# ALRhub/d3il

Hardware: AMD Instinct MI355X
Metric: env-steps/s (higher is better)
Workload: dtype f64

## Files before the change

### d3il_amd/capi.py

```python
from __future__ import annotations

import ctypes as C
import os

from .model.blob import ModelBlob

_LIB = None


class Buffers(C.Structure):
    _fields_ = [("n_envs", C.c_int32), ("stride", C.c_int32), ("obs_dim", C.c_int32), ("action_dim", C.c_int32),
                ("obs", C.c_void_p), ("done", C.c_void_p), ("success", C.c_void_p), ("mode", C.c_void_p),
                ("state", C.c_void_p), ("flags", C.c_void_p), ("step_count", C.c_void_p), ("policy_des", C.c_void_p),
                ("info_f64", C.c_void_p), ("n_info_f64", C.c_int32), ("state_rows", C.c_int32), ("last_reset", C.c_void_p)]


STATE_F64 = 42
STATE_QPOS, STATE_QVEL, STATE_BIAS, STATE_TCP, STATE_IK_Q, STATE_IK_QD = 0, 9, 18, 25, 28, 35
FLAG_MODE_MASK, FLAG_TERMINATED, FLAG_SUCCESS, FLAG_ROD_CONTACT = 0x1FF, 1 << 12, 1 << 13, 1 << 14
FLAG_IK_VALID, FLAG_SOLVER_FAIL, FLAG_MULTI_CONTACT = 1 << 15, 1 << 16, 1 << 17
PUSH_STATE_BOX, PUSH_STATE_WARM, PUSH_STATE_TASK, PUSH_STATE_F64 = 42, 68, 89, 91
PFLAG_FIRST_MASK, PFLAG_MODE_MASK, PFLAG_WARM_VALID, PFLAG_CON_OVERFLOW, PFLAG_OFF_TABLE = 0x7, 0x38, 1 << 6, 1 << 18, 1 << 19
PFLAG_LINK_NEAR = 1 << 20
LINK_GUARD_SLACK = 1.25e-4
TASK_AVOIDING, TASK_PUSHING, TASK_SORTING, TASK_STACKING, TASK_ALIGNING, TASK_INSERTING = 0, 1, 2, 3, 4, 5
ALIGN_STATE_BOX, ALIGN_STATE_WARM, ALIGN_STATE_TARGET, ALIGN_STATE_F64 = 42, 55, 70, 77
STACK_STATE_BOX, STACK_STATE_WARM, STACK_STATE_F64 = 28, 67, 94
SFLAG_MODE_MASK, SFLAG_WARM_VALID, SFLAG_HAND_NEAR = 0xFF, 1 << 8, 1 << 20
TALLY_ROW, TALLY_ALL = 514, 256
ERCCL = -7
SORT_STATE_BOX, SORT_STATE_WARM, SORT_STATE_TASK, SORT_STATE_F64 = 42, 94, 127, 129
INS_STATE_BOX, INS_STATE_WARM, INS_STATE_TASK, INS_STATE_F64 = 42, 81, 108, 110
BUILD_POISON, BUILD_SK_POISON, BUILD_STATS = 1, 2, 4
BET_TAG = 0x42655448
DDPM_GPT_TAG = 0x44470000
IBC_TAG = 0x49420000
ACT_TAG = 0x41430000
CVAE_TAG = 0x43560000
DDPM_ACT_TAG = 0x44410000
HXG_CLIPPED, HXG_NONFINITE, HXG_LAUNCHES, HXG_N = 0, 1, 2, 4

EXPORTS = ["d3il_create", "d3il_destroy", "d3il_start", "d3il_reset", "d3il_step", "d3il_get_buffers", "d3il_get_state",
           "d3il_set_state", "d3il_policy_begin", "d3il_policy_action", "d3il_attention_causal_f32", "d3il_layernorm_f32", "d3il_mlp_gelu_residual_f32", "d3il_mlp_ln_gelu_residual_f32", "d3il_linear120_f32", "d3il_mlp_ln_gelu_residual_f16x3", "d3il_linear120_f16x3", "d3il_attn_half_f16x3", "d3il_f16x3_set_guard", "d3il_bet_head_f32", "d3il_ddpm_gpt_step_f32", "d3il_ibc_langevin_f32", "d3il_act_chunk_f32", "d3il_ddpm_act_chunk_f32", "d3il_cvae_decode_f32", "d3il_ddpm_mlp_f32", "d3il_resmlp_f32", "d3il_auto_reset", "d3il_set_tally", "d3il_count_metrics",
           "d3il_rccl_available", "d3il_comm_unique_id", "d3il_comm_init", "d3il_comm_count", "d3il_comm_destroy", "d3il_reduce_metrics", "d3il_set_timing",
           "d3il_last_step_ms", "d3il_timing_stats", "d3il_step_auto_reset", "d3il_random_rollout_step", "d3il_random_rollout_prepare", "d3il_group_create", "d3il_group_flush", "d3il_group_destroy", "d3il_group_set_option", "d3il_group_stats", "d3il_set_option", "d3il_set_link_guard", "d3il_debug_stats", "d3il_debug_wave_stats", "d3il_debug_wave_counts", "d3il_debug_scratch", "d3il_debug_build_flags", "d3il_last_error", "d3il_blob_sizeof", "d3il_version"]


class D3ilError(RuntimeError):
    pass


def lib_path() -> str:
    if os.environ.get("D3IL_LIB_PATH"):
        return os.environ["D3IL_LIB_PATH"]
    name = "libd3il_rollout_stats.so" if os.environ.get("D3IL_STATS_LIB") == "1" else "libd3il_rollout.so"
    return os.path.join(os.path.dirname(os.path.abspath(__file__)), name)


def load():
    global _LIB
    if _LIB is None:
        path = lib_path()
        if not os.path.exists(path):
            raise D3ilError("%s is missing: build it with `python -m d3il_amd.build` (hipcc, gfx950). "
                            "There is no CPU fallback for the rollout path." % path)
        L = C.CDLL(path)
        L.d3il_last_error.restype = C.c_char_p
        L.d3il_blob_sizeof.restype = C.c_size_t
        L.d3il_create.argtypes = [C.c_int, C.c_int, C.c_int, C.c_void_p, C.c_size_t, C.POINTER(C.c_void_p)]
        L.d3il_destroy.argtypes = [C.c_void_p]
        L.d3il_start.argtypes = [C.c_void_p, C.c_void_p]
        L.d3il_reset.argtypes = [C.c_void_p, C.c_void_p, C.c_void_p, C.c_void_p]
        L.d3il_step.argtypes = [C.c_void_p, C.c_void_p, C.c_void_p]
        L.d3il_get_buffers.argtypes = [C.c_void_p, C.POINTER(Buffers)]
        L.d3il_get_state.argtypes = [C.c_void_p, C.c_void_p, C.c_int32, C.c_void_p, C.c_void_p]
        L.d3il_set_state.argtypes = [C.c_void_p, C.c_void_p, C.c_int32, C.c_void_p, C.c_void_p]
        L.d3il_policy_begin.argtypes = [C.c_void_p, C.c_void_p, C.c_void_p]
        L.d3il_policy_action.argtypes = [C.c_void_p, C.c_uint64, C.c_uint64, C.c_uint32, C.c_void_p, C.c_void_p]
        L.d3il_count_metrics.argtypes = [C.c_void_p, C.c_void_p, C.c_void_p]
        L.d3il_attention_causal_f32.argtypes = [C.c_void_p, C.c_void_p, C.c_int, C.c_int, C.c_int, C.c_int, C.c_void_p]
        L.d3il_layernorm_f32.argtypes = [C.c_void_p, C.c_void_p, C.c_void_p, C.c_void_p, C.c_long, C.c_int, C.c_float, C.c_void_p]
        L.d3il_mlp_ln_gelu_residual_f32.argtypes = [C.c_void_p, C.c_void_p, C.c_void_p, C.c_float, C.c_void_p, C.c_void_p, C.c_void_p, C.c_void_p, C.c_void_p, C.c_long, C.c_int, C.c_int, C.c_void_p]
        L.d3il_linear120_f32.argtypes = [C.c_void_p, C.c_void_p, C.c_void_p, C.c_float, C.c_void_p, C.c_void_p, C.c_void_p, C.c_void_p, C.c_long, C.c_int, C.c_void_p]
        L.d3il_mlp_ln_gelu_residual_f16x3.argtypes = L.d3il_mlp_ln_gelu_residual_f32.argtypes
        L.d3il_linear120_f16x3.argtypes = L.d3il_linear120_f32.argtypes
        L.d3il_attn_half_f16x3.argtypes = [C.c_void_p, C.c_void_p, C.c_void_p, C.c_float, C.c_void_p, C.c_void_p, C.c_void_p, C.c_void_p, C.c_long, C.c_int, C.c_int, C.c_int, C.c_void_p]
        L.d3il_f16x3_set_guard.argtypes = [C.c_void_p]
        L.d3il_bet_head_f32.argtypes = [C.c_void_p, C.c_void_p, C.c_void_p, C.c_float] + [C.c_void_p] * 6 + [C.c_uint64, C.c_uint64] + [C.c_void_p] * 6 + [C.c_long, C.c_int, C.c_int, C.c_int, C.c_void_p]
        L.d3il_ddpm_gpt_step_f32.argtypes = [C.c_void_p, C.c_void_p, C.c_void_p, C.c_float] + [C.c_void_p] * 11 + [C.c_uint64, C.c_uint64] + [C.c_void_p] * 7 + [C.c_long] + [C.c_int] * 5 + [C.c_void_p]
        L.d3il_ibc_langevin_f32.argtypes = [C.c_void_p] * 10 + [C.c_float] + [C.c_void_p] * 5 + [C.c_uint64, C.c_uint64] + [C.c_void_p] * 11 + [C.c_long] + [C.c_int] * 6 + [C.c_void_p]
        L.d3il_act_chunk_f32.argtypes = [C.c_void_p] * 12 + [C.c_uint64, C.c_uint64] + [C.c_void_p] * 6 + [C.c_long] + [C.c_int] * 8 + [C.c_void_p]
        L.d3il_ddpm_act_chunk_f32.argtypes = [C.c_void_p] * 13 + [C.c_uint64, C.c_uint64] + [C.c_void_p] * 9 + [C.c_long] + [C.c_int] * 12 + [C.c_void_p]
        L.d3il_cvae_decode_f32.argtypes = [C.c_void_p] * 11 + [C.c_uint64, C.c_uint64] + [C.c_void_p] * 4 + [C.c_long] + [C.c_int] * 5 + [C.c_void_p]
        L.d3il_ddpm_mlp_f32.argtypes = [C.c_void_p] * 12 + [C.c_long, C.c_int, C.c_int, C.c_int, C.c_int, C.c_void_p]
        L.d3il_resmlp_f32.argtypes = [C.c_void_p] * 8 + [C.c_long, C.c_int, C.c_int, C.c_int, C.c_int, C.c_void_p]
        L.d3il_mlp_gelu_residual_f32.argtypes = [C.c_void_p, C.c_void_p, C.c_void_p, C.c_void_p, C.c_void_p, C.c_void_p, C.c_long, C.c_int, C.c_int, C.c_void_p]
        L.d3il_auto_reset.argtypes = [C.c_void_p, C.c_void_p, C.c_void_p]
        L.d3il_step_auto_reset.argtypes = [C.c_void_p, C.c_void_p, C.c_void_p, C.c_void_p]
        L.d3il_random_rollout_step.argtypes = [C.c_void_p, C.c_uint64, C.c_uint64, C.c_uint32, C.c_void_p, C.c_void_p, C.c_void_p]
        L.d3il_random_rollout_prepare.argtypes = [C.c_void_p, C.c_uint64, C.c_uint64, C.c_uint32, C.c_void_p, C.c_void_p, C.c_void_p]
        L.d3il_timing_stats.argtypes = [C.c_void_p, C.c_void_p]
        L.d3il_set_tally.argtypes = [C.c_void_p, C.c_void_p, C.c_int, C.c_void_p]
        L.d3il_comm_unique_id.argtypes = [C.c_void_p]
        L.d3il_comm_init.argtypes = [C.c_void_p, C.c_int, C.c_int, C.c_int, C.POINTER(C.c_void_p)]
        L.d3il_comm_destroy.argtypes = [C.c_void_p]
        L.d3il_comm_count.argtypes = [C.c_void_p, C.POINTER(C.c_int)]
        L.d3il_rccl_available.restype = C.c_int
        L.d3il_reduce_metrics.argtypes = [C.c_void_p, C.c_void_p, C.c_void_p, C.c_size_t, C.c_void_p]
        L.d3il_set_timing.argtypes = [C.c_void_p, C.c_int]
        L.d3il_last_step_ms.argtypes = [C.c_void_p, C.POINTER(C.c_float)]
        L.d3il_set_option.argtypes = [C.c_void_p, C.c_char_p, C.c_int]
        L.d3il_debug_scratch.argtypes = [C.c_void_p, C.c_int, C.c_void_p, C.c_int]
        L.d3il_debug_build_flags.argtypes = [C.c_void_p]
        L.d3il_set_link_guard.argtypes = [C.c_void_p, C.c_void_p, C.c_int, C.c_double, C.c_void_p]
        if hasattr(L, "d3il_group_create"):
            L.d3il_group_create.argtypes = [C.c_void_p, C.c_int, C.POINTER(C.c_void_p)]
            L.d3il_group_flush.argtypes = [C.c_void_p]
            L.d3il_group_destroy.argtypes = [C.c_void_p]
        if hasattr(L, "d3il_group_set_option"):
            L.d3il_group_set_option.argtypes = [C.c_void_p, C.c_char_p, C.c_int]
            L.d3il_group_stats.argtypes = [C.c_void_p, C.POINTER(C.c_int64), C.POINTER(C.c_int64)]
        if L.d3il_blob_sizeof() != C.sizeof(ModelBlob):
            raise D3ilError("model blob layout mismatch between include/d3il_model_blob.h and d3il_amd/model/blob.py")
        _LIB = L
    return _LIB


def has_step_group() -> bool:
    return hasattr(load(), "d3il_group_create")


def has_group_options() -> bool:
    return hasattr(load(), "d3il_group_set_option")


def is_unknown_group_option(err: Exception) -> bool:
    return isinstance(err, D3ilError) and "d3il_group_set_option: unknown option" in str(err)


def check(rc: int):
    if rc != 0:
        raise D3ilError("libd3il_rollout error %d: %s" % (rc, load().d3il_last_error().decode()))


_CAPSULES = os.path.join(os.path.dirname(os.path.abspath(__file__)), "model", "blobs", "panda_link_capsules.json")


def link_capsules(body_names, path: str | None = None):
    import json
    import numpy as np
    with open(path or _CAPSULES) as f:
        js = json.load(f)
    rows = [[body_names.index(c["body"]), c["statics"]] + list(c["p0"]) + list(c["p1"]) + [c["r"]] for c in js["capsules"]]
    return np.ascontiguousarray(rows, dtype=np.float64), float(js["margin"])


def set_link_guard(h, capsules, margin: float, counter_ptr=None):
    import numpy as np
    caps = np.zeros((0, 9)) if capsules is None else np.ascontiguousarray(capsules, dtype=np.float64).reshape(-1, 9)
    check(load().d3il_set_link_guard(h, caps.ctypes.data_as(C.c_void_p) if len(caps) else None, len(caps), float(margin), counter_ptr))
```

### d3il_amd/csrc/rollout.hip

```cpp
#include <hip/hip_runtime.h>
#include <cstdio>
#include <cstdlib>
#include <cstring>
#include <dlfcn.h>
#include <memory>
#include <mutex>
#include <string>
#include "../../include/d3il_rollout.h"
#include "panda_step.h"
#include "rigid_common.h"
#include "gen/avoiding_consts.inc"
#include "gen/stacking_consts.inc"

namespace d3il {
constexpr int WAVE = 64;
}
#include "gen_kernels.h"
#include "link_guard.h"
#include "stack_kernels.h"
#include "policy_f16x3.h"
#include "policy_bet.h"
#include "policy_ddpm_gpt.h"
#include "policy_ibc.h"
#include "policy_act.h"
// ... 31 lines not shown
#pragma unroll
  for (int i = 0; i < NARM; i++) s[(D3IL_STATE_BIAS + i) * (size_t)stride] = st.bias[i];
#pragma unroll
  for (int i = 0; i < 3; i++) s[(D3IL_STATE_TCP + i) * (size_t)stride] = st.tcp[i];
#pragma unroll
  for (int i = 0; i < NARM; i++) s[(D3IL_STATE_IK_Q + i) * (size_t)stride] = st.ikq[i];
#pragma unroll
  for (int i = 0; i < NARM; i++) s[(D3IL_STATE_IK_QD + i) * (size_t)stride] = st.ikqd[i];
  flags[e] = st.flags; steps[e] = st.step;
}
__device__ __forceinline__ void store_outputs(const EnvState& st, int e, const float* o, unsigned char dn, float* __restrict__ obs,
                                              unsigned char* __restrict__ done, unsigned char* __restrict__ success, unsigned short* __restrict__ mode) {
  obs[2 * e] = o[0]; obs[2 * e + 1] = o[1];
  done[e] = dn; success[e] = (st.flags & F_SUCCESS) ? 1 : 0; mode[e] = (unsigned short)(st.flags & F_MODE_MASK);
}

struct AvoidResetImage {
  const double* state;
  const unsigned* flags;
  const int* steps;
  const float* obs;
};
struct AvoidEpilogue {
  AvoidResetImage img;
  double* state; unsigned* flags; int* steps; float* obs; unsigned char* done; unsigned char* success; unsigned short* mode;
  double* des; long long* episode_counts; unsigned char* mask; const int* ctx_id; long long* table;
  double* actions; double* des_before;
  unsigned long long seed, env_offset;
  int n_ctx, n, stride, pad_;
};
typedef const __attribute__((address_space(4))) AvoidEpilogue CEpilogue4;
__device__ __forceinline__ void philox4x32_10(unsigned k0, unsigned k1, unsigned c0, unsigned c1, unsigned c2, unsigned c3, unsigned* out);
template <class IM>
__device__ __forceinline__ void store_reset_image(const IM& im, double* __restrict__ state, unsigned* __restrict__ flags, int* __restrict__ steps, float* __restrict__ obs,
                                                  unsigned char* __restrict__ done, unsigned char* __restrict__ success, unsigned short* __restrict__ mode, int stride, int e) {
  const double* src = im.state;
  double* s = state + e;
#pragma unroll
  for (int i = 0; i < D3IL_STATE_F64; i++) s[i * (size_t)stride] = src[i * WAVE];
  const unsigned fl = im.flags[0];
  flags[e] = fl; steps[e] = im.steps[0];
  obs[2 * e] = im.obs[0]; obs[2 * e + 1] = im.obs[1];
  done[e] = 0; success[e] = (fl & F_SUCCESS) ? 1 : 0; mode[e] = (unsigned short)(fl & F_MODE_MASK);
}
template <class EP>
__device__ __forceinline__ void avoiding_tail_lane(const EP& a, unsigned t_next, int e) {
  if (e >= a.n) return;
  unsigned char* done = a.done; unsigned char* success = a.success; unsigned short* mode = a.mode;
  const int stride = a.stride;
  const bool fin = done[e] != 0, ok = success[e] != 0;
  const int code = (int)(short)mode[e];
  a.mask[e] = fin ? 1 : 0;
  double* des = a.des;
  if (fin) {
    long long* episode_counts = a.episode_counts;
    atomicAdd((unsigned long long*)&episode_counts[0], 1ull);
    if (ok) atomicAdd((unsigned long long*)&episode_counts[1], 1ull);
    long long* table = a.table;
    if (table) {
      const int* ctx_id = a.ctx_id;
      int c = ctx_id ? ctx_id[e] : 0;
      if (c >= 0 && c < a.n_ctx) {
        long long* row = table + (size_t)c * D3IL_TALLY_ROW;
        atomicAdd((unsigned long long*)&row[0], 1ull);
        if (ok) {
          atomicAdd((unsigned long long*)&row[1], 1ull);
          if (code >= 0 && code < D3IL_TALLY_ROW - 2) atomicAdd((unsigned long long*)&row[2 + code], 1ull);
        }
      }
    }
    store_reset_image(a.img, a.state, a.flags, a.steps, a.obs, done, success, mode, stride, e);
    const double* tcp = a.img.state + D3IL_STATE_TCP * WAVE;
#pragma unroll
    for (int k = 0; k < 3; k++) des[k * (size_t)stride + e] = tcp[k * WAVE];
  }
  unsigned long long ge = a.env_offset + (unsigned long long)e;
  const unsigned long long seed = a.seed;
  unsigned r[4];
  philox4x32_10((unsigned)seed, (unsigned)(seed >> 32), (unsigned)ge, (unsigned)(ge >> 32), t_next, 0u, r);
  double u0 = r[0] * (1.0 / 4294967296.0), u1 = r[1] * (1.0 / 4294967296.0);
  double* des_before = a.des_before;
  const double dx = des[e], dy = des[(size_t)stride + e];
  des_before[e] = dx; des_before[(size_t)stride + e] = dy;
  double x = dx + (0.02 * u0 - 0.01), y = dy + (0.02 * u1 - 0.01), z = des[2 * (size_t)stride + e];
  des[e] = x; des[(size_t)stride + e] = y;
  double* act = a.actions + (size_t)e * 7;
  act[0] = x; act[1] = y; act[2] = z; act[3] = 0; act[4] = 1; act[5] = 0; act[6] = 0;
}

template <bool FAST, bool BAKED>
__global__ __launch_bounds__(WAVE) void k_avoiding_step(const PandaConsts* __restrict__ cp, double* __restrict__ state,
                                                        unsigned* __restrict__ flags, int* __restrict__ steps,
                                                        const double* __restrict__ actions, float* __restrict__ obs,
                                                        unsigned char* __restrict__ done, unsigned char* __restrict__ success,
                                                        unsigned short* __restrict__ mode, int n, int stride, int n_substeps, int max_steps, int lanes) {
  int e = blockIdx.x * lanes + threadIdx.x;
  if ((int)threadIdx.x >= lanes || e >= n) return;
  EnvState st;
  load_state(state, flags, steps, stride, e, st);
  double act[7];
#pragma unroll
  for (int k = 0; k < 7; k++) act[k] = actions[(size_t)e * 7 + k];
  const bool bad_action = sanitize_action(act, actions + (size_t)e * 7);
  float o[2]; unsigned char dn;
#if defined(D3IL_DEVICE_STATS)
  unsigned long long t0 = wall_clock64();
#endif
  if constexpr (BAKED) env_step<FAST>(kAvoidingConsts, st, act, o, &dn, n_substeps, max_steps);
  else env_step<FAST>(*to_const_as(cp), st, act, o, &dn, n_substeps, max_steps);
#if defined(D3IL_DEVICE_STATS)
  if (threadIdx.x == 0 && blockIdx.x < 4096) g_dev_wave[blockIdx.x][9] = wall_clock64() - t0;
#endif
  if (bad_action) st.flags |= F_SOLVER_FAIL | F_TERMINATED;
  store_state(state, flags, steps, stride, e, st);
  store_outputs(st, e, o, dn, obs, done, success, mode);
}

struct RareXch {
  static constexpr bool remote = true, retire = true;
  double* buf;
  int* ctl;
  int lane, seq;
  __device__ __forceinline__ void put(int k, double v) { buf[k * WAVE + lane] = v; }
  __device__ __forceinline__ double get(int k) const { return buf[k * WAVE + lane]; }
  __device__ __forceinline__ bool post(bool need) {
    const unsigned long long m = __ballot(need);
    if (lane == 0) { ctl[2] = (int)(unsigned)m; ctl[3] = (int)(unsigned)(m >> 32); }
    __builtin_amdgcn_fence(__ATOMIC_RELEASE, "workgroup");
    if (lane == 0) __hip_atomic_store(&ctl[0], seq, __ATOMIC_RELEASE, __HIP_MEMORY_SCOPE_WORKGROUP);
    if (m == 0) return false;
    while (__builtin_amdgcn_readfirstlane(__hip_atomic_load(&ctl[1], __ATOMIC_ACQUIRE, __HIP_MEMORY_SCOPE_WORKGROUP)) != seq) __builtin_amdgcn_s_sleep(1);
    __builtin_amdgcn_fence(__ATOMIC_ACQUIRE, "workgroup");
    return true;
  }
  __device__ __forceinline__ unsigned long long wait_request() {
    while (__builtin_amdgcn_readfirstlane(__hip_atomic_load(&ctl[0], __ATOMIC_ACQUIRE, __HIP_MEMORY_SCOPE_WORKGROUP)) != seq) __builtin_amdgcn_s_sleep(2);
    __builtin_amdgcn_fence(__ATOMIC_ACQUIRE, "workgroup");
    return (unsigned long long)(unsigned)ctl[2] | ((unsigned long long)(unsigned)ctl[3] << 32);
  }
  __device__ __forceinline__ void acknowledge() {
    __builtin_amdgcn_fence(__ATOMIC_RELEASE, "workgroup");
    if (lane == 0) __hip_atomic_store(&ctl[1], seq, __ATOMIC_RELEASE, __HIP_MEMORY_SCOPE_WORKGROUP);
  }
};
constexpr size_t AVOID_LDS_SERVE = (size_t)RX_ROWS * WAVE * sizeof(double) + 4 * sizeof(int);

constexpr int AVOID_GROUP_MAX = 8;
struct AvoidGroupMember {
  double* state; unsigned* flags; int* steps; const double* actions; float* obs; unsigned char* done; unsigned char* success; unsigned short* mode;
  const AvoidEpilogue* ep;
  int n, stride;
  unsigned first_wg, pad_;
};
struct AvoidGroupTable { AvoidGroupMember m[AVOID_GROUP_MAX]; };
typedef const __attribute__((address_space(4))) AvoidGroupTable CGroupTable4;
template <bool FAST, bool SERVE, bool GROUP = false>
__global__ __launch_bounds__((SERVE ? 3 : 2) * WAVE) void k_avoiding_step_split(typename std::conditional<GROUP, const AvoidGroupTable*, const PandaConsts*>::type __restrict__ cp, double* __restrict__ state,
                                                                  unsigned* __restrict__ flags, int* __restrict__ steps,
                                                                  const double* __restrict__ actions, float* __restrict__ obs,
                                                                  unsigned char* __restrict__ done, unsigned char* __restrict__ success,
                                                                  unsigned short* __restrict__ mode, int n, int stride, int n_substeps, int max_steps,
                                                                  const AvoidEpilogue* __restrict__ ep, unsigned t_next) {
  __shared__ double xch[2][2 * NARM][WAVE];
  __shared__ double trg[2][2 * NARM + 1][WAVE];
  extern __shared__ double rx_smem[];
  __shared__ unsigned long long ep_arg[3];
  const int lane = threadIdx.x & (WAVE - 1);
  const int role = threadIdx.x / WAVE;
  RareXch rx; rx.buf = rx_smem; rx.ctl = (int*)(rx_smem + RX_ROWS * WAVE); rx.lane = lane; rx.seq = 0;
  unsigned wg_index = blockIdx.x;
  if constexpr (GROUP) {
    CGroupTable4* gt = (CGroupTable4*)(unsigned long long)cp;
    int k = 0;
#pragma unroll
    for (int j = 1; j < AVOID_GROUP_MAX; j++) if (blockIdx.x >= gt->m[j].first_wg) k = j;
    state = gt->m[k].state; flags = gt->m[k].flags; steps = gt->m[k].steps; actions = gt->m[k].actions; obs = gt->m[k].obs;
    done = gt->m[k].done; success = gt->m[k].success; mode = gt->m[k].mode; ep = gt->m[k].ep; n = gt->m[k].n; stride = gt->m[k].stride;
    wg_index = blockIdx.x - gt->m[k].first_wg;
  }
  int e = wg_index * WAVE + lane;
  const bool live = e < n;
  if (!live) e = n - 1;
  const PandaConsts& c = kAvoidingConsts;
  (void)cp;
#if defined(D3IL_POISON)
  {
    auto poison = [](void* p, int words, int idx, int nthreads) { for (int q = idx; q < words; q += nthreads) ((unsigned long long*)p)[q] = D3IL_POISON_BITS; };
    const int nt = (SERVE ? 3 : 2) * WAVE;
    poison(&xch[0][0][0], 2 * 2 * NARM * WAVE, threadIdx.x, nt);
    poison(&trg[0][0][0], 2 * (2 * NARM + 1) * WAVE, threadIdx.x, nt);
    if (SERVE) poison(rx_smem, (int)(AVOID_LDS_SERVE / 8), threadIdx.x, nt);
    __syncthreads();
  }
#endif
#if defined(D3IL_DEVICE_STATS)
  unsigned long long t0 = wall_clock64(), tw = 0;
#endif
  if (role == 0) {
    const double* sp = state + e;
    double ikq[NARM], ikqd[NARM], q0[NARM], act[7], des[7];
#pragma unroll
    for (int i = 0; i < NARM; i++) {
      ikq[i] = sp[(D3IL_STATE_IK_Q + i) * (size_t)stride]; ikqd[i] = sp[(D3IL_STATE_IK_QD + i) * (size_t)stride];
      q0[i] = sp[(D3IL_STATE_QPOS + i) * (size_t)stride];
    }
#pragma unroll
    for (int k = 0; k < 7; k++) act[k] = actions[(size_t)e * 7 + k];
    unsigned fl = flags[e];
    sanitize_action(act, actions + (size_t)e * 7);
    make_setpoint(act, des);
    double vwarm[7];
    vwarm[6] = 0.0; trg[0][2 * NARM][lane] = 0.0;
#pragma clang loop unroll(disable)
    for (int s = 0; s < n_substeps; s++) {
      {
        double trig[2 * NARM + 1];
#pragma unroll
        for (int k = 0; k <= 2 * NARM; k++) trig[k] = trg[0][k][lane];
        ik_update<FAST>(c, des, des + 3, q0, fl, ikq, ikqd, vwarm, trig);
#pragma unroll
        for (int k = 0; k <= 2 * NARM; k++) trg[0][k][lane] = trig[k];
      }
      const int b = s & 1;
#pragma unroll
      for (int k = 0; k < NARM; k++) { xch[b][k][lane] = ikq[k]; xch[b][NARM + k][lane] = ikqd[k]; }
#if defined(D3IL_DEVICE_STATS)
      unsigned long long tb = wall_clock64();
#endif
      __syncthreads();
#if defined(D3IL_DEVICE_STATS)
      tw += wall_clock64() - tb;
#endif
    }
#if defined(D3IL_DEVICE_STATS)
    if (lane == 0 && blockIdx.x < 4096) { g_dev_wave[blockIdx.x][8] = wall_clock64() - t0 - tw; }
#endif
    if (live) {
      double* so = state + e;
#pragma unroll
      for (int i = 0; i < NARM; i++) { so[(D3IL_STATE_IK_Q + i) * (size_t)stride] = ikq[i]; so[(D3IL_STATE_IK_QD + i) * (size_t)stride] = ikqd[i]; }
    }
    __syncthreads();
  } else if (SERVE && role == 2) {
    double warm[6];
    warm[5] = 0.0;
    if (lane == 0) { rx.ctl[0] = 0; rx.ctl[1] = 0; }
#pragma clang loop unroll(disable)
    for (int s = 0; s < n_substeps; s++) {
      __syncthreads();
      rx.seq = s + 1;
      const unsigned long long m = rx.wait_request();
      if (m != 0) {
#if defined(D3IL_DEVICE_STATS)
        unsigned long long tb = wall_clock64();
#endif
        if ((m >> lane) & 1ull) rare_serve(c, &rx, warm);
        rx.acknowledge();
#if defined(D3IL_DEVICE_STATS)
        tw += wall_clock64() - tb;
#endif
      }
    }
#if defined(D3IL_DEVICE_STATS)
    if (lane == 0 && blockIdx.x < 4096) g_dev_wave[blockIdx.x][7] = tw;
#endif
    __syncthreads();
  } else {
    ep_arg[0] = (unsigned long long)ep; ep_arg[1] = t_next; ep_arg[2] = wg_index;
    EnvState st;
    load_state(state, flags, steps, stride, e, st);
    float o[2]; unsigned char dn;
    step_begin(c, st, o, &dn, max_steps);
    st.flags = ((((unsigned long long)ep | t_next) != 0ull) && dn && !(st.flags & F_SUCCESS)) ? (st.flags | F_RETIRED) : (st.flags & ~F_RETIRED);
    double warm[6];
    warm[5] = 0.0;
#pragma unroll
    for (int k = 0; k < NARM; k++) { double sk, ck; sincos(st.q[k], &sk, &ck); trg[1][k][lane] = sk; trg[1][NARM + k][lane] = ck; }
#pragma clang loop unroll(disable)
    for (int s = 0; s < n_substeps; s++) {
#if defined(D3IL_DEVICE_STATS)
      unsigned long long tb = wall_clock64();
#endif
      __syncthreads();
#if defined(D3IL_DEVICE_STATS)
      tw += wall_clock64() - tb;
#endif
      const int b = s & 1;
      double qd[NARM], qdd[NARM];
#pragma unroll
      for (int k = 0; k < NARM; k++) { qd[k] = xch[b][k][lane]; qdd[k] = xch[b][NARM + k][lane]; }
#if defined(D3IL_POISON)
      for (int k = 0; k < 2 * NARM; k++) ((unsigned long long*)&xch[b][k][lane])[0] = D3IL_POISON_BITS;
#endif
      double trig[2 * NARM];
#pragma unroll
      for (int k = 0; k < 2 * NARM; k++) trig[k] = trg[1][k][lane];
      if constexpr (SERVE) { rx.seq = s + 1; control_and_physics(c, st, qd, qdd, 0.04, false, warm, trig, &rx); }
      else control_and_physics(c, st, qd, qdd, 0.04, false, warm, trig, (RareInlineRetire*)nullptr);
#pragma unroll
      for (int k = 0; k < 2 * NARM; k++) trg[1][k][lane] = trig[k];
    }
#if defined(D3IL_DEVICE_STATS)
    if (lane == 0 && blockIdx.x < 4096) { g_dev_wave[blockIdx.x][9] = wall_clock64() - t0 - tw; }
#endif
    st.flags = (st.flags & ~F_RETIRED) | F_IK_VALID;
    if (action_is_bad(actions + (size_t)e * 7)) st.flags |= F_SOLVER_FAIL | F_TERMINATED;
    step_end(c, st);
    if (live) {
      double* so = state + e;
#pragma unroll
      for (int i = 0; i < NDOF; i++) { so[(D3IL_STATE_QPOS + i) * (size_t)stride] = st.q[i]; so[(D3IL_STATE_QVEL + i) * (size_t)stride] = st.v[i]; }
#pragma unroll
      for (int i = 0; i < NARM; i++) so[(D3IL_STATE_BIAS + i) * (size_t)stride] = st.bias[i];
#pragma unroll
      for (int i = 0; i < 3; i++) so[(D3IL_STATE_TCP + i) * (size_t)stride] = st.tcp[i];
      flags[e] = st.flags; steps[e] = st.step;
      store_outputs(st, e, o, dn, obs, done, success, mode);
    }
    __syncthreads();
    const unsigned ep_lo = __builtin_amdgcn_readfirstlane((unsigned)ep_arg[0]), ep_hi = __builtin_amdgcn_readfirstlane((unsigned)(ep_arg[0] >> 32));
    const unsigned long long ep_bits = (unsigned long long)ep_lo | ((unsigned long long)ep_hi << 32);
    const unsigned lane_now = __builtin_amdgcn_mbcnt_hi(~0u, __builtin_amdgcn_mbcnt_lo(~0u, 0u));
    if (ep_bits != 0ull) {
      const unsigned wg = __builtin_amdgcn_readfirstlane((unsigned)ep_arg[2]);
      avoiding_tail_lane(*(CEpilogue4*)ep_bits, __builtin_amdgcn_readfirstlane((unsigned)ep_arg[1]), (int)(wg * WAVE + lane_now));
    }
  }
}

__global__ __launch_bounds__(WAVE) void k_avoiding_reset(const PandaConsts* __restrict__ cp, const double* __restrict__ init_qpos,
                                                         const unsigned char* __restrict__ mask, double* __restrict__ state,
                                                         unsigned* __restrict__ flags, int* __restrict__ steps, float* __restrict__ obs,
                                                         unsigned char* __restrict__ done, unsigned char* __restrict__ success,
                                                         unsigned short* __restrict__ mode, int n, int stride) {
  int e = blockIdx.x * WAVE + threadIdx.x;
  if (e >= n) return;
  if (mask && !mask[e]) return;
  EnvState st;
  double iq[NARM];
#pragma unroll
  for (int k = 0; k < NARM; k++) iq[k] = init_qpos[k];
  float o[2];
  env_reset(kAvoidingConsts, st, iq, o);
  store_state(state, flags, steps, stride, e, st);
  store_outputs(st, e, o, 0, obs, done, success, mode);
}

__global__ __launch_bounds__(WAVE) void k_avoiding_auto_reset(AvoidResetImage img, double* __restrict__ state, unsigned* __restrict__ flags, int* __restrict__ steps,
                                                              float* __restrict__ obs, unsigned char* __restrict__ done,
                                                              unsigned char* __restrict__ success, unsigned short* __restrict__ mode,
                                                              double* __restrict__ des, long long* __restrict__ episode_counts, int n, int stride) {
  int e = blockIdx.x * WAVE + threadIdx.x;
  if (e >= n || !done[e]) return;
  atomicAdd((unsigned long long*)&episode_counts[0], 1ull);
  if (success[e]) atomicAdd((unsigned long long*)&episode_counts[1], 1ull);
  store_reset_image(img, state, flags, steps, obs, done, success, mode, stride, e);
#pragma unroll
  for (int k = 0; k < 3; k++) des[k * (size_t)stride + e] = img.state[(D3IL_STATE_TCP + k) * WAVE];
}

typedef float mlp_f4 __attribute__((ext_vector_type(4)));
constexpr int MLP_C = 120, MLP_H = 480, MLP_CHUNKS = MLP_H / 16, MLP_CHUNK_F = 16 * 256;
__device__ __forceinline__ void mlp_load_row(const float* __restrict__ src, long rr, int g, const float* __restrict__ ln_w, const float* __restrict__ ln_b, float eps, float* hk) {
#pragma unroll
  for (int s2 = 0; s2 < MLP_C / 4; s2++) hk[s2] = src[rr * MLP_C + 4 * s2 + g];
  if (ln_w) {
    float sum = 0.f;
#pragma unroll
    for (int s2 = 0; s2 < MLP_C / 4; s2++) sum += hk[s2];
    sum += __shfl_xor(sum, 16); sum += __shfl_xor(sum, 32);
    const float mean = sum * (1.0f / MLP_C);
    float var = 0.f;
#pragma unroll
    for (int s2 = 0; s2 < MLP_C / 4; s2++) { const float d = hk[s2] - mean; var += d * d; }
    var += __shfl_xor(var, 16); var += __shfl_xor(var, 32);
    const float rstd = 1.0f / sqrtf(var * (1.0f / MLP_C) + eps);
#pragma unroll
    for (int s2 = 0; s2 < MLP_C / 4; s2++) hk[s2] = (hk[s2] - mean) * rstd * ln_w[4 * s2 + g] + ln_b[4 * s2 + g];
  }
}
__global__ __launch_bounds__(256) void k_mlp_gelu_residual_f32(const float* __restrict__ h, const float* __restrict__ x, const float* __restrict__ wp,
                                                                const float* __restrict__ b1, const float* __restrict__ b2, float* __restrict__ out, long M,
                                                                const float* __restrict__ ln_w, const float* __restrict__ ln_b, float eps) {
  __shared__ mlp_f4 sw[2][MLP_CHUNK_F / 4];
  const int tid = threadIdx.x, lane = tid & 63, wave = tid >> 6, j = lane & 15, g = lane >> 4;
  const long row0 = (long)blockIdx.x * 64 + wave * 16, row = row0 + j;
  const bool live = row < M;
  const long rr = live ? row : (M - 1);
  float hk[MLP_C / 4];
  mlp_load_row(h, rr, g, ln_w, ln_b, eps, hk);
  mlp_f4 acc2[8];
#pragma unroll
  for (int t = 0; t < 8; t++) acc2[t] = mlp_f4{0.f, 0.f, 0.f, 0.f};
  const mlp_f4* wp4 = (const mlp_f4*)wp;
  mlp_f4 pre[4];
#pragma unroll
  for (int q = 0; q < 4; q++) sw[0][tid + 256 * q] = wp4[tid + 256 * q];
  __syncthreads();
  for (int c = 0; c < MLP_CHUNKS; c++) {
    const int cur = c & 1;
    if (c + 1 < MLP_CHUNKS) {
#pragma unroll
      for (int q = 0; q < 4; q++) pre[q] = wp4[(long)(c + 1) * (MLP_CHUNK_F / 4) + tid + 256 * q];
    }
    mlp_f4 acc1 = mlp_f4{0.f, 0.f, 0.f, 0.f}, acc1b = mlp_f4{0.f, 0.f, 0.f, 0.f};
#pragma unroll
    for (int q = 0; q < 8; q++) {
      const mlp_f4 a4 = sw[cur][q * 64 + lane];
#pragma unroll
      for (int e = 0; e < 4; e++) if (4 * q + e < MLP_C / 4) {
        if (e & 1) acc1b = __builtin_amdgcn_mfma_f32_16x16x4f32(a4[e], hk[4 * q + e], acc1b, 0, 0, 0);
        else acc1 = __builtin_amdgcn_mfma_f32_16x16x4f32(a4[e], hk[4 * q + e], acc1, 0, 0, 0);
      }
    }
    acc1 += acc1b;
    float gv[4];
#pragma unroll
    for (int r = 0; r < 4; r++) {
      const float v = acc1[r] + b1[16 * c + 4 * g + r];
      gv[r] = 0.5f * v * (1.0f + erff(v * 0.70710678118654752440f));
    }
#pragma unroll
    for (int t = 0; t < 8; t++) {
      const mlp_f4 a4 = sw[cur][(8 + t) * 64 + lane];
#pragma unroll
      for (int e = 0; e < 4; e++) acc2[t] = __builtin_amdgcn_mfma_f32_16x16x4f32(a4[e], gv[e], acc2[t], 0, 0, 0);
    }
    if (c + 1 < MLP_CHUNKS) {
#pragma unroll
      for (int q = 0; q < 4; q++) sw[cur ^ 1][tid + 256 * q] = pre[q];
    }
    __syncthreads();
  }
  if (!live) return;
#pragma unroll
  for (int t = 0; t < 8; t++) {
    const int col = 16 * t + 4 * g;
    if (col >= MLP_C) continue;
    const mlp_f4 xr = *(const mlp_f4*)(x + row * MLP_C + col), bb = *(const mlp_f4*)(b2 + col);
    *(mlp_f4*)(out + row * MLP_C + col) = xr + bb + acc2[t];
  }
}
__global__ __launch_bounds__(256) void k_linear120_f32(const float* __restrict__ xin, const float* __restrict__ wp, const float* __restrict__ bias, const float* __restrict__ resid,
                                                        float* __restrict__ out, long M, int N, const float* __restrict__ ln_w, const float* __restrict__ ln_b, float eps) {
  __shared__ mlp_f4 sw[2][8 * 64];
  const int tid = threadIdx.x, lane = tid & 63, wave = tid >> 6, j = lane & 15, g = lane >> 4;
  const long row = (long)blockIdx.x * 64 + wave * 16 + j;
  const bool live = row < M;
  const long rr = live ? row : (M - 1);
  float hk[MLP_C / 4];
  mlp_load_row(xin, rr, g, ln_w, ln_b, eps, hk);
  const int ntiles = (N + 15) / 16;
  const mlp_f4* wp4 = (const mlp_f4*)wp;
  mlp_f4 pre[2];
#pragma unroll
  for (int q = 0; q < 2; q++) sw[0][tid + 256 * q] = wp4[tid + 256 * q];
  __syncthreads();
  for (int t = 0; t < ntiles; t++) {
    const int cur = t & 1;
    if (t + 1 < ntiles) {
#pragma unroll
      for (int q = 0; q < 2; q++) pre[q] = wp4[(long)(t + 1) * 512 + tid + 256 * q];
    }
    mlp_f4 acc = mlp_f4{0.f, 0.f, 0.f, 0.f}, acc_b = mlp_f4{0.f, 0.f, 0.f, 0.f};
#pragma unroll
    for (int q = 0; q < 8; q++) {
      const mlp_f4 a4 = sw[cur][q * 64 + lane];
#pragma unroll
      for (int e = 0; e < 4; e++) if (4 * q + e < MLP_C / 4) {
        if (e & 1) acc_b = __builtin_amdgcn_mfma_f32_16x16x4f32(a4[e], hk[4 * q + e], acc_b, 0, 0, 0);
        else acc = __builtin_amdgcn_mfma_f32_16x16x4f32(a4[e], hk[4 * q + e], acc, 0, 0, 0);
      }
    }
    const int col = 16 * t + 4 * g;
    if (live && col < N) {
      mlp_f4 v = acc + acc_b + *(const mlp_f4*)(bias + col);
      if (resid) v += *(const mlp_f4*)(resid + row * (long)N + col);
      *(mlp_f4*)(out + row * (long)N + col) = v;
    }
// ... 250 lines not shown
    }
  };
  for (int half = 0; half < 2; half++) {
    const int i = half == 0 ? p : T - 1 - p;
    if (half == 1 && i == p) break;
    float q[DR], acc[DR], kk[DR], vv[DR];
    load(base + (long)i * 3 * C, q);
#pragma unroll
    for (int d = 0; d < DR; d++) q[d] *= scale;
    load(base + C, kk); load(base + 2 * C, acc);
    float m = 0.0f, l = 1.0f;
#pragma unroll
    for (int d = 0; d < DR; d++) m += q[d] * kk[d];
    for (int j = 1; j <= i; j++) {
      const float* kj = base + (long)j * 3 * C + C;
      load(kj, kk); load(kj + C, vv);
      float sc = 0.0f;
#pragma unroll
      for (int d = 0; d < DR; d++) sc += q[d] * kk[d];
      const float mn = fmaxf(m, sc), corr = __expf(m - mn), pj = __expf(sc - mn);
      l = l * corr + pj;
#pragma unroll
      for (int d = 0; d < DR; d++) acc[d] = acc[d] * corr + pj * vv[d];
      m = mn;
    }
    float* o = out + (b * T + i) * (long)C + h * D;
    const float inv = 1.0f / l;
    if constexpr (D4 > 0) {
#pragma unroll
      for (int c = 0; c < D4; c++) reinterpret_cast<float4*>(o)[c] = make_float4(acc[4 * c] * inv, acc[4 * c + 1] * inv, acc[4 * c + 2] * inv, acc[4 * c + 3] * inv);
    } else {
#pragma unroll
      for (int d = 0; d < 32; d++) if (d < D) o[d] = acc[d] * inv;
    }
  }
  if (p == 0) {
    float s0 = 0.0f;
    for (int d = 0; d < D; d++) s0 += (base[d] * scale) * base[C + d];
    if (dd_nonfinite(s0)) {
      float* o = out + (b * T) * (long)C + h * D;
      const float qnan = __uint_as_float(0x7FC00000u);
      for (int d = 0; d < D; d++) o[d] = qnan;
    }
  }
}

__device__ __forceinline__ void philox4x32_10(unsigned k0, unsigned k1, unsigned c0, unsigned c1, unsigned c2, unsigned c3, unsigned* out) {
  const unsigned M0 = 0xD2511F53u, M1 = 0xCD9E8D57u, W0 = 0x9E3779B9u, W1 = 0xBB67AE85u;
#pragma unroll
  for (int r = 0; r < 10; r++) {
    unsigned hi0 = __umulhi(M0, c0), lo0 = M0 * c0, hi1 = __umulhi(M1, c2), lo1 = M1 * c2;
    unsigned n0 = hi1 ^ c1 ^ k0, n1 = lo1, n2 = hi0 ^ c3 ^ k1, n3 = lo0;
    c0 = n0; c1 = n1; c2 = n2; c3 = n3; k0 += W0; k1 += W1;
  }
  out[0] = c0; out[1] = c1; out[2] = c2; out[3] = c3;
}
__global__ void k_policy_begin(const unsigned char* __restrict__ mask, const double* __restrict__ state, double* __restrict__ des, int n, int stride) {
  int e = blockIdx.x * blockDim.x + threadIdx.x;
  if (e >= n || (mask && !mask[e])) return;
#pragma unroll
  for (int k = 0; k < 3; k++) des[k * (size_t)stride + e] = state[(D3IL_STATE_TCP + k) * (size_t)stride + e];
}
__global__ void k_policy_action(double* __restrict__ des, double* __restrict__ actions, unsigned long long seed, unsigned long long env_offset,
                                unsigned t, int n, int stride) {
  int e = blockIdx.x * blockDim.x + threadIdx.x;
  if (e >= n) return;
  unsigned long long ge = env_offset + (unsigned long long)e;
  unsigned r[4];
  philox4x32_10((unsigned)seed, (unsigned)(seed >> 32), (unsigned)ge, (unsigned)(ge >> 32), t, 0u, r);
  double u0 = r[0] * (1.0 / 4294967296.0), u1 = r[1] * (1.0 / 4294967296.0);
  double x = des[e] + (0.02 * u0 - 0.01), y = des[(size_t)stride + e] + (0.02 * u1 - 0.01), z = des[2 * (size_t)stride + e];
  des[e] = x; des[(size_t)stride + e] = y;
  double* a = actions + (size_t)e * 7;
  a[0] = x; a[1] = y; a[2] = z; a[3] = 0; a[4] = 1; a[5] = 0; a[6] = 0;
}
__global__ void k_policy_action_dev(double* __restrict__ des, double* __restrict__ actions, unsigned long long seed, unsigned long long env_offset,
                                    const unsigned* __restrict__ t_dev, int n, int stride) {
  int e = blockIdx.x * blockDim.x + threadIdx.x;
  if (e >= n) return;
  const unsigned t = *t_dev;
  unsigned long long ge = env_offset + (unsigned long long)e;
  unsigned r[4];
  philox4x32_10((unsigned)seed, (unsigned)(seed >> 32), (unsigned)ge, (unsigned)(ge >> 32), t, 0u, r);
  double u0 = r[0] * (1.0 / 4294967296.0), u1 = r[1] * (1.0 / 4294967296.0);
  double x = des[e] + (0.02 * u0 - 0.01), y = des[(size_t)stride + e] + (0.02 * u1 - 0.01), z = des[2 * (size_t)stride + e];
  des[e] = x; des[(size_t)stride + e] = y;
  double* a = actions + (size_t)e * 7;
  a[0] = x; a[1] = y; a[2] = z; a[3] = 0; a[4] = 1; a[5] = 0; a[6] = 0;
}
__global__ void k_inc_counter(unsigned* __restrict__ t_dev) { if (threadIdx.x == 0 && blockIdx.x == 0) *t_dev += 1u; }
__global__ __launch_bounds__(WAVE) void k_avoiding_tail(AvoidEpilogue a, unsigned t_next) { avoiding_tail_lane(a, t_next, (int)(blockIdx.x * WAVE + threadIdx.x)); }
__global__ void k_restore_des(double* __restrict__ des, const double* __restrict__ des_before, int n, int stride) {
  int e = blockIdx.x * blockDim.x + threadIdx.x;
  if (e >= n) return;
  des[e] = des_before[e]; des[(size_t)stride + e] = des_before[(size_t)stride + e];
}

__global__ void k_count_metrics(const unsigned char* __restrict__ done, const unsigned* __restrict__ flags, long long* __restrict__ counts, int n) {
  int e = blockIdx.x * blockDim.x + threadIdx.x;
  if (e >= n) return;
  if (done[e]) atomicAdd((unsigned long long*)&counts[0], 1ull);
  if (flags[e] & F_SUCCESS) {
    atomicAdd((unsigned long long*)&counts[1], 1ull);
    atomicAdd((unsigned long long*)&counts[2 + (flags[e] & F_MODE_MASK)], 1ull);
  }
}

__global__ void k_episode_tally(const unsigned char* __restrict__ done, const unsigned char* __restrict__ success, const unsigned short* __restrict__ mode,
                                const int* __restrict__ ctx_id, long long* __restrict__ table, long long* __restrict__ episode_counts, int n, int n_ctx, int mode_bias, int all_by_code) {
  int e = blockIdx.x * blockDim.x + threadIdx.x;
  if (e >= n || !done[e]) return;
  if (episode_counts) {
    atomicAdd((unsigned long long*)&episode_counts[0], 1ull);
    if (success[e]) atomicAdd((unsigned long long*)&episode_counts[1], 1ull);
  }
  if (!table) return;
  int c = ctx_id ? ctx_id[e] : 0;
  if (c < 0 || c >= n_ctx) return;
  long long* row = table + (size_t)c * D3IL_TALLY_ROW;
  atomicAdd((unsigned long long*)&row[0], 1ull);
  int code = (int)(short)mode[e] + mode_bias;
  if (success[e]) {
    atomicAdd((unsigned long long*)&row[1], 1ull);
    if (code >= 0 && code < D3IL_TALLY_ROW - 2) atomicAdd((unsigned long long*)&row[2 + code], 1ull);
  }
  if (all_by_code && code >= 0 && code < 256) atomicAdd((unsigned long long*)&row[2 + D3IL_TALLY_ALL + code], 1ull);
}
__global__ void k_store_contexts(const unsigned char* __restrict__ mask, const double* __restrict__ src, double* __restrict__ dst, int n, int dim) {
  int i = blockIdx.x * blockDim.x + threadIdx.x;
  if (i >= n * dim) return;
  if (mask && !mask[i / dim]) return;
  dst[i] = src[i];
}

}

using namespace d3il;

static_assert(D3IL_STACK_STATE_BOX == SK_STATE_BOX && D3IL_STACK_STATE_WARM == SK_STATE_WARM && D3IL_STACK_STATE_F64 == SK_STATE_F64, "d3il_rollout.h: Stacking state layout");
static_assert(D3IL_SFLAG_WARM_VALID == SKF_WARM_VALID && D3IL_SFLAG_HAND_NEAR == SKF_HAND_NEAR && D3IL_PFLAG_CON_OVERFLOW == SKF_CON_OVERFLOW && D3IL_PFLAG_OFF_TABLE == SKF_OFF_TABLE,
              "d3il_rollout.h: Stacking flag bits");
static_assert(D3IL_PFLAG_LINK_NEAR == LG_FLAG && D3IL_PFLAG_LINK_NEAR == D3IL_SFLAG_HAND_NEAR, "d3il_rollout.h: the link-near bit of the generic engine is the hand-near bit of the cooperative one");
static_assert(D3IL_SFLAG_MODE_MASK == (SKF_NMODE_MASK | (0x3Fu << SKF_IND_SHIFT)), "d3il_rollout.h: Stacking order code");
static_assert(D3IL_ALIGN_STATE_BOX == AL_STATE_BOX && D3IL_ALIGN_STATE_WARM == AL_STATE_WARM && D3IL_ALIGN_STATE_TARGET == AL_STATE_TARGET && D3IL_ALIGN_STATE_F64 == AL_STATE_F64, "d3il_rollout.h: Aligning state layout");
static_assert(D3IL_INS_STATE_BOX == 42 && D3IL_INS_STATE_WARM == 42 + 13 * 3 && D3IL_INS_STATE_TASK == 42 + 13 * 3 + 6 * 3 + NDOF && D3IL_INS_STATE_F64 == gen_state_rows(3), "d3il_rollout.h: Inserting state layout");
static_assert(D3IL_PUSH_STATE_BOX == 42 && D3IL_PUSH_STATE_WARM == 42 + 13 * 2 && D3IL_PUSH_STATE_TASK == 42 + 13 * 2 + 6 * 2 + NDOF && D3IL_PUSH_STATE_F64 == gen_state_rows(2) && D3IL_TALLY_ALL + 256 <= D3IL_TALLY_ROW - 2,
              "d3il_rollout.h: Pushing state rows / tally row");

static inline bool gen_task(int task_id) {
  return task_id == D3IL_TASK_SORTING || task_id == D3IL_TASK_INSERTING || task_id == D3IL_TASK_PUSHING;
}

constexpr int RG_SLOTS = 2, RG_SAMPLE = 8;
struct d3il_handle_s {
  int task_id, n, stride, device;
  PandaConsts hc;
  PandaConsts* dc;
  GenConsts gc;
  StackConsts kc;
  AlignTask atk;
  double* d_scratch;
  int state_rows;
  double* d_init_qpos;
  bool started;
  d3il_buffers buf;
  bool fast, timing;
  int split;
  bool serve_avail;
  int serve_max_wg;
  int lanes;
  int lds_pad;
  hipEvent_t ev0, ev1;
  bool ev_valid, ev_created;
  hipEvent_t ring0[128], ring1[128];
  bool ring_created;
  long ring_head, ring_drained, t_n;
  double t_sum, t_min, t_max;
  int tol_mode;
  int stack_reset_coop;
  unsigned long long kc_id;
  double* d_ctx;
  int ctx_dim;
  uint8_t* d_mask;
  const int32_t* tally_ctx; int tally_nctx; int64_t* tally_table;
  bool rg_enabled, rg_ready, rg_capturing, rg_ev_made, rg_timing;
  int rg_slot;
  hipGraph_t rg_graph[RG_SLOTS]; hipGraphExec_t rg_exec[RG_SLOTS];
  unsigned* rg_t_dev; uint32_t rg_next_t; long rg_launched, rg_drained;
  uint64_t rg_seed, rg_off; double* rg_actions; int64_t* rg_counts; hipStream_t rg_stream;
  void* d_reset_img; AvoidResetImage reset_img; AvoidEpilogue* d_epilogue; AvoidEpilogue epilogue_host; bool epilogue_valid; hipStream_t epilogue_stream;
  bool prep_valid; uint32_t prep_t; uint64_t prep_seed, prep_off; double* prep_actions; bool fuse_tail; double* d_des_before; hipStream_t prep_stream;
  bool info_is_view;
  d3il_model_blob model;
  LinkGuardConsts lg; LinkGuardConsts* d_lg; int64_t* lg_flagged;
  struct d3il_group_s* group; int grp_set; bool grp_pending; uint64_t grp_seed, grp_off; uint32_t grp_t; double* grp_actions; int64_t* grp_counts; hipStream_t grp_stream;
  hipEvent_t ring_alt0[128], ring_alt1[128];
};
struct d3il_dispatch_set {
  int count; d3il_handle_s* m[AVOID_GROUP_MAX];
  int n_pending;
  uint32_t t; int n_substeps, max_steps; bool timing;
  AvoidGroupTable* d_table; AvoidGroupTable table_host; bool table_valid;
  hipEvent_t ev_join[AVOID_GROUP_MAX], ev_done; bool ev_made;
  hipEvent_t ring0[128], ring1[128]; bool ring_created; long ring_head;
  bool armed;
};
struct d3il_group_s {
  int device, count; d3il_handle_s* m[AVOID_GROUP_MAX];
  int n_sets; d3il_dispatch_set set[AVOID_GROUP_MAX];
  int n_pending; bool busy;
  bool quiet; int64_t n_merged, n_joined;
};
static inline void group_arm(d3il_group_s* g) { for (int k = 0; k < AVOID_GROUP_MAX; k++) g->set[k].armed = true; }
#if defined(D3IL_EVENT_SYSTEM_FENCE)
constexpr unsigned EV_ORDER_FLAGS = hipEventDisableTiming, EV_TIMING_FLAGS = hipEventDefault;
#else
constexpr unsigned EV_ORDER_FLAGS = hipEventDisableTiming | hipEventDisableSystemFence, EV_TIMING_FLAGS = hipEventDefault | hipEventDisableSystemFence;
#endif

struct ActiveModel { int refs; bool valid; GenConsts gc; StackConsts kc; };
static ActiveModel g_active_gen[16], g_active_stack[16];
static int g_active_tol[16];
static std::mutex g_model_mutex;

static unsigned long long g_stack_loaded_id[16];
static StackConsts g_stack_loaded[16];
static unsigned long long g_kc_counter = 0;

static thread_local std::string g_err;
static int fail(int code, const std::string& msg) { g_err = msg; return code; }
#define HIPCHK(x) do { hipError_t e_ = (x); if (e_ != hipSuccess) return fail(D3IL_EHIP, std::string(#x) + ": " + hipGetErrorString(e_)); } while (0)

extern "C" {

static int group_flush(d3il_group_s* g);
static inline int group_settle(d3il_handle_s* h) {
  if (!h || !h->group || h->group->busy) return D3IL_OK;
  group_arm(h->group);
  return h->group->n_pending ? group_flush(h->group) : D3IL_OK;
}
#define GROUP_SETTLE(h) do { if (int rc_g_ = group_settle(h)) return rc_g_; } while (0)

const char* d3il_last_error(void) { return g_err.c_str(); }
size_t d3il_blob_sizeof(void) { return sizeof(d3il_model_blob); }
int d3il_version(void) { return 2; }

static void rg_drop(d3il_handle_s* h);
static void group_leave(d3il_handle_s* h);
static void rg_drop_for_free(d3il_handle_s* h) {
  if (h->rg_ready) for (int k = 0; k < RG_SLOTS; k++) { (void)hipGraphExecDestroy(h->rg_exec[k]); (void)hipGraphDestroy(h->rg_graph[k]); }
  if (h->rg_t_dev) (void)hipFree(h->rg_t_dev);
}
static void free_handle(d3il_handle_s* h) {
  if (!h) return;
  int dev = h->device;
  if (dev >= 0 && dev < 16) {
    std::lock_guard<std::mutex> lock(g_model_mutex);
    if (gen_task(h->task_id) && g_active_gen[dev].refs > 0) g_active_gen[dev].refs--;
    if (h->task_id == D3IL_TASK_STACKING && g_active_stack[dev].refs > 0) g_active_stack[dev].refs--;
  }
  void* ptrs[] = {h->dc, h->d_init_qpos, h->buf.obs, h->buf.done, h->buf.success, h->buf.mode, h->buf.state, h->buf.flags, h->buf.step_count, h->buf.policy_des,
                  h->info_is_view ? nullptr : (void*)h->buf.info_f64, h->d_scratch, h->d_ctx, h->d_mask, h->d_des_before, h->d_lg, h->d_reset_img, h->d_epilogue};
  for (void* p : ptrs) if (p) (void)hipFree(p);
  if (h->ring_created) for (int i = 0; i < 128; i++) { (void)hipEventDestroy(h->ring0[i]); (void)hipEventDestroy(h->ring1[i]); }
  rg_drop_for_free(h);
  delete h;
}
#define HIPCHK_H(x) do { hipError_t e_ = (x); if (e_ != hipSuccess) { free_handle(h); return fail(D3IL_EHIP, std::string(#x) + ": " + hipGetErrorString(e_)); } } while (0)

int d3il_create(int task_id, int n_envs, int device_id, const void* model_blob, size_t blob_len, d3il_handle* out) {
  if (!out || !model_blob) return fail(D3IL_EINVAL, "d3il_create: null argument");
  *out = nullptr;
  if (blob_len != sizeof(d3il_model_blob)) return fail(D3IL_EBLOB, "d3il_create: blob size mismatch");
  if (n_envs <= 0) return fail(D3IL_EINVAL, "d3il_create: n_envs must be positive");
  const d3il_model_blob& m = *(const d3il_model_blob*)model_blob;
  if (task_id != m.task_id) return fail(D3IL_EINVAL, "d3il_create: task_id does not match the model blob");
  if (task_id != D3IL_TASK_AVOIDING && task_id != D3IL_TASK_PUSHING && task_id != D3IL_TASK_SORTING && task_id != D3IL_TASK_STACKING && task_id != D3IL_TASK_ALIGNING && task_id != D3IL_TASK_INSERTING)
    return fail(D3IL_EUNSUPPORTED, "d3il_create: unknown task id (Avoiding, Pushing, Sorting, Stacking, Aligning and Inserting are implemented)");
  int ndev = 0;
  if (hipGetDeviceCount(&ndev) != hipSuccess || ndev <= 0) return fail(D3IL_ENODEVICE, "d3il_create: no HIP device available (there is no CPU fallback)");
  if (device_id < 0 || device_id >= ndev || device_id >= 16) return fail(D3IL_ENODEVICE, "d3il_create: device_id out of range");
  HIPCHK(hipSetDevice(device_id));
  d3il_handle_s* h = new d3il_handle_s();
  std::memset(&h->buf, 0, sizeof h->buf);
  h->task_id = -1; h->device = device_id;
  h->model = m; h->d_lg = nullptr; h->lg_flagged = nullptr; h->lg.n = 0;
  h->dc = nullptr; h->d_init_qpos = nullptr; h->d_scratch = nullptr; h->d_ctx = nullptr; h->d_mask = nullptr; h->ev_created = false; h->ring_created = false;
  h->tally_ctx = nullptr; h->tally_nctx = 0; h->tally_table = nullptr; h->tol_mode = 0; h->ctx_dim = 0; h->stack_reset_coop = 1; h->kc_id = 0;
  const char* err = "";
  int rc = build_panda_consts(m, h->hc, &err);
  if (rc) { free_handle(h); return fail(D3IL_EBLOB, std::string("d3il_create: ") + err); }
  finish_invweights(h->hc);
  if (gen_task(task_id) && build_gen_consts(m, h->hc, h->gc, &err)) { free_handle(h); return fail(D3IL_EBLOB, std::string("d3il_create: ") + err); }
  if (task_id == D3IL_TASK_STACKING && build_stack_consts(m, h->hc, h->kc, &err)) { free_handle(h); return fail(D3IL_EBLOB, std::string("d3il_create: ") + err); }
  if (task_id == D3IL_TASK_ALIGNING && build_coop_align_consts(m, h->hc, h->kc, h->atk, &err)) { free_handle(h); return fail(D3IL_EBLOB, std::string("d3il_create: ") + err); }
  {
    PandaConsts a = h->hc, b = task_id == D3IL_TASK_STACKING ? kStackingConsts : kAvoidingConsts;
    if (task_id != D3IL_TASK_AVOIDING) {
      a.n_obst = b.n_obst;
      std::memcpy(a.ob_c, b.ob_c, sizeof a.ob_c); std::memcpy(a.ob_u, b.ob_u, sizeof a.ob_u); std::memcpy(a.ob_r, b.ob_r, sizeof a.ob_r); std::memcpy(a.ob_h, b.ob_h, sizeof a.ob_h);
      std::memcpy(a.ct_K, b.ct_K, sizeof a.ct_K); std::memcpy(a.ct_B, b.ct_B, sizeof a.ct_B); std::memcpy(a.ct_solimp, b.ct_solimp, sizeof a.ct_solimp);
      std::memcpy(a.ct_margin, b.ct_margin, sizeof a.ct_margin); std::memcpy(a.ct_fric, b.ct_fric, sizeof a.ct_fric); std::memcpy(a.task_f, b.task_f, sizeof a.task_f);
    }
    bool same = a.n_obst == b.n_obst && a.ik_iters == b.ik_iters;
    a.n_obst = b.n_obst = 0; a.ik_iters = b.ik_iters = 0; a.n_substeps = b.n_substeps = 0; a.max_steps = b.max_steps = 0; a.pad_i = b.pad_i = 0; a.pad_j = b.pad_j = 0;
    const double* pa = (const double*)&a; const double* pb = (const double*)&b;
    for (size_t i = 0; same && i < sizeof(PandaConsts) / sizeof(double); i++) {
      double d = pa[i] - pb[i], m = pa[i] < 0 ? -pa[i] : pa[i];
      if (!(d <= 1e-12 * (m > 1 ? m : 1) && -d <= 1e-12 * (m > 1 ? m : 1))) same = false;
    }
    if (!same) { free_handle(h); return fail(D3IL_EUNSUPPORTED, "d3il_create: the model blob differs from the model this library was specialised for at build time; "
                                                                 "regenerate csrc/gen/*_consts.inc and rebuild (python -m d3il_amd.build)"); }
  }
  const bool sorting = gen_task(task_id);
  const bool gen_pushing = sorting && task_id == D3IL_TASK_PUSHING;
  const bool stacking = task_id == D3IL_TASK_STACKING;
  if (stacking) {
    ActiveModel& am = g_active_stack[device_id];
    bool other;
    { std::lock_guard<std::mutex> lock(g_model_mutex); other = am.refs > 0 && std::memcmp(&am.kc, &h->kc, sizeof(StackConsts)) != 0; }
    if (other) {
      free_handle(h);
      return fail(D3IL_EUNSUPPORTED, "d3il_create: another live Stacking handle on this device uses a different model (the kernels read one model per device from constant memory); destroy it first");
    }
  }
  h->n = n_envs; h->stride = (n_envs + WAVE - 1) / WAVE * WAVE;
  h->started = false; h->split = -1; h->serve_avail = true; h->serve_max_wg = 256; h->lanes = WAVE; h->lds_pad = -1; h->fast = true; h->timing = false; h->ev_valid = false;
  const bool aligning = task_id == D3IL_TASK_ALIGNING;
  h->state_rows = (sorting ? gen_state_rows(h->gc.nb) : (stacking ? SK_STATE_F64 : (aligning ? AL_STATE_F64 : D3IL_STATE_F64)));
  h->ctx_dim = (sorting ? 7 * h->gc.nb : (stacking ? 21 : (aligning ? AL_CTX : 0)));
  size_t S = (size_t)h->stride;
  d3il_buffers& b = h->buf;
  b.n_envs = n_envs; b.stride = h->stride; b.obs_dim = sorting ? 2 + 3 * h->gc.nb : (stacking ? SK_OBS : (aligning ? AL_OBS : 2)); b.action_dim = stacking ? SK_ACT : 7; b.state_rows = h->state_rows; b.n_info_f64 = (aligning || gen_pushing) ? 2 : (stacking ? 1 : 0);
  HIPCHK_H(hipMalloc(&h->dc, sizeof(PandaConsts)));
  if (task_id == D3IL_TASK_AVOIDING) {
    if (hipFuncSetAttribute((const void*)k_avoiding_step_split<true, true>, hipFuncAttributeMaxDynamicSharedMemorySize, (int)AVOID_LDS_SERVE) != hipSuccess) {
      (void)hipGetLastError();
      h->serve_avail = false; h->serve_max_wg = 0;
    }
    const size_t img_bytes = (size_t)WAVE * (D3IL_STATE_F64 * sizeof(double) + sizeof(unsigned) + sizeof(int) + 2 * sizeof(float) + 2 + sizeof(unsigned short));
    HIPCHK_H(hipMalloc(&h->d_reset_img, img_bytes)); HIPCHK_H(hipMemset(h->d_reset_img, 0, img_bytes));
    HIPCHK_H(hipMalloc(&h->d_epilogue, sizeof(AvoidEpilogue)));
  }
  HIPCHK_H(hipMemcpy(h->dc, &h->hc, sizeof(PandaConsts), hipMemcpyHostToDevice));
  HIPCHK_H(hipMalloc(&h->d_init_qpos, 7 * sizeof(double)));
  HIPCHK_H(hipMalloc(&b.obs, S * b.obs_dim * sizeof(float)));
  HIPCHK_H(hipMalloc(&b.done, S)); HIPCHK_H(hipMalloc(&b.success, S));
  HIPCHK_H(hipMalloc(&b.mode, S * sizeof(uint16_t)));
  HIPCHK_H(hipMalloc(&b.state, S * h->state_rows * sizeof(double)));
  HIPCHK_H(hipMalloc(&b.flags, S * sizeof(uint32_t)));
  HIPCHK_H(hipMalloc(&b.step_count, S * sizeof(int32_t)));
  HIPCHK_H(hipMalloc(&b.policy_des, S * 3 * sizeof(double)));
  HIPCHK_H(hipMalloc(&h->d_mask, S)); HIPCHK_H(hipMemset(h->d_mask, 0, S));
  b.last_reset = h->d_mask;
  HIPCHK_H(hipMemset(b.obs, 0, S * b.obs_dim * sizeof(float))); HIPCHK_H(hipMemset(b.done, 0, S)); HIPCHK_H(hipMemset(b.success, 0, S));
  HIPCHK_H(hipMemset(b.mode, 0, S * sizeof(uint16_t))); HIPCHK_H(hipMemset(b.state, 0, S * h->state_rows * sizeof(double)));
  HIPCHK_H(hipMemset(b.flags, 0, S * sizeof(uint32_t))); HIPCHK_H(hipMemset(b.step_count, 0, S * sizeof(int32_t)));
  HIPCHK_H(hipMemset(b.policy_des, 0, S * 3 * sizeof(double)));
  if (h->ctx_dim) { HIPCHK_H(hipMalloc(&h->d_ctx, S * h->ctx_dim * sizeof(double))); HIPCHK_H(hipMemset(h->d_ctx, 0, S * h->ctx_dim * sizeof(double))); }
  if (sorting) {
    {
      std::lock_guard<std::mutex> lock(g_model_mutex);
      g_active_gen[device_id].refs++; h->task_id = task_id;
    }
#if defined(D3IL_POISON)
    HIPCHK_H(hipMalloc(&h->d_scratch, S * GG_BLOCK * sizeof(double))); HIPCHK_H(hipMemset(h->d_scratch, 0xFF, S * GG_BLOCK * sizeof(double)));
#else
    HIPCHK_H(hipMalloc(&h->d_scratch, S * GG_BLOCK * sizeof(double))); HIPCHK_H(hipMemset(h->d_scratch, 0, S * GG_BLOCK * sizeof(double)));
#endif
    if (gen_pushing) { b.info_f64 = b.state + (size_t)(gen_state_rows(h->gc.nb) - 2) * S; h->info_is_view = true; }
    HIPCHK_H(hipFuncSetAttribute((const void*)k_sorting_step<true, false>, hipFuncAttributeMaxDynamicSharedMemorySize, GEN_LDS_STEP));
    HIPCHK_H(hipFuncSetAttribute((const void*)k_sorting_step<false, false>, hipFuncAttributeMaxDynamicSharedMemorySize, GEN_LDS_STEP));
    HIPCHK_H(hipFuncSetAttribute((const void*)k_sorting_step<true, true>, hipFuncAttributeMaxDynamicSharedMemorySize, GEN_LDS_STEP));
    HIPCHK_H(hipFuncSetAttribute((const void*)k_sorting_step<false, true>, hipFuncAttributeMaxDynamicSharedMemorySize, GEN_LDS_STEP));
    HIPCHK_H(hipFuncSetAttribute((const void*)k_sorting_reset, hipFuncAttributeMaxDynamicSharedMemorySize, GEN_LDS_H));
  }
  if (stacking) {
    ActiveModel& am = g_active_stack[device_id];
    {
      std::unique_lock<std::mutex> lock(g_model_mutex);
      if (am.refs == 0) am.kc = h->kc;
      am.refs++; h->task_id = task_id;
      h->kc_id = ++g_kc_counter;
    }
    HIPCHK_H(hipMalloc(&b.info_f64, S * sizeof(double))); HIPCHK_H(hipMemset(b.info_f64, 0, S * sizeof(double)));
    HIPCHK_H(hipMalloc(&h->d_scratch, S * SG_SIZE * sizeof(double))); HIPCHK_H(hipMemset(h->d_scratch, 0, S * SG_SIZE * sizeof(double)));
    HIPCHK_H(hipFuncSetAttribute((const void*)k_stacking_step, hipFuncAttributeMaxDynamicSharedMemorySize, STACK_LDS));
    HIPCHK_H(hipFuncSetAttribute((const void*)k_stacking_reset, hipFuncAttributeMaxDynamicSharedMemorySize, STACK_LDS_RESET));
  }
  if (aligning) {
    {
      std::lock_guard<std::mutex> lock(g_model_mutex);
      h->kc_id = ++g_kc_counter;
    }
    HIPCHK_H(hipMalloc(&b.info_f64, S * 2 * sizeof(double))); HIPCHK_H(hipMemset(b.info_f64, 0, S * 2 * sizeof(double)));
    HIPCHK_H(hipMalloc(&h->d_scratch, S * SG_SIZE * sizeof(double))); HIPCHK_H(hipMemset(h->d_scratch, 0, S * SG_SIZE * sizeof(double)));
    HIPCHK_H(hipFuncSetAttribute((const void*)k_aligning_step, hipFuncAttributeMaxDynamicSharedMemorySize, STACK_LDS));
  }
  h->task_id = task_id;
  h->ring_created = false; h->ring_head = h->ring_drained = h->t_n = 0; h->t_sum = 0; h->t_min = 1e300; h->t_max = 0;
  h->ev_created = true;
  *out = h;
  return D3IL_OK;
}

int d3il_destroy(d3il_handle h) {
  if (!h) return fail(D3IL_EINVAL, "d3il_destroy: null handle");
  (void)hipSetDevice(h->device);
  group_leave(h);
  (void)hipDeviceSynchronize();
  free_handle(h);
  return D3IL_OK;
}

int d3il_start(d3il_handle h, const double* init_qpos7) {
  GROUP_SETTLE(h);
  if (!h || !init_qpos7) return fail(D3IL_EINVAL, "d3il_start: null argument");
  for (int k = 0; k < 7; k++) if (!(init_qpos7[k] == init_qpos7[k])) return fail(D3IL_EINVAL, "d3il_start: init_qpos contains NaN");
  HIPCHK(hipSetDevice(h->device));
  HIPCHK(hipMemcpy(h->d_init_qpos, init_qpos7, 7 * sizeof(double), hipMemcpyHostToDevice));
  if (h->task_id == D3IL_TASK_AVOIDING) {
    double* st = (double*)h->d_reset_img;
    unsigned* fl = (unsigned*)(st + (size_t)D3IL_STATE_F64 * WAVE);
    int* sc = (int*)(fl + WAVE);
    float* ob = (float*)(sc + WAVE);
    unsigned char* dn = (unsigned char*)(ob + 2 * WAVE);
    unsigned short* md = (unsigned short*)(dn + 2 * WAVE);
    HIPCHK(hipDeviceSynchronize());
    hipLaunchKernelGGL(k_avoiding_reset, dim3(1), dim3(WAVE), 0, (hipStream_t)nullptr, h->dc, h->d_init_qpos, (const unsigned char*)nullptr, st, fl, sc, ob, dn, dn + WAVE, md, 1, WAVE);
    HIPCHK(hipGetLastError());
    HIPCHK(hipDeviceSynchronize());
    h->reset_img.state = st; h->reset_img.flags = fl; h->reset_img.steps = sc; h->reset_img.obs = ob;
  }
  h->started = true;
  return D3IL_OK;
}

static AlignTask g_align_loaded[16];
static bool g_align_loaded_valid[16];
static int sync_stack_consts_locked(d3il_handle_s* h) {
  if (h->task_id == D3IL_TASK_ALIGNING && (!g_align_loaded_valid[h->device] || std::memcmp(&g_align_loaded[h->device], &h->atk, sizeof(AlignTask)) != 0)) {
    HIPCHK(hipDeviceSynchronize());
    HIPCHK(hipMemcpyToSymbol(HIP_SYMBOL(g_align_task), &h->atk, sizeof(AlignTask)));
    HIPCHK(hipDeviceSynchronize());
    g_align_loaded[h->device] = h->atk; g_align_loaded_valid[h->device] = true;
  }
  if (g_stack_loaded_id[h->device] == h->kc_id) return D3IL_OK;
  if (g_stack_loaded_id[h->device] != 0 && std::memcmp(&g_stack_loaded[h->device], &h->kc, sizeof(StackConsts)) == 0) { g_stack_loaded_id[h->device] = h->kc_id; return D3IL_OK; }
  HIPCHK(hipDeviceSynchronize());
  HIPCHK(hipMemcpyToSymbol(HIP_SYMBOL(g_stack_consts), &h->kc, sizeof(StackConsts)));
  HIPCHK(hipDeviceSynchronize());
  g_stack_loaded[h->device] = h->kc; g_stack_loaded_id[h->device] = h->kc_id;
  return D3IL_OK;
}
struct StackLaunch {
  std::unique_lock<std::mutex> lock;
  int rc;
  explicit StackLaunch(d3il_handle_s* h) : lock(g_model_mutex), rc(sync_stack_consts_locked(h)) {}
};

static GenConsts g_gen_loaded[16];
static bool g_gen_loaded_valid[16];
static int sync_gen_consts_locked(d3il_handle_s* h) {
  if (g_gen_loaded_valid[h->device] && std::memcmp(&g_gen_loaded[h->device], &h->gc, sizeof(GenConsts)) == 0) return D3IL_OK;
  HIPCHK(hipDeviceSynchronize());
  HIPCHK(hipMemcpyToSymbol(HIP_SYMBOL(g_gen_consts), &h->gc, sizeof(GenConsts)));
  HIPCHK(hipDeviceSynchronize());
  g_gen_loaded[h->device] = h->gc; g_gen_loaded_valid[h->device] = true;
  return D3IL_OK;
}
struct GenLaunch {
  std::unique_lock<std::mutex> lock;
  int rc;
  explicit GenLaunch(d3il_handle_s* h) : lock(g_model_mutex), rc(sync_gen_consts_locked(h)) {}
};

static int sync_solver_tol(d3il_handle_s* h, hipStream_t s) {
  static const SolverTol k_tol[2] = {SOLVER_TOL_PRODUCTION, SOLVER_TOL_STRICT};
  if (h->task_id == D3IL_TASK_AVOIDING) return D3IL_OK;
  std::lock_guard<std::mutex> lock(g_model_mutex);
  if (g_active_tol[h->device] == h->tol_mode) return D3IL_OK;
  (void)s;
  HIPCHK(hipDeviceSynchronize());
  HIPCHK(hipMemcpyToSymbol(HIP_SYMBOL(g_solver_tol), &k_tol[h->tol_mode ? 1 : 0], sizeof(SolverTol)));
  HIPCHK(hipDeviceSynchronize());
  g_active_tol[h->device] = h->tol_mode;
  return D3IL_OK;
}

static int drop_prepared_action(d3il_handle_s* h) {
  if (!h->prep_valid) return D3IL_OK;
  h->prep_valid = false;
  HIPCHK(hipSetDevice(h->device));
  hipLaunchKernelGGL(k_restore_des, dim3((h->n + 255) / 256), dim3(256), 0, h->prep_stream, h->buf.policy_des, h->d_des_before, h->n, h->stride);
  HIPCHK(hipGetLastError());
  return D3IL_OK;
}
int d3il_reset(d3il_handle h, const uint8_t* env_mask, const double* contexts, void* stream) {
  GROUP_SETTLE(h);
  if (!h) return fail(D3IL_EINVAL, "d3il_reset: null handle");
  if (int rc_ = drop_prepared_action(h)) return rc_;
  if (!h->started) return fail(D3IL_ESTATE, "d3il_reset: d3il_start() has not been called (env.start() before env.reset())");
  HIPCHK(hipSetDevice(h->device));
  d3il_buffers& b = h->buf;
  if (h->ctx_dim && !contexts) return fail(D3IL_EINVAL, "d3il_reset: this task needs contexts (device f64 [n_envs][ctx_dim]: Pushing 14, Sorting 7 n_boxes, Stacking 21, Aligning 14)");
  if (!h->ctx_dim && contexts) return fail(D3IL_EUNSUPPORTED, "d3il_reset: the Avoiding task takes no contexts");
  if (int rc = sync_solver_tol(h, (hipStream_t)stream)) return rc;
  if (h->ctx_dim && contexts && contexts != h->d_ctx) {
    int tot = h->n * h->ctx_dim;
    hipLaunchKernelGGL(k_store_contexts, dim3((tot + 255) / 256), dim3(256), 0, (hipStream_t)stream, env_mask, contexts, h->d_ctx, h->n, h->ctx_dim);
    HIPCHK(hipGetLastError());
  }
  if (gen_task(h->task_id)) {
    if (!contexts) return fail(D3IL_EINVAL, "d3il_reset: the task needs contexts (device f64 [n_envs][7 * n_boxes])");
    GenLaunch guard(h);
    if (guard.rc) return guard.rc;
    hipLaunchKernelGGL(k_sorting_reset, dim3((h->n + GEN_LANES - 1) / GEN_LANES), dim3(WAVE), GEN_LDS_H, (hipStream_t)stream, h->d_init_qpos, env_mask, contexts, b.state,
                       b.flags, b.step_count, b.obs, b.done, b.success, b.mode, h->d_scratch, h->n, h->stride);
    HIPCHK(hipGetLastError());
    return D3IL_OK;
  }
  if (h->task_id == D3IL_TASK_STACKING) {
    if (!contexts) return fail(D3IL_EINVAL, "d3il_reset: the Stacking task needs contexts (device f64 [n_envs][21])");
    StackLaunch guard(h);
    if (guard.rc) return guard.rc;
    if (h->stack_reset_coop)
      hipLaunchKernelGGL(k_stacking_step, dim3((h->n + SK_LANES - 1) / SK_LANES), dim3(WAVE), STACK_LDS, (hipStream_t)stream, b.state, b.flags, b.step_count, (const double*)nullptr, b.obs,
                         b.done, b.success, b.mode, b.info_f64, h->d_scratch, h->n, h->stride, 1, h->hc.max_steps, 1, env_mask, h->d_init_qpos, contexts);
    else
      hipLaunchKernelGGL(k_stacking_reset, dim3((h->n + SK_LANES - 1) / SK_LANES), dim3(WAVE), STACK_LDS_RESET, (hipStream_t)stream, h->d_init_qpos, env_mask, contexts, b.state,
                         b.flags, b.step_count, b.obs, b.done, b.success, b.mode, b.info_f64, h->d_scratch, h->n, h->stride);
    HIPCHK(hipGetLastError());
    return D3IL_OK;
  }
  if (h->task_id == D3IL_TASK_ALIGNING) {
    if (!contexts) return fail(D3IL_EINVAL, "d3il_reset: the Aligning task needs contexts (device f64 [n_envs][14]: box pos3 quat4 | target pos3 quat4)");
    StackLaunch guard(h);
    if (guard.rc) return guard.rc;
    hipLaunchKernelGGL(k_aligning_step, dim3((h->n + SK_LANES - 1) / SK_LANES), dim3(WAVE), STACK_LDS, (hipStream_t)stream, b.state, b.flags, b.step_count, (const double*)nullptr, b.obs,
                       b.done, b.success, b.mode, b.info_f64, h->d_scratch, h->n, h->stride, 1, h->hc.max_steps, 1, env_mask, h->d_init_qpos, contexts);
    HIPCHK(hipGetLastError());
    return D3IL_OK;
  }
  if (contexts) return fail(D3IL_EUNSUPPORTED, "d3il_reset: the Avoiding task takes no contexts");
  hipLaunchKernelGGL(k_avoiding_reset, dim3(h->stride / WAVE), dim3(WAVE), 0, (hipStream_t)stream, h->dc, h->d_init_qpos, env_mask, b.state, b.flags,
                     b.step_count, b.obs, b.done, b.success, b.mode, h->n, h->stride);
  HIPCHK(hipGetLastError());
  return D3IL_OK;
}

static int timing_drain_one(d3il_handle h) {
  const int slot = (int)(h->ring_drained % 128);
  float ms = 0;
  hipEvent_t e0 = h->ring_alt0[slot] ? h->ring_alt0[slot] : h->ring0[slot], e1 = h->ring_alt1[slot] ? h->ring_alt1[slot] : h->ring1[slot];
  HIPCHK(hipEventSynchronize(e1));
  HIPCHK(hipEventElapsedTime(&ms, e0, e1));
  h->t_sum += ms; h->t_n++; if (ms < h->t_min) h->t_min = ms; if (ms > h->t_max) h->t_max = ms;
  h->ring_drained++;
  return D3IL_OK;
}
static int timing_begin(d3il_handle h, hipStream_t s) {
  if (h->ring_head - h->ring_drained >= 128) { if (int rc = timing_drain_one(h)) return rc; }
  const int slot = (int)(h->ring_head % 128);
  h->ev0 = h->ring0[slot]; h->ev1 = h->ring1[slot]; h->ring_alt0[slot] = nullptr; h->ring_alt1[slot] = nullptr;
  HIPCHK(hipEventRecord(h->ev0, s));
  return D3IL_OK;
}
static bool split_step_kernel(const d3il_handle_s* h) { return h->task_id == D3IL_TASK_AVOIDING && h->fast && h->lanes == WAVE && h->split != 0; }
static int step_launch(d3il_handle h, const double* actions, void* stream, const AvoidEpilogue* ep, unsigned t_next);
int d3il_step(d3il_handle h, const double* actions, void* stream) { GROUP_SETTLE(h); return step_launch(h, actions, stream, nullptr, 0u); }
static int step_launch(d3il_handle h, const double* actions, void* stream, const AvoidEpilogue* ep, unsigned t_next) {
  if (!h || !actions) return fail(D3IL_EINVAL, "d3il_step: null argument");
  if (int rc_ = drop_prepared_action(h)) return rc_;
  if (!h->started) return fail(D3IL_ESTATE, "d3il_step: d3il_start() has not been called");
  HIPCHK(hipSetDevice(h->device));
  d3il_buffers& b = h->buf;
  hipStream_t s = (hipStream_t)stream;
  if (int rc = sync_solver_tol(h, s)) return rc;
  if (gen_task(h->task_id)) {
    int nwgs = (h->n + GEN_LANES - 1) / GEN_LANES;
    GenLaunch guard(h);
    if (guard.rc) return guard.rc;
    if (h->timing) { if (int rc_ = timing_begin(h, s)) return rc_; }
#define D3IL_GEN_LAUNCH(F, R) hipLaunchKernelGGL((k_sorting_step<F, R>), dim3(nwgs), dim3((1 + GEN_NSUB) * WAVE), GEN_LDS_STEP, s, b.state, b.flags, b.step_count, actions, b.obs, b.done, \
                                                  b.success, b.mode, h->d_scratch, h->n, h->stride, h->hc.n_substeps, h->hc.max_steps)
    if (h->gc.rod_static) { if (h->fast) D3IL_GEN_LAUNCH(true, true); else D3IL_GEN_LAUNCH(false, true); }
    else { if (h->fast) D3IL_GEN_LAUNCH(true, false); else D3IL_GEN_LAUNCH(false, false); }
#undef D3IL_GEN_LAUNCH
    HIPCHK(hipGetLastError());
    if (h->timing) { HIPCHK(hipEventRecord(h->ev1, s)); h->ev_valid = true; h->ring_head++; }
    if (h->lg.n > 0) {
      hipLaunchKernelGGL(k_gen_link_guard, dim3((h->n + LG_ENVS - 1) / LG_ENVS), dim3(GEN_WAVE), 0, s, h->d_lg, b.state, b.flags, (unsigned long long*)h->lg_flagged, h->n, h->stride);
      HIPCHK(hipGetLastError());
    }
    return D3IL_OK;
  }
  if (h->task_id == D3IL_TASK_STACKING) {
    StackLaunch guard(h);
    if (guard.rc) return guard.rc;
    if (h->timing) { if (int rc_ = timing_begin(h, s)) return rc_; }
    hipLaunchKernelGGL(k_stacking_step, dim3((h->n + SK_LANES - 1) / SK_LANES), dim3(WAVE), STACK_LDS, s, b.state, b.flags, b.step_count, actions, b.obs, b.done, b.success, b.mode,
                       b.info_f64, h->d_scratch, h->n, h->stride, h->hc.n_substeps, h->hc.max_steps, 0, (const unsigned char*)nullptr, (const double*)nullptr, (const double*)nullptr);
    HIPCHK(hipGetLastError());
    if (h->timing) { HIPCHK(hipEventRecord(h->ev1, s)); h->ev_valid = true; h->ring_head++; }
    return D3IL_OK;
  }
  if (h->task_id == D3IL_TASK_ALIGNING) {
    StackLaunch guard(h);
    if (guard.rc) return guard.rc;
    if (h->timing) { if (int rc_ = timing_begin(h, s)) return rc_; }
    hipLaunchKernelGGL(k_aligning_step, dim3((h->n + SK_LANES - 1) / SK_LANES), dim3(WAVE), STACK_LDS, s, b.state, b.flags, b.step_count, actions, b.obs, b.done, b.success, b.mode,
                       b.info_f64, h->d_scratch, h->n, h->stride, h->hc.n_substeps, h->hc.max_steps, 0, (const unsigned char*)nullptr, (const double*)nullptr, (const double*)nullptr);
    HIPCHK(hipGetLastError());
    if (h->timing) { HIPCHK(hipEventRecord(h->ev1, s)); h->ev_valid = true; h->ring_head++; }
    return D3IL_OK;
  }
  int nwg = (h->n + h->lanes - 1) / h->lanes, lds = h->lds_pad;
  if (lds < 0) {
    int per_cu = (nwg + 255) / 256;
    lds = per_cu >= 8 ? 0 : (160 * 1024 / per_cu) - 1024;
    if (lds > 64 * 1024) lds = 64 * 1024;
  }
  if (h->timing && !h->rg_capturing) { if (int rc_ = timing_begin(h, s)) return rc_; }
  const bool split = split_step_kernel(h);
  if (ep && !split) return fail(D3IL_ESTATE, "d3il_step: the rollout epilogue needs the split step kernel");
  if (split && nwg <= h->serve_max_wg)
    hipLaunchKernelGGL((k_avoiding_step_split<true, true>), dim3(nwg), dim3(3 * WAVE), AVOID_LDS_SERVE, s, h->dc, b.state, b.flags, b.step_count, actions, b.obs, b.done,
                       b.success, b.mode, h->n, h->stride, h->hc.n_substeps, h->hc.max_steps, ep, t_next);
  else if (split)
    hipLaunchKernelGGL((k_avoiding_step_split<true, false>), dim3(nwg), dim3(2 * WAVE), 0, s, h->dc, b.state, b.flags, b.step_count, actions, b.obs, b.done,
                       b.success, b.mode, h->n, h->stride, h->hc.n_substeps, h->hc.max_steps, ep, t_next);
  else if (h->fast)
    hipLaunchKernelGGL((k_avoiding_step<true, true>), dim3(nwg), dim3(WAVE), lds, s, h->dc, b.state, b.flags, b.step_count, actions, b.obs, b.done,
                       b.success, b.mode, h->n, h->stride, h->hc.n_substeps, h->hc.max_steps, h->lanes);
  else
    hipLaunchKernelGGL((k_avoiding_step<false, true>), dim3(nwg), dim3(WAVE), lds, s, h->dc, b.state, b.flags, b.step_count, actions, b.obs, b.done,
                       b.success, b.mode, h->n, h->stride, h->hc.n_substeps, h->hc.max_steps, h->lanes);
  HIPCHK(hipGetLastError());
  if (h->timing && !h->rg_capturing) { HIPCHK(hipEventRecord(h->ev1, s)); h->ev_valid = true; h->ring_head++; }
  return D3IL_OK;
}

int d3il_get_buffers(d3il_handle h, d3il_buffers* out) {
  if (!h || !out) return fail(D3IL_EINVAL, "d3il_get_buffers: null argument");
  *out = h->buf;
  return D3IL_OK;
}

static int check_state_rows(d3il_handle h, const void* state, int32_t state_rows, const char* who) {
  if (state && state_rows != h->state_rows)
    return fail(D3IL_EINVAL, std::string(who) + ": the caller's buffer has " + std::to_string(state_rows) + " state rows, this handle has " + std::to_string(h->state_rows) +
                                 " (d3il_buffers.state_rows)");
  return D3IL_OK;
}
int d3il_get_state(d3il_handle h, double* state, int32_t state_rows, uint32_t* flags, int32_t* steps) {
  GROUP_SETTLE(h);
  if (!h) return fail(D3IL_EINVAL, "d3il_get_state: null handle");
  if (int rc_ = check_state_rows(h, state, state_rows, "d3il_get_state")) return rc_;
  HIPCHK(hipSetDevice(h->device));
  HIPCHK(hipDeviceSynchronize());
  if (state) HIPCHK(hipMemcpy2D(state, (size_t)h->n * 8, h->buf.state, (size_t)h->stride * 8, (size_t)h->n * 8, h->state_rows, hipMemcpyDeviceToHost));
  if (flags) HIPCHK(hipMemcpy(flags, h->buf.flags, (size_t)h->n * 4, hipMemcpyDeviceToHost));
  if (steps) HIPCHK(hipMemcpy(steps, h->buf.step_count, (size_t)h->n * 4, hipMemcpyDeviceToHost));
  return D3IL_OK;
}
int d3il_set_state(d3il_handle h, const double* state, int32_t state_rows, const uint32_t* flags, const int32_t* steps) {
  GROUP_SETTLE(h);
  if (!h) return fail(D3IL_EINVAL, "d3il_set_state: null handle");
  if (int rc_ = check_state_rows(h, state, state_rows, "d3il_set_state")) return rc_;
  if (int rc_ = drop_prepared_action(h)) return rc_;
  HIPCHK(hipSetDevice(h->device));
  HIPCHK(hipDeviceSynchronize());
  if (state) HIPCHK(hipMemcpy2D(h->buf.state, (size_t)h->stride * 8, state, (size_t)h->n * 8, (size_t)h->n * 8, h->state_rows, hipMemcpyHostToDevice));
  if (flags) HIPCHK(hipMemcpy(h->buf.flags, flags, (size_t)h->n * 4, hipMemcpyHostToDevice));
  if (steps) HIPCHK(hipMemcpy(h->buf.step_count, steps, (size_t)h->n * 4, hipMemcpyHostToDevice));
  return D3IL_OK;
}

int d3il_policy_begin(d3il_handle h, const uint8_t* env_mask, void* stream) {
  GROUP_SETTLE(h);
  if (!h) return fail(D3IL_EINVAL, "d3il_policy_begin: null handle");
  if (int rc_ = drop_prepared_action(h)) return rc_;
  HIPCHK(hipSetDevice(h->device));
  hipLaunchKernelGGL(k_policy_begin, dim3((h->n + 255) / 256), dim3(256), 0, (hipStream_t)stream, env_mask, h->buf.state, h->buf.policy_des, h->n, h->stride);
  HIPCHK(hipGetLastError());
  return D3IL_OK;
}
int d3il_policy_action(d3il_handle h, uint64_t seed, uint64_t env_offset, uint32_t t, double* actions, void* stream) {
  GROUP_SETTLE(h);
  if (!h || !actions) return fail(D3IL_EINVAL, "d3il_policy_action: null argument");
  if (int rc_ = drop_prepared_action(h)) return rc_;
  if (h->buf.action_dim != 7) return fail(D3IL_EUNSUPPORTED, "d3il_policy_action: the random Cartesian policy writes 7-wide rows (Avoiding / Pushing / Sorting); Stacking actions are 8 wide");
  HIPCHK(hipSetDevice(h->device));
  hipLaunchKernelGGL(k_policy_action, dim3((h->n + 255) / 256), dim3(256), 0, (hipStream_t)stream, h->buf.policy_des, actions, (unsigned long long)seed,
                     (unsigned long long)env_offset, t, h->n, h->stride);
  HIPCHK(hipGetLastError());
  return D3IL_OK;
}
int d3il_attention_causal_f32(const float* qkv, float* out, int B, int T, int H, int D, void* stream) {
  if (!qkv || !out) return fail(D3IL_EINVAL, "d3il_attention_causal_f32: null argument");
  if (B < 0 || T < 1 || T > 32 || H < 1 || D < 1 || D > 32) return fail(D3IL_EINVAL, "d3il_attention_causal_f32: needs 1 <= T <= 32, 1 <= D <= 32");
  const long total = (long)B * H * ((T + 1) / 2);
  if (total == 0) return D3IL_OK;
  const dim3 grid((unsigned)((total + 255) / 256)), block(256);
  const bool aligned = D % 4 == 0 && ((uintptr_t)qkv % 16) == 0 && ((uintptr_t)out % 16) == 0;
  if (aligned && D == 20) hipLaunchKernelGGL(k_attention_causal_f32<5>, grid, block, 0, (hipStream_t)stream, qkv, out, B, T, H, D);
  else if (aligned && D == 16) hipLaunchKernelGGL(k_attention_causal_f32<4>, grid, block, 0, (hipStream_t)stream, qkv, out, B, T, H, D);
  else if (aligned && D == 32) hipLaunchKernelGGL(k_attention_causal_f32<8>, grid, block, 0, (hipStream_t)stream, qkv, out, B, T, H, D);
  else hipLaunchKernelGGL(k_attention_causal_f32<0>, grid, block, 0, (hipStream_t)stream, qkv, out, B, T, H, D);
  HIPCHK(hipGetLastError());
  return D3IL_OK;
}
int d3il_layernorm_f32(const float* x, const float* weight, const float* bias, float* y, long rows, int C, float eps, void* stream) {
  if (!x || !weight || !bias || !y) return fail(D3IL_EINVAL, "d3il_layernorm_f32: null argument");
  if (rows < 0 || C < 4 || C > 128 || C % 4 != 0) return fail(D3IL_EINVAL, "d3il_layernorm_f32: needs 4 <= C <= 128, C a multiple of 4");
  if (((uintptr_t)x | (uintptr_t)y | (uintptr_t)weight | (uintptr_t)bias) % 16 != 0) return fail(D3IL_EINVAL, "d3il_layernorm_f32: pointers must be 16-byte aligned");
  if (rows == 0) return D3IL_OK;
  const long threads = rows * 32;
  hipLaunchKernelGGL(k_layernorm_f32, dim3((unsigned)((threads + 255) / 256)), dim3(256), 0, (hipStream_t)stream, x, weight, bias, y, rows, C, eps);
  HIPCHK(hipGetLastError());
  return D3IL_OK;
}
int d3il_linear120_f32(const float* xin, const float* ln_weight, const float* ln_bias, float ln_eps, const float* w_packed, const float* bias, const float* resid, float* out,
                       long rows, int N, void* stream) {
  if (!xin || !w_packed || !bias || !out) return fail(D3IL_EINVAL, "d3il_linear120_f32: null argument");
  if ((ln_weight == nullptr) != (ln_bias == nullptr)) return fail(D3IL_EINVAL, "d3il_linear120_f32: LayerNorm weight and bias come together");
  if (rows < 0 || N < 4 || N % 4 != 0) return fail(D3IL_EINVAL, "d3il_linear120_f32: needs rows >= 0 and N a positive multiple of 4");
  if (((uintptr_t)xin | (uintptr_t)w_packed | (uintptr_t)bias | (uintptr_t)resid | (uintptr_t)out) % 16 != 0) return fail(D3IL_EINVAL, "d3il_linear120_f32: pointers must be 16-byte aligned");
  if (rows == 0) return D3IL_OK;
  hipLaunchKernelGGL(k_linear120_f32, dim3((unsigned)((rows + 63) / 64)), dim3(256), 0, (hipStream_t)stream, xin, w_packed, bias, resid, out, rows, N, ln_weight, ln_bias, ln_eps);
  HIPCHK(hipGetLastError());
  return D3IL_OK;
}
int d3il_ddpm_mlp_f32(const float* state, const float* noise, const float* temb, const float* w_in, const float* b_in, const float* w_blocks, const float* b_blocks,
                      const float* w_out, const float* b_out, const float* sched, const float* bounds, float* out, long rows, int state_dim, int n_timesteps, int hidden,
                      int n_blocks, void* stream) {
  if (!state || !noise || !temb || !w_in || !b_in || !w_blocks || !b_blocks || !w_out || !b_out || !sched || !bounds || !out) return fail(D3IL_EINVAL, "d3il_ddpm_mlp_f32: null argument");
  if (hidden != DD_H) return fail(D3IL_EUNSUPPORTED, "d3il_ddpm_mlp_f32: built for hidden 256 (the DiffusionMLP of the DDPM configs)");
  if (state_dim < 1 || state_dim > 18) return fail(D3IL_EUNSUPPORTED, "d3il_ddpm_mlp_f32: action 2 + time embedding 8 + state must fit 28 inputs (state_dim <= 18)");
  if (n_timesteps < 1 || n_blocks < 0 || rows < 0) return fail(D3IL_EINVAL, "d3il_ddpm_mlp_f32: bad counts");
  if (((uintptr_t)w_in | (uintptr_t)b_in | (uintptr_t)w_blocks | (uintptr_t)b_blocks | (uintptr_t)w_out) % 16 != 0) return fail(D3IL_EINVAL, "d3il_ddpm_mlp_f32: weights and biases must be 16-byte aligned");
  if (rows == 0) return D3IL_OK;
  hipLaunchKernelGGL(k_ddpm_mlp_f32, dim3((unsigned)((rows + 15) / 16)), dim3(64 * DD_NW), 0, (hipStream_t)stream, state, noise, temb, w_in, b_in, w_blocks, b_blocks, w_out, b_out, sched, bounds, out,
                     rows, state_dim, n_timesteps, n_blocks);
  HIPCHK(hipGetLastError());
  return D3IL_OK;
}
int d3il_resmlp_f32(const float* x, const float* w_in, const float* b_in, const float* w_blocks, const float* b_blocks, const float* w_out, const float* b_out, float* out, long rows,
                    int in_dim, int hidden, int n_blocks, int out_dim, void* stream) {
  if (!x || !w_in || !b_in || !w_blocks || !b_blocks || !w_out || !b_out || !out) return fail(D3IL_EINVAL, "d3il_resmlp_f32: null argument");
  if (hidden != 128 && hidden != 256) return fail(D3IL_EUNSUPPORTED, "d3il_resmlp_f32: built for hidden 128 and 256 (the ResidualMLPNetwork of the BC and DDPM configs)");
  if (in_dim < 1 || in_dim > 28 || out_dim < 1 || out_dim > 16) return fail(D3IL_EUNSUPPORTED, "d3il_resmlp_f32: at most 28 inputs and 16 outputs");
  if (n_blocks < 0 || rows < 0) return fail(D3IL_EINVAL, "d3il_resmlp_f32: bad counts");
  if (((uintptr_t)w_in | (uintptr_t)b_in | (uintptr_t)w_blocks | (uintptr_t)b_blocks | (uintptr_t)w_out) % 16 != 0) return fail(D3IL_EINVAL, "d3il_resmlp_f32: weights and biases must be 16-byte aligned");
  if (rows == 0) return D3IL_OK;
  const dim3 grid((unsigned)((rows + 15) / 16)), block(512);
  if (hidden == 128) hipLaunchKernelGGL(k_resmlp_f32<128>, grid, block, 0, (hipStream_t)stream, x, w_in, b_in, w_blocks, b_blocks, w_out, b_out, out, rows, in_dim, out_dim, n_blocks);
  else hipLaunchKernelGGL(k_resmlp_f32<256>, grid, block, 0, (hipStream_t)stream, x, w_in, b_in, w_blocks, b_blocks, w_out, b_out, out, rows, in_dim, out_dim, n_blocks);
  HIPCHK(hipGetLastError());
  return D3IL_OK;
}
int d3il_mlp_gelu_residual_f32(const float* h, const float* x, const float* w_packed, const float* b1, const float* b2, float* out, long rows, int C, int H, void* stream) {
  return d3il_mlp_ln_gelu_residual_f32(h, nullptr, nullptr, 0.f, x, w_packed, b1, b2, out, rows, C, H, stream);
}
int d3il_mlp_ln_gelu_residual_f32(const float* h, const float* ln_weight, const float* ln_bias, float ln_eps, const float* x, const float* w_packed, const float* b1, const float* b2,
                                  float* out, long rows, int C, int H, void* stream) {
  if ((ln_weight == nullptr) != (ln_bias == nullptr)) return fail(D3IL_EINVAL, "d3il_mlp_ln_gelu_residual_f32: LayerNorm weight and bias come together");
  if (!h || !x || !w_packed || !b1 || !b2 || !out) return fail(D3IL_EINVAL, "d3il_mlp_gelu_residual_f32: null argument");
  if (C != MLP_C || H != MLP_H) return fail(D3IL_EUNSUPPORTED, "d3il_mlp_gelu_residual_f32: built for n_embd 120, hidden 480 (the DiffusionGPT of the BESO configs)");
  if (rows < 0) return fail(D3IL_EINVAL, "d3il_mlp_gelu_residual_f32: negative row count");
  if (((uintptr_t)h | (uintptr_t)x | (uintptr_t)w_packed | (uintptr_t)b2 | (uintptr_t)out) % 16 != 0) return fail(D3IL_EINVAL, "d3il_mlp_gelu_residual_f32: pointers must be 16-byte aligned");
  if (rows == 0) return D3IL_OK;
  hipLaunchKernelGGL(k_mlp_gelu_residual_f32, dim3((unsigned)((rows + 63) / 64)), dim3(256), 0, (hipStream_t)stream, h, x, w_packed, b1, b2, out, rows, ln_weight, ln_bias, ln_eps);
  HIPCHK(hipGetLastError());
  return D3IL_OK;
}
static long long* g_hx_guard_counts = nullptr;
int d3il_f16x3_set_guard(long long* counts_device) {
  g_hx_guard_counts = counts_device;
  return D3IL_OK;
}
int d3il_mlp_ln_gelu_residual_f16x3(const float* h, const float* ln_weight, const float* ln_bias, float ln_eps, const float* x, const void* w_packed, const float* b1, const float* b2,
                                    float* out, long rows, int C, int H, void* stream) {
  if ((ln_weight == nullptr) != (ln_bias == nullptr)) return fail(D3IL_EINVAL, "d3il_mlp_ln_gelu_residual_f16x3: LayerNorm weight and bias come together");
  if (!h || !x || !w_packed || !b1 || !b2 || !out) return fail(D3IL_EINVAL, "d3il_mlp_ln_gelu_residual_f16x3: null argument");
  if (C != HX_C || H != HX_H) return fail(D3IL_EUNSUPPORTED, "d3il_mlp_ln_gelu_residual_f16x3: built for n_embd 120, hidden 480 (the DiffusionGPT of the BESO configs)");
  if (rows < 0) return fail(D3IL_EINVAL, "d3il_mlp_ln_gelu_residual_f16x3: negative row count");
  if (((uintptr_t)h | (uintptr_t)x | (uintptr_t)w_packed | (uintptr_t)b2 | (uintptr_t)out) % 16 != 0) return fail(D3IL_EINVAL, "d3il_mlp_ln_gelu_residual_f16x3: pointers must be 16-byte aligned");
  if (rows == 0) return D3IL_OK;
  const dim3 grid((unsigned)((rows + 16 * HX_MLP_NW - 1) / (16 * HX_MLP_NW))), block(64 * HX_MLP_NW);
  if (long long* counts = g_hx_guard_counts)
    hipLaunchKernelGGL((k_mlp_gelu_residual_f16x3<HX_MLP_NW, true>), grid, block, 0, (hipStream_t)stream, h, x, (const hx_h8*)w_packed, b1, b2, out, rows, ln_weight, ln_bias, ln_eps, counts);
  else
    hipLaunchKernelGGL((k_mlp_gelu_residual_f16x3<HX_MLP_NW, false>), grid, block, 0, (hipStream_t)stream, h, x, (const hx_h8*)w_packed, b1, b2, out, rows, ln_weight, ln_bias, ln_eps, (long long*)nullptr);
  HIPCHK(hipGetLastError());
  return D3IL_OK;
}
int d3il_linear120_f16x3(const float* xin, const float* ln_weight, const float* ln_bias, float ln_eps, const void* w_packed, const float* bias, const float* resid, float* out,
                         long rows, int N, void* stream) {
  if (!xin || !w_packed || !bias || !out) return fail(D3IL_EINVAL, "d3il_linear120_f16x3: null argument");
  if ((ln_weight == nullptr) != (ln_bias == nullptr)) return fail(D3IL_EINVAL, "d3il_linear120_f16x3: LayerNorm weight and bias come together");
  if (rows < 0 || N < 4 || N % 4 != 0 || N > 384) return fail(D3IL_EINVAL, "d3il_linear120_f16x3: needs rows >= 0 and N a multiple of 4 in 4 .. 384");
  if (((uintptr_t)xin | (uintptr_t)w_packed | (uintptr_t)bias | (uintptr_t)resid | (uintptr_t)out) % 16 != 0) return fail(D3IL_EINVAL, "d3il_linear120_f16x3: pointers must be 16-byte aligned");
  if (rows == 0) return D3IL_OK;
  const dim3 grid((unsigned)((rows + 16 * HX_LIN_NW - 1) / (16 * HX_LIN_NW))), block(64 * HX_LIN_NW);
  if (long long* counts = g_hx_guard_counts)
    hipLaunchKernelGGL((k_linear120_f16x3<HX_LIN_NW, true>), grid, block, 0, (hipStream_t)stream, xin, (const hx_h8*)w_packed, bias, resid, out, rows, N, ln_weight, ln_bias, ln_eps, counts);
  else
    hipLaunchKernelGGL((k_linear120_f16x3<HX_LIN_NW, false>), grid, block, 0, (hipStream_t)stream, xin, (const hx_h8*)w_packed, bias, resid, out, rows, N, ln_weight, ln_bias, ln_eps, (long long*)nullptr);
  HIPCHK(hipGetLastError());
  return D3IL_OK;
}
int d3il_attn_half_f16x3(const float* x, const float* ln_weight, const float* ln_bias, float ln_eps, const void* w_packed, const float* b_qkv, const float* b_proj, float* out,
// ... 137 lines not shown
             n_env, obs_dim, latent, A, n_blocks};
  const dim3 grid((unsigned)((n_env + 15) / 16)), block(512);
  if (hidden == 128) hipLaunchKernelGGL(k_cvae_decode<128>, grid, block, 0, (hipStream_t)stream, a);
  else hipLaunchKernelGGL(k_cvae_decode<256>, grid, block, 0, (hipStream_t)stream, a);
  HIPCHK(hipGetLastError());
  return D3IL_OK;
}
int d3il_set_tally(d3il_handle h, const int32_t* ctx_id_device, int n_ctx, int64_t* table_device) {
  GROUP_SETTLE(h);
  if (!h) return fail(D3IL_EINVAL, "d3il_set_tally: null handle");
  if (table_device && n_ctx <= 0) return fail(D3IL_EINVAL, "d3il_set_tally: n_ctx must be positive");
  if (h->rg_ready) { HIPCHK(hipDeviceSynchronize()); rg_drop(h); }
  h->tally_ctx = ctx_id_device; h->tally_nctx = n_ctx; h->tally_table = table_device;
  return D3IL_OK;
}

int d3il_auto_reset(d3il_handle h, int64_t* episode_counts_device, void* stream) {
  GROUP_SETTLE(h);
  if (!h) return fail(D3IL_EINVAL, "d3il_auto_reset: null handle");
  if (int rc_ = drop_prepared_action(h)) return rc_;
  if (!h->started) return fail(D3IL_ESTATE, "d3il_auto_reset: d3il_start() has not been called");
  HIPCHK(hipSetDevice(h->device));
  d3il_buffers& b = h->buf;
  hipStream_t s = (hipStream_t)stream;
  const bool avoiding = h->task_id == D3IL_TASK_AVOIDING;
  if (avoiding && !episode_counts_device) return fail(D3IL_EINVAL, "d3il_auto_reset: the Avoiding task needs episode_counts (device i64[2])");
  HIPCHK(hipMemcpyAsync(h->d_mask, b.done, (size_t)h->n, hipMemcpyDeviceToDevice, s));
  if (h->tally_table || (!avoiding && episode_counts_device)) {
    hipLaunchKernelGGL(k_episode_tally, dim3((h->n + 255) / 256), dim3(256), 0, s, b.done, b.success, b.mode, h->tally_ctx, (long long*)h->tally_table,
                       avoiding ? (long long*)nullptr : (long long*)episode_counts_device, h->n, h->tally_nctx, (h->task_id == D3IL_TASK_PUSHING || h->task_id == D3IL_TASK_ALIGNING) ? 1 : 0,
                       (h->task_id == D3IL_TASK_STACKING || h->task_id == D3IL_TASK_INSERTING) ? 1 : 0);
    HIPCHK(hipGetLastError());
  }
  if (avoiding) {
    hipLaunchKernelGGL(k_avoiding_auto_reset, dim3(h->stride / WAVE), dim3(WAVE), 0, s, h->reset_img, b.state, b.flags, b.step_count,
                       b.obs, b.done, b.success, b.mode, b.policy_des, (long long*)episode_counts_device, h->n, h->stride);
    HIPCHK(hipGetLastError());
    return D3IL_OK;
  }
  if (int rc = d3il_reset(h, h->d_mask, h->d_ctx, stream)) return rc;
  return d3il_policy_begin(h, h->d_mask, stream);
}

int d3il_count_metrics(d3il_handle h, int64_t* out_counts_device, void* stream) {
  GROUP_SETTLE(h);
  if (!h || !out_counts_device) return fail(D3IL_EINVAL, "d3il_count_metrics: null argument");
  if (h->task_id != D3IL_TASK_AVOIDING) return fail(D3IL_EUNSUPPORTED, "d3il_count_metrics: Avoiding only");
  HIPCHK(hipSetDevice(h->device));
  HIPCHK(hipMemsetAsync(out_counts_device, 0, (2 + 512) * sizeof(int64_t), (hipStream_t)stream));
  hipLaunchKernelGGL(k_count_metrics, dim3((h->n + 255) / 256), dim3(256), 0, (hipStream_t)stream, h->buf.done, h->buf.flags, (long long*)out_counts_device, h->n);
  HIPCHK(hipGetLastError());
  return D3IL_OK;
}
namespace {
struct RcclApi {
  int (*GetUniqueId)(void*);
  int (*CommInitRank)(void**, int, d3il_rccl_unique_id, int);
  int (*CommDestroy)(void*);
  int (*AllReduce)(const void*, void*, size_t, int, int, void*, hipStream_t);
  int (*CommCount)(void*, int*);
  const char* (*GetErrorString)(int);
  bool ok;
};
RcclApi* rccl_api() {
  static RcclApi api = [] {
    RcclApi a{}; a.ok = false;
    void* hnd = RTLD_DEFAULT;
    if (!dlsym(hnd, "ncclAllReduce")) {
      hnd = dlopen("librccl.so", RTLD_NOW | RTLD_GLOBAL);
      if (!hnd) hnd = dlopen("librccl.so.1", RTLD_NOW | RTLD_GLOBAL);
      if (!hnd) hnd = dlopen("/opt/rocm/lib/librccl.so", RTLD_NOW | RTLD_GLOBAL);
      if (!hnd) return a;
    }
    a.GetUniqueId = (int (*)(void*))dlsym(hnd, "ncclGetUniqueId");
    a.CommInitRank = (int (*)(void**, int, d3il_rccl_unique_id, int))dlsym(hnd, "ncclCommInitRank");
    a.CommDestroy = (int (*)(void*))dlsym(hnd, "ncclCommDestroy");
    a.AllReduce = (int (*)(const void*, void*, size_t, int, int, void*, hipStream_t))dlsym(hnd, "ncclAllReduce");
    a.CommCount = (int (*)(void*, int*))dlsym(hnd, "ncclCommCount");
    a.GetErrorString = (const char* (*)(int))dlsym(hnd, "ncclGetErrorString");
    a.ok = a.GetUniqueId && a.CommInitRank && a.CommDestroy && a.AllReduce;
    return a;
  }();
  return &api;
}
int rccl_fail(const char* what, int rc) {
  RcclApi* a = rccl_api();
  return fail(D3IL_ERCCL, std::string(what) + ": " + (a->GetErrorString ? a->GetErrorString(rc) : "RCCL error") + " (" + std::to_string(rc) + ")");
}
}

int d3il_rccl_available(void) { return rccl_api()->ok ? 1 : 0; }
int d3il_comm_count(d3il_comm comm, int* ranks) {
  if (!comm || !ranks) return fail(D3IL_EINVAL, "d3il_comm_count: null argument");
  RcclApi* a = rccl_api();
  if (!a->ok || !a->CommCount) return fail(D3IL_ERCCL, "d3il_comm_count: RCCL could not be resolved");
  if (int rc = a->CommCount((void*)comm, ranks)) return rccl_fail("ncclCommCount", rc);
  return D3IL_OK;
}
int d3il_comm_unique_id(d3il_rccl_unique_id* out) {
  if (!out) return fail(D3IL_EINVAL, "d3il_comm_unique_id: null argument");
  RcclApi* a = rccl_api();
  if (!a->ok) return fail(D3IL_ERCCL, "d3il_comm_unique_id: RCCL (librccl.so) could not be resolved");
  if (int rc = a->GetUniqueId(out)) return rccl_fail("ncclGetUniqueId", rc);
  return D3IL_OK;
}
int d3il_comm_init(const d3il_rccl_unique_id* id, int rank, int world, int device_id, d3il_comm* out) {
  if (!id || !out) return fail(D3IL_EINVAL, "d3il_comm_init: null argument");
  if (world < 1 || rank < 0 || rank >= world) return fail(D3IL_EINVAL, "d3il_comm_init: need 0 <= rank < world");
  RcclApi* a = rccl_api();
  if (!a->ok) return fail(D3IL_ERCCL, "d3il_comm_init: RCCL (librccl.so) could not be resolved");
  HIPCHK(hipSetDevice(device_id));
  void* comm = nullptr;
  if (int rc = a->CommInitRank(&comm, world, *id, rank)) return rccl_fail("ncclCommInitRank", rc);
  *out = (d3il_comm)comm;
  return D3IL_OK;
}
int d3il_comm_destroy(d3il_comm comm) {
  if (!comm) return fail(D3IL_EINVAL, "d3il_comm_destroy: null communicator");
  RcclApi* a = rccl_api();
  if (!a->ok) return fail(D3IL_ERCCL, "d3il_comm_destroy: RCCL could not be resolved");
  if (int rc = a->CommDestroy((void*)comm)) return rccl_fail("ncclCommDestroy", rc);
  return D3IL_OK;
}
int d3il_reduce_metrics(d3il_handle h, d3il_comm comm, int64_t* table_device, size_t count, void* stream) {
  GROUP_SETTLE(h);
  if (!comm || (!h && !table_device)) return fail(D3IL_EINVAL, "d3il_reduce_metrics: null argument");
  if (!table_device) { table_device = h->tally_table; count = (size_t)h->tally_nctx * D3IL_TALLY_ROW; }
  if (!table_device || count == 0) return fail(D3IL_EINVAL, "d3il_reduce_metrics: no table (pass one, or register it with d3il_set_tally)");
  RcclApi* a = rccl_api();
  if (!a->ok) return fail(D3IL_ERCCL, "d3il_reduce_metrics: RCCL could not be resolved");
  if (h) HIPCHK(hipSetDevice(h->device));
  if (int rc = a->AllReduce(table_device, table_device, count, 4, 0, (void*)comm, (hipStream_t)stream)) return rccl_fail("ncclAllReduce", rc);
  return D3IL_OK;
}

int d3il_set_timing(d3il_handle h, int enabled) {
  GROUP_SETTLE(h);
  if (!h) return fail(D3IL_EINVAL, "d3il_set_timing: null handle");
  HIPCHK(hipSetDevice(h->device));
  if (enabled && !h->ring_created) {
    for (int i = 0; i < 128; i++) { HIPCHK(hipEventCreateWithFlags(&h->ring0[i], EV_TIMING_FLAGS)); HIPCHK(hipEventCreateWithFlags(&h->ring1[i], EV_TIMING_FLAGS)); }
    h->ring_created = true;
  }
  if (h->rg_ready) { HIPCHK(hipDeviceSynchronize()); rg_drop(h); }
  if (enabled) { HIPCHK(hipDeviceSynchronize()); h->ring_head = h->ring_drained = h->t_n = 0; h->t_sum = 0; h->t_min = 1e300; h->t_max = 0; }
  h->timing = enabled != 0; h->ev_valid = false;
  return D3IL_OK;
}
int d3il_timing_stats(d3il_handle h, double* out4) {
  GROUP_SETTLE(h);
  if (!h || !out4) return fail(D3IL_EINVAL, "d3il_timing_stats: null argument");
  HIPCHK(hipSetDevice(h->device));
  while (h->ring_drained < h->ring_head) { if (int rc = timing_drain_one(h)) return rc; }
  out4[0] = h->t_sum; out4[1] = h->t_n ? h->t_min : 0.0; out4[2] = h->t_max; out4[3] = (double)h->t_n;
  return D3IL_OK;
}
int d3il_step_auto_reset(d3il_handle h, const double* actions, int64_t* episode_counts_device, void* stream) {
  GROUP_SETTLE(h);
  if (h && h->task_id == D3IL_TASK_AVOIDING && split_step_kernel(h)) {
    if (!episode_counts_device) return fail(D3IL_EINVAL, "d3il_step_auto_reset: the Avoiding task needs episode_counts (device i64[2])");
    if (int rc = step_launch(h, actions, stream, nullptr, 1u)) return rc;
    return d3il_auto_reset(h, episode_counts_device, stream);
  }
  if (int rc = d3il_step(h, actions, stream)) return rc;
  return d3il_auto_reset(h, episode_counts_device, stream);
}
static void rg_drop(d3il_handle_s* h) {
  if (!h->rg_ready) return;
  for (int k = 0; k < RG_SLOTS; k++) { (void)hipGraphExecDestroy(h->rg_exec[k]); (void)hipGraphDestroy(h->rg_graph[k]); }
  h->rg_ready = false;
}
static int rg_capture(d3il_handle h, uint64_t seed, uint64_t env_offset, uint32_t t, double* actions, int64_t* counts, hipStream_t s) {
  if (int rc_ = drop_prepared_action(h)) return rc_;
  if (!h->rg_t_dev) HIPCHK(hipMalloc(&h->rg_t_dev, sizeof(unsigned)));
  HIPCHK(hipMemcpyAsync(h->rg_t_dev, &t, sizeof(unsigned), hipMemcpyHostToDevice, s));
  HIPCHK(hipStreamSynchronize(s));
  h->rg_timing = h->timing;
  for (int k = 0; k < RG_SLOTS; k++) {
    HIPCHK(hipStreamBeginCapture(s, hipStreamCaptureModeRelaxed));
    h->rg_capturing = true; h->rg_slot = k;
    hipLaunchKernelGGL(k_policy_action_dev, dim3((h->n + 255) / 256), dim3(256), 0, s, h->buf.policy_des, actions, (unsigned long long)seed, (unsigned long long)env_offset,
                       (const unsigned*)h->rg_t_dev, h->n, h->stride);
    int rc = d3il_step(h, actions, s);
    if (!rc) rc = d3il_auto_reset(h, counts, s);
    if (!rc) hipLaunchKernelGGL(k_inc_counter, dim3(1), dim3(64), 0, s, h->rg_t_dev);
    h->rg_capturing = false;
    hipGraph_t g = nullptr;
    hipError_t e = hipStreamEndCapture(s, &g);
    if (rc || e != hipSuccess || !g) {
      for (int j = 0; j < k; j++) { (void)hipGraphExecDestroy(h->rg_exec[j]); (void)hipGraphDestroy(h->rg_graph[j]); }
      if (g) (void)hipGraphDestroy(g);
      return rc ? rc : fail(D3IL_EHIP, std::string("graph_rollout: stream capture failed: ") + hipGetErrorString(e));
    }
    h->rg_graph[k] = g;
    e = hipGraphInstantiate(&h->rg_exec[k], g, nullptr, nullptr, 0);
    if (e != hipSuccess) {
      for (int j = 0; j < k; j++) { (void)hipGraphExecDestroy(h->rg_exec[j]); (void)hipGraphDestroy(h->rg_graph[j]); }
      (void)hipGraphDestroy(g);
      return fail(D3IL_EHIP, std::string("graph_rollout: hipGraphInstantiate: ") + hipGetErrorString(e));
    }
  }
  h->rg_seed = seed; h->rg_off = env_offset; h->rg_actions = actions; h->rg_counts = counts; h->rg_stream = s; h->rg_next_t = t;
  h->rg_launched = h->rg_drained = 0; h->rg_ready = true;
  return D3IL_OK;
}
int d3il_random_rollout_prepare(d3il_handle h, uint64_t seed, uint64_t env_offset, uint32_t t, double* actions, int64_t* episode_counts_device, void* stream) {
  GROUP_SETTLE(h);
  if (!h || !actions) return fail(D3IL_EINVAL, "d3il_random_rollout_prepare: null argument");
  if (!(h->rg_enabled && h->task_id == D3IL_TASK_AVOIDING && stream != nullptr && h->started)) return D3IL_OK;
  hipStream_t s = (hipStream_t)stream;
  HIPCHK(hipSetDevice(h->device));
  if (h->rg_ready && (h->rg_seed != seed || h->rg_off != env_offset || h->rg_actions != actions || h->rg_counts != episode_counts_device || h->rg_stream != s ||
                      h->rg_timing != h->timing)) {
    HIPCHK(hipStreamSynchronize(h->rg_stream));
    rg_drop(h);
  }
  if (!h->rg_ready) return rg_capture(h, seed, env_offset, t, actions, episode_counts_device, s);
  return D3IL_OK;
}
static bool continues_sequence(const d3il_handle_s* h, uint64_t seed, uint64_t env_offset, uint32_t t, const double* actions, void* stream) {
  return h->prep_valid && h->prep_t == t && h->prep_seed == seed && h->prep_off == env_offset && h->prep_actions == actions && h->prep_stream == (hipStream_t)stream;
}
static int fused_step_begin(d3il_handle h, uint64_t seed, uint64_t env_offset, uint32_t t, double* actions, int64_t* episode_counts_device, void* stream, AvoidEpilogue& a) {
  const bool cont = continues_sequence(h, seed, env_offset, t, actions, stream);
  if (!h->d_des_before) { HIPCHK(hipSetDevice(h->device)); HIPCHK(hipMalloc(&h->d_des_before, (size_t)h->stride * 2 * sizeof(double))); }
  if (cont) h->prep_valid = 0;
  else { if (int rc = d3il_policy_action(h, seed, env_offset, t, actions, stream)) return rc; }
  d3il_buffers& b = h->buf;
  a = AvoidEpilogue{};
  a.img = h->reset_img; a.state = b.state; a.flags = b.flags; a.steps = b.step_count; a.obs = b.obs; a.done = b.done; a.success = b.success; a.mode = b.mode;
  a.n = h->n; a.stride = h->stride; a.des = b.policy_des; a.episode_counts = (long long*)episode_counts_device; a.mask = h->d_mask; a.ctx_id = h->tally_ctx;
  a.table = (long long*)h->tally_table; a.actions = actions; a.des_before = h->d_des_before; a.seed = seed; a.env_offset = env_offset; a.n_ctx = h->tally_nctx;
  if (split_step_kernel(h)) {
    if (!h->epilogue_valid || std::memcmp(&h->epilogue_host, &a, sizeof a) != 0) {
      HIPCHK(hipSetDevice(h->device));
      if (h->epilogue_valid && (h->epilogue_stream != (hipStream_t)stream || h->group)) HIPCHK(hipDeviceSynchronize());
      HIPCHK(hipMemcpyAsync(h->d_epilogue, &a, sizeof a, hipMemcpyHostToDevice, (hipStream_t)stream));
      HIPCHK(hipStreamSynchronize((hipStream_t)stream));
      h->epilogue_host = a; h->epilogue_valid = true; h->epilogue_stream = (hipStream_t)stream;
    }
  }
  return D3IL_OK;
}
static void fused_step_end(d3il_handle h, uint64_t seed, uint64_t env_offset, uint32_t t, double* actions, void* stream) {
  h->prep_valid = true; h->prep_t = t + 1u; h->prep_seed = seed; h->prep_off = env_offset; h->prep_actions = actions; h->prep_stream = (hipStream_t)stream;
}
static int rollout_step_single(d3il_handle h, uint64_t seed, uint64_t env_offset, uint32_t t, double* actions, int64_t* episode_counts_device, void* stream) {
  if (h && h->rg_enabled && h->task_id == D3IL_TASK_AVOIDING && stream != nullptr && actions && h->started) {
    hipStream_t s = (hipStream_t)stream;
    if (int rc_ = drop_prepared_action(h)) return rc_;
    if (int rc = d3il_random_rollout_prepare(h, seed, env_offset, t, actions, episode_counts_device, stream)) return rc;
    if (t != h->rg_next_t) { HIPCHK(hipMemcpyAsync(h->rg_t_dev, &t, sizeof(unsigned), hipMemcpyHostToDevice, s)); HIPCHK(hipStreamSynchronize(s)); }
    if (h->timing && h->rg_launched % RG_SAMPLE == RG_SAMPLE - 1) {
      if (int rc = d3il_policy_action(h, seed, env_offset, t, actions, stream)) return rc;
      if (int rc = d3il_step(h, actions, stream)) return rc;
      if (int rc = d3il_auto_reset(h, episode_counts_device, stream)) return rc;
      hipLaunchKernelGGL(k_inc_counter, dim3(1), dim3(64), 0, s, h->rg_t_dev);
      HIPCHK(hipGetLastError());
    } else HIPCHK(hipGraphLaunch(h->rg_exec[h->rg_launched % RG_SLOTS], s));
    h->rg_launched++; h->rg_next_t = t + 1;
    return D3IL_OK;
  }
  if (h && h->fuse_tail && h->task_id == D3IL_TASK_AVOIDING && actions && episode_counts_device && h->started) {
    AvoidEpilogue a;
    if (int rc = fused_step_begin(h, seed, env_offset, t, actions, episode_counts_device, stream, a)) return rc;
    if (split_step_kernel(h)) {
      if (int rc = step_launch(h, actions, stream, h->d_epilogue, t + 1u)) return rc;
    } else {
      if (int rc = d3il_step(h, actions, stream)) return rc;
      hipLaunchKernelGGL(k_avoiding_tail, dim3(h->stride / WAVE), dim3(WAVE), 0, (hipStream_t)stream, a, t + 1u);
      HIPCHK(hipGetLastError());
    }
    fused_step_end(h, seed, env_offset, t, actions, stream);
    return D3IL_OK;
  }
  if (int rc = d3il_policy_action(h, seed, env_offset, t, actions, stream)) return rc;
  if (int rc = d3il_step(h, actions, stream)) return rc;
  return d3il_auto_reset(h, episode_counts_device, stream);
}

static int group_flush(d3il_group_s* g) {
  if (g->busy) return D3IL_OK;
  group_arm(g);
  g->busy = true;
  int rc = D3IL_OK;
  for (int i = 0; i < g->count; i++) {
    d3il_handle_s* h = g->m[i];
    if (!h->grp_pending) continue;
    h->grp_pending = false; g->n_pending--;
    if (!rc) rc = rollout_step_single(h, h->grp_seed, h->grp_off, h->grp_t, h->grp_actions, h->grp_counts, (void*)h->grp_stream);
  }
  for (int k = 0; k < g->n_sets; k++) g->set[k].n_pending = 0;
  g->n_pending = 0; g->busy = false;
  return rc;
}
static int group_launch_locked(d3il_group_s* grp, d3il_dispatch_set* g) {
  HIPCHK(hipSetDevice(grp->device));
  if (!g->ev_made) {
    for (int i = 0; i < AVOID_GROUP_MAX; i++) HIPCHK(hipEventCreateWithFlags(&g->ev_join[i], EV_ORDER_FLAGS));
    HIPCHK(hipEventCreateWithFlags(&g->ev_done, EV_ORDER_FLAGS));
    HIPCHK(hipMalloc(&g->d_table, sizeof(AvoidGroupTable)));
    g->ev_made = true;
  }
  AvoidGroupTable tab;
  std::memset(&tab, 0, sizeof tab);
  unsigned total = 0; int serve_budget = 0;
  for (int i = 0; i < AVOID_GROUP_MAX; i++) tab.m[i].first_wg = 0xFFFFFFFFu;
  for (int i = 0; i < g->count; i++) {
    d3il_handle_s* h = g->m[i];
    AvoidEpilogue a;
    if (int rc = fused_step_begin(h, h->grp_seed, h->grp_off, h->grp_t, h->grp_actions, h->grp_counts, (void*)h->grp_stream, a)) return rc;
    const d3il_buffers& b = h->buf;
    AvoidGroupMember& r = tab.m[i];
    r.state = b.state; r.flags = b.flags; r.steps = b.step_count; r.actions = h->grp_actions; r.obs = b.obs; r.done = b.done; r.success = b.success; r.mode = b.mode;
    r.ep = h->d_epilogue; r.n = h->n; r.stride = h->stride; r.first_wg = total;
    total += (unsigned)((h->n + WAVE - 1) / WAVE); serve_budget += h->serve_max_wg;
  }
  hipStream_t s0 = g->m[0]->grp_stream;
  if (!g->table_valid || std::memcmp(&g->table_host, &tab, sizeof tab) != 0) {
    if (g->table_valid) HIPCHK(hipDeviceSynchronize());
    HIPCHK(hipMemcpy(g->d_table, &tab, sizeof tab, hipMemcpyHostToDevice));
    g->table_host = tab; g->table_valid = true;
  }
  const bool join = !grp->quiet || g->armed;
  if (join) for (int i = 1; i < g->count; i++) {
    if (g->m[i]->grp_stream == s0) continue;
    HIPCHK(hipEventRecord(g->ev_join[i], g->m[i]->grp_stream));
    HIPCHK(hipStreamWaitEvent(s0, g->ev_join[i], 0));
  }
  hipEvent_t t0 = nullptr, t1 = nullptr;
  if (g->timing) {
    if (!g->ring_created) {
      for (int i = 0; i < 128; i++) { HIPCHK(hipEventCreateWithFlags(&g->ring0[i], EV_TIMING_FLAGS)); HIPCHK(hipEventCreateWithFlags(&g->ring1[i], EV_TIMING_FLAGS)); }
      g->ring_created = true;
    }
    for (int i = 0; i < g->count; i++) { d3il_handle_s* h = g->m[i]; if (h->ring_head - h->ring_drained >= 128) { if (int rc = timing_drain_one(h)) return rc; } }
    t0 = g->ring0[g->ring_head % 128]; t1 = g->ring1[g->ring_head % 128];
    HIPCHK(hipEventRecord(t0, s0));
  }
  const d3il_handle_s* h0 = g->m[0];
  const unsigned t_next = g->t + 1u;
  if ((long)total <= (long)serve_budget)
    hipLaunchKernelGGL((k_avoiding_step_split<true, true, true>), dim3(total), dim3(3 * WAVE), AVOID_LDS_SERVE, s0, (const AvoidGroupTable*)g->d_table, (double*)nullptr, (unsigned*)nullptr,
                       (int*)nullptr, (const double*)nullptr, (float*)nullptr, (unsigned char*)nullptr, (unsigned char*)nullptr, (unsigned short*)nullptr, 0, 0, h0->hc.n_substeps,
                       h0->hc.max_steps, (const AvoidEpilogue*)nullptr, t_next);
  else
    hipLaunchKernelGGL((k_avoiding_step_split<true, false, true>), dim3(total), dim3(2 * WAVE), 0, s0, (const AvoidGroupTable*)g->d_table, (double*)nullptr, (unsigned*)nullptr,
                       (int*)nullptr, (const double*)nullptr, (float*)nullptr, (unsigned char*)nullptr, (unsigned char*)nullptr, (unsigned short*)nullptr, 0, 0, h0->hc.n_substeps,
                       h0->hc.max_steps, (const AvoidEpilogue*)nullptr, t_next);
  HIPCHK(hipGetLastError());
  hipEvent_t done_ev = g->ev_done;
  if (g->timing) {
    HIPCHK(hipEventRecord(t1, s0));
    done_ev = t1;
    for (int i = 0; i < g->count; i++) {
      d3il_handle_s* h = g->m[i];
      const int slot = (int)(h->ring_head % 128);
      h->ring_alt0[slot] = t0; h->ring_alt1[slot] = t1; h->ev0 = t0; h->ev1 = t1; h->ev_valid = true; h->ring_head++;
    }
    g->ring_head++;
  } else HIPCHK(hipEventRecord(done_ev, s0));
  for (int i = 1; i < g->count; i++) if (g->m[i]->grp_stream != s0) HIPCHK(hipStreamWaitEvent(g->m[i]->grp_stream, done_ev, 0));
  for (int i = 0; i < g->count; i++) { d3il_handle_s* h = g->m[i]; fused_step_end(h, h->grp_seed, h->grp_off, h->grp_t, h->grp_actions, (void*)h->grp_stream); }
  grp->n_merged++; grp->n_joined += join ? 1 : 0;
  g->armed = false;
  return D3IL_OK;
}
static int group_launch(d3il_group_s* g, d3il_dispatch_set* s) {
  g->busy = true;
  const int rc = group_launch_locked(g, s);
  for (int i = 0; i < s->count; i++) s->m[i]->grp_pending = false;
  g->n_pending -= s->n_pending; s->n_pending = 0;
  if (rc) {
    group_arm(g);
    for (int i = 0; i < g->count; i++) g->m[i]->grp_pending = false;
    for (int k = 0; k < g->n_sets; k++) g->set[k].n_pending = 0;
    g->n_pending = 0;
  }
  g->busy = false;
  return rc;
}
static int group_rollout_step(d3il_handle h, uint64_t seed, uint64_t env_offset, uint32_t t, double* actions, int64_t* episode_counts_device, void* stream, int* handled) {
  d3il_group_s* g = h->group;
  *handled = 0;
  if (g->busy) return D3IL_OK;
  const bool eligible = h->fuse_tail && !h->rg_enabled && h->task_id == D3IL_TASK_AVOIDING && actions && episode_counts_device && h->started && split_step_kernel(h) &&
                        h->serve_avail && continues_sequence(h, seed, env_offset, t, actions, stream);
  if (!eligible) {
    group_arm(g);
    return g->n_pending ? group_flush(g) : D3IL_OK;
  }
  d3il_dispatch_set* s = &g->set[h->grp_set];
  if (s->n_pending && (h->grp_pending || s->t != t || s->n_substeps != h->hc.n_substeps || s->max_steps != h->hc.max_steps || s->timing != h->timing)) {
    if (int rc = group_flush(g)) return rc;
  }
  if (!s->n_pending) { s->t = t; s->n_substeps = h->hc.n_substeps; s->max_steps = h->hc.max_steps; s->timing = h->timing; }
  h->grp_pending = true; h->grp_seed = seed; h->grp_off = env_offset; h->grp_t = t; h->grp_actions = actions; h->grp_counts = episode_counts_device; h->grp_stream = (hipStream_t)stream;
  s->n_pending++; g->n_pending++;
  *handled = 1;
  return s->n_pending == s->count ? group_launch(g, s) : D3IL_OK;
}
int d3il_random_rollout_step(d3il_handle h, uint64_t seed, uint64_t env_offset, uint32_t t, double* actions, int64_t* episode_counts_device, void* stream) {
  if (h && h->group) {
    int handled = 0;
    if (int rc = group_rollout_step(h, seed, env_offset, t, actions, episode_counts_device, stream, &handled)) return rc;
    if (handled) return D3IL_OK;
  }
  return rollout_step_single(h, seed, env_offset, t, actions, episode_counts_device, stream);
}
static void timing_drain_all(d3il_handle_s* h) { while (h->ring_drained < h->ring_head) { if (timing_drain_one(h)) { h->ring_drained = h->ring_head; break; } } }
static void group_forget_events(d3il_handle_s* h) {
  timing_drain_all(h);
  if (h->ring_head > 0 && h->ring_alt0[(h->ring_head - 1) % 128]) { h->ev_valid = false; h->ev0 = h->ev1 = nullptr; }
  for (int i = 0; i < 128; i++) h->ring_alt0[i] = h->ring_alt1[i] = nullptr;
}
static void group_leave(d3il_handle_s* h) {
  d3il_group_s* g = h->group;
  if (!g) return;
  (void)group_flush(g);
  group_arm(g);
  group_forget_events(h);
  d3il_dispatch_set* s = &g->set[h->grp_set];
  if (h->grp_pending) { s->n_pending--; g->n_pending--; }
  int k = 0;
  for (int i = 0; i < s->count; i++) if (s->m[i] != h) s->m[k++] = s->m[i];
  s->count = k;
  k = 0;
  for (int i = 0; i < g->count; i++) if (g->m[i] != h) g->m[k++] = g->m[i];
  g->count = k; h->group = nullptr; h->grp_pending = false;
}
static void group_partition(d3il_group_s* g, int k) {
  const int base = g->count / k, extra = g->count % k;
  g->n_sets = k;
  int i = 0;
  for (int j = 0; j < AVOID_GROUP_MAX; j++) {
    d3il_dispatch_set* s = &g->set[j];
    s->count = j < k ? base + (j < extra ? 1 : 0) : 0;
    s->n_pending = 0;
    for (int q = 0; q < s->count; q++, i++) {
      d3il_handle_s* h = g->m[i];
      if (h->grp_set != j) group_forget_events(h);
      s->m[q] = h; h->grp_set = j;
    }
  }
}
int d3il_group_create(const d3il_handle* handles, int count, d3il_group* out) {
  if (!handles || !out) return fail(D3IL_EINVAL, "d3il_group_create: null argument");
  *out = nullptr;
  if (count < 1 || count > AVOID_GROUP_MAX) return fail(D3IL_EINVAL, "d3il_group_create: a group has 1 .. 8 members");
  for (int i = 0; i < count; i++) {
    d3il_handle_s* h = handles[i];
    if (!h) return fail(D3IL_EINVAL, "d3il_group_create: null handle");
    if (h->task_id != D3IL_TASK_AVOIDING) return fail(D3IL_EUNSUPPORTED, "d3il_group_create: Avoiding handles only");
    if (h->device != handles[0]->device) return fail(D3IL_EINVAL, "d3il_group_create: the members must live on one device");
    if (h->group) return fail(D3IL_ESTATE, "d3il_group_create: a handle is already in a group");
    for (int j = 0; j < i; j++) if (handles[j] == h) return fail(D3IL_EINVAL, "d3il_group_create: a handle is listed twice");
  }
  HIPCHK(hipSetDevice(handles[0]->device));
  if (hipFuncSetAttribute((const void*)k_avoiding_step_split<true, true, true>, hipFuncAttributeMaxDynamicSharedMemorySize, (int)AVOID_LDS_SERVE) != hipSuccess) (void)hipGetLastError();
  d3il_group_s* g = new d3il_group_s();
  g->device = handles[0]->device; g->count = count;
  group_arm(g);
  for (int i = 0; i < count; i++) { g->m[i] = handles[i]; handles[i]->group = g; handles[i]->grp_set = 0; handles[i]->grp_pending = false; }
  group_partition(g, 1);
  *out = g;
  return D3IL_OK;
}
int d3il_group_flush(d3il_group g) {
  if (!g) return fail(D3IL_EINVAL, "d3il_group_flush: null group");
  group_arm(g);
  return g->n_pending ? group_flush(g) : D3IL_OK;
}
int d3il_group_set_option(d3il_group g, const char* name, int value) {
  if (!g || !name) return fail(D3IL_EINVAL, "d3il_group_set_option: null argument");
  if (std::strcmp(name, "quiet_streams") == 0) {
    if (value != 0 && value != 1) return fail(D3IL_EINVAL, "quiet_streams must be 0 or 1");
    group_arm(g);
    if (g->n_pending) { if (int rc = group_flush(g)) return rc; }
    g->quiet = value != 0;
    return D3IL_OK;
  }
  if (std::strcmp(name, "dispatch_sets") == 0) {
    if (value < 1 || value > g->count) return fail(D3IL_EINVAL, "dispatch_sets must be 1 .. the number of members");
    group_arm(g);
    if (g->n_pending) { if (int rc = group_flush(g)) return rc; }
    (void)hipSetDevice(g->device);
    group_partition(g, value);
    return D3IL_OK;
  }
  return fail(D3IL_EINVAL, std::string("d3il_group_set_option: unknown option ") + name);
}
int d3il_group_stats(d3il_group g, int64_t* merged_rounds, int64_t* joined_rounds) {
  if (!g || !merged_rounds || !joined_rounds) return fail(D3IL_EINVAL, "d3il_group_stats: null argument");
  *merged_rounds = g->n_merged; *joined_rounds = g->n_joined;
  return D3IL_OK;
}
int d3il_group_destroy(d3il_group g) {
  if (!g) return fail(D3IL_EINVAL, "d3il_group_destroy: null group");
  (void)hipSetDevice(g->device);
  const int rc = group_flush(g);
  while (g->count > 0) group_leave(g->m[g->count - 1]);
  (void)hipDeviceSynchronize();
  for (int k = 0; k < AVOID_GROUP_MAX; k++) {
    d3il_dispatch_set* s = &g->set[k];
    if (s->ev_made) { for (int i = 0; i < AVOID_GROUP_MAX; i++) (void)hipEventDestroy(s->ev_join[i]); (void)hipEventDestroy(s->ev_done); (void)hipFree(s->d_table); }
    if (s->ring_created) for (int i = 0; i < 128; i++) { (void)hipEventDestroy(s->ring0[i]); (void)hipEventDestroy(s->ring1[i]); }
  }
  delete g;
  return rc;
}
int d3il_last_step_ms(d3il_handle h, float* ms) {
  GROUP_SETTLE(h);
  if (!h || !ms) return fail(D3IL_EINVAL, "d3il_last_step_ms: null argument");
  if (!h->ev_valid) return fail(D3IL_ESTATE, "d3il_last_step_ms: timing not enabled or no step recorded");
  HIPCHK(hipEventSynchronize(h->ev1));
  HIPCHK(hipEventElapsedTime(ms, h->ev0, h->ev1));
  return D3IL_OK;
}
int d3il_debug_wave_stats(uint64_t* out, int nwaves, int reset) {
#if defined(D3IL_DEVICE_STATS)
  HIPCHK(hipDeviceSynchronize());
  HIPCHK(hipMemcpyFromSymbol(out, HIP_SYMBOL(d3il::g_dev_wave), (size_t)nwaves * 10 * sizeof(unsigned long long)));
  if (reset) { static unsigned long long z[4096][10]; HIPCHK(hipMemcpyToSymbol(HIP_SYMBOL(d3il::g_dev_wave), z, sizeof z)); }
  return D3IL_OK;
#else
  (void)out; (void)nwaves; (void)reset;
  return fail(D3IL_EUNSUPPORTED, "d3il_debug_wave_stats: library built without D3IL_DEVICE_STATS");
#endif
}

int d3il_debug_wave_counts(uint64_t* out, int nwaves, int reset) {
#if defined(D3IL_DEVICE_STATS)
  HIPCHK(hipDeviceSynchronize());
  HIPCHK(hipMemcpyFromSymbol(out, HIP_SYMBOL(d3il::g_dev_cnt), (size_t)nwaves * 8 * sizeof(unsigned long long)));
  if (reset) { static unsigned long long z[4096][8]; HIPCHK(hipMemcpyToSymbol(HIP_SYMBOL(d3il::g_dev_cnt), z, sizeof z)); }
  return D3IL_OK;
#else
  (void)out; (void)nwaves; (void)reset;
  return fail(D3IL_EUNSUPPORTED, "d3il_debug_wave_counts: library built without D3IL_DEVICE_STATS");
#endif
}

int d3il_debug_stats(uint64_t* out32, int reset) {
#if defined(D3IL_DEVICE_STATS)
  unsigned long long tmp[32];
  HIPCHK(hipDeviceSynchronize());
  HIPCHK(hipMemcpyFromSymbol(tmp, HIP_SYMBOL(d3il::g_dev_stats), sizeof tmp));
  for (int i = 0; i < 32; i++) out32[i] = tmp[i];
  if (reset) { unsigned long long z[32] = {0}; HIPCHK(hipMemcpyToSymbol(HIP_SYMBOL(d3il::g_dev_stats), z, sizeof z)); }
  return D3IL_OK;
#else
  (void)out32; (void)reset;
  return fail(D3IL_EUNSUPPORTED, "d3il_debug_stats: library built without D3IL_DEVICE_STATS");
#endif
}

int d3il_debug_scratch(d3il_handle h, int env, double* out, int count) {
  GROUP_SETTLE(h);
  if (!h || !out) return fail(D3IL_EINVAL, "d3il_debug_scratch: null argument");
  if (!h->d_scratch || env < 0 || env >= h->n) return fail(D3IL_EINVAL, "d3il_debug_scratch: no scratch area / env out of range");
  HIPCHK(hipSetDevice(h->device));
  HIPCHK(hipDeviceSynchronize());
  if (h->task_id == D3IL_TASK_STACKING || h->task_id == D3IL_TASK_ALIGNING) {
    if (count > SG_SIZE) return fail(D3IL_EINVAL, "d3il_debug_scratch: count exceeds the environment's scratch area");
    HIPCHK(hipMemcpy(out, h->d_scratch + (size_t)env * SG_SIZE, (size_t)count * sizeof(double), hipMemcpyDeviceToHost));
    return D3IL_OK;
  }
  if (gen_task(h->task_id)) {
    if (count > GG_SIZE) return fail(D3IL_EINVAL, "d3il_debug_scratch: count exceeds the environment's scratch area");
    const double* base = h->d_scratch + (size_t)(env / GEN_LANES) * GG_BLOCK * GEN_LANES + 2 * (env % GEN_LANES);
    HIPCHK(hipMemcpy2D(out, 2 * sizeof(double), base, (size_t)2 * GEN_LANES * sizeof(double), sizeof(double), (size_t)(count + 1) / 2, hipMemcpyDeviceToHost));
    HIPCHK(hipMemcpy2D(out + 1, 2 * sizeof(double), base + 1, (size_t)2 * GEN_LANES * sizeof(double), sizeof(double), (size_t)count / 2, hipMemcpyDeviceToHost));
    return D3IL_OK;
  }
  HIPCHK(hipMemcpy2D(out, sizeof(double), h->d_scratch + env, (size_t)h->stride * sizeof(double), sizeof(double), (size_t)count, hipMemcpyDeviceToHost));
  return D3IL_OK;
}

int d3il_debug_build_flags(int* out8) {
  if (!out8) return fail(D3IL_EINVAL, "d3il_debug_build_flags: null argument");
  int f = 0;
#if defined(D3IL_POISON)
  f |= D3IL_BUILD_POISON;
#endif
#if defined(D3IL_SK_POISON)
  f |= D3IL_BUILD_SK_POISON;
#endif
#if defined(D3IL_DEVICE_STATS)
  f |= D3IL_BUILD_STATS;
#endif
  out8[0] = f; out8[1] = GG_SIZE; out8[2] = GEN_SEG; out8[3] = GREC; out8[4] = GEN_MAXNB; out8[5] = GL_SIZE; out8[6] = GEN_LANES; out8[7] = 0;
  return D3IL_OK;
}

int d3il_set_link_guard(d3il_handle h, const double* capsules, int n, double margin, int64_t* flagged_episodes_device) {
  if (!h) return fail(D3IL_EINVAL, "d3il_set_link_guard: null handle");
  if (!gen_task(h->task_id)) return fail(D3IL_EUNSUPPORTED, "d3il_set_link_guard: Pushing / Sorting / Inserting only (Stacking and Aligning have their own guard, D3IL_SFLAG_HAND_NEAR; Avoiding has no objects)");
  LinkGuardConsts lg;
  const char* err = "";
  if (build_link_guard(h->model, capsules, n, margin, lg, &err)) return fail(D3IL_EINVAL, std::string("d3il_set_link_guard: ") + err);
  HIPCHK(hipSetDevice(h->device));
  HIPCHK(hipDeviceSynchronize());
  if (h->rg_ready) rg_drop(h);
  if (n > 0) {
    if (!h->d_lg) HIPCHK(hipMalloc(&h->d_lg, sizeof(LinkGuardConsts)));
    HIPCHK(hipMemcpy(h->d_lg, &lg, sizeof(LinkGuardConsts), hipMemcpyHostToDevice));
  }
  h->lg = lg; h->lg_flagged = n > 0 ? flagged_episodes_device : nullptr;
  return D3IL_OK;
}

int d3il_set_option(d3il_handle h, const char* name, int value) {
  GROUP_SETTLE(h);
  if (!h || !name) return fail(D3IL_EINVAL, "d3il_set_option: null argument");
  if (h->rg_ready) { HIPCHK(hipDeviceSynchronize()); rg_drop(h); }
  if (std::strcmp(name, "graph_rollout") == 0) { if (int rc_ = drop_prepared_action(h)) return rc_; h->rg_enabled = value != 0; return D3IL_OK; }
  if (std::strcmp(name, "fuse_rollout_tail") == 0) { if (int rc_ = drop_prepared_action(h)) return rc_; h->fuse_tail = value != 0; return D3IL_OK; }
  if (std::strcmp(name, "ik_fast_path") == 0) { h->fast = value != 0; return D3IL_OK; }
  if (std::strcmp(name, "solver_strict") == 0) { h->tol_mode = value != 0; return D3IL_OK; }
  if (std::strcmp(name, "stack_reset_coop") == 0) { h->stack_reset_coop = value != 0; return D3IL_OK; }
  if (std::strcmp(name, "split_waves") == 0) { h->split = value; return D3IL_OK; }
  if (std::strcmp(name, "serve_wave_max_workgroups") == 0) { if (value < 0) return fail(D3IL_EINVAL, "serve_wave_max_workgroups must be >= 0"); h->serve_max_wg = h->serve_avail ? value : 0; return D3IL_OK; }
  if (std::strcmp(name, "lds_pad_bytes") == 0) { h->lds_pad = value; return D3IL_OK; }
  if (std::strcmp(name, "lanes_per_wave") == 0) { if (value < 1 || value > WAVE) return fail(D3IL_EINVAL, "lanes_per_wave must be in 1..64"); h->lanes = value; return D3IL_OK; }
  return fail(D3IL_EINVAL, std::string("d3il_set_option: unknown option ") + name);
}

}
```

### d3il_amd/envs/avoiding.py

```python
from __future__ import annotations

import ctypes as C

import numpy as np
import torch

from .. import capi
from ..controllers.offline_ik import offline_ik
from ..kinematics import UrdfChain
from ..model import blob as blob_mod


class _DevArray:

    def __init__(self, ptr, shape, typestr, owner):
        self.__cuda_array_interface__ = {"shape": tuple(shape), "typestr": typestr, "data": (int(ptr), False), "version": 2}
        self._owner = owner


def _view(ptr, shape, typestr, device, owner):
    return torch.as_tensor(_DevArray(ptr, shape, typestr, owner), device=device)


class StepGroup:

    MAX_MEMBERS = 8

    def __init__(self, envs, quiet_streams: bool = False, dispatch_sets: int = 1):
        envs = list(envs)
        if not capi.has_step_group():
            raise capi.D3ilError("the loaded libd3il_rollout has no step group (d3il_group_create)")
        self.L = capi.load()
        arr = (C.c_void_p * len(envs))(*[e.h for e in envs])
        g = C.c_void_p()
        capi.check(self.L.d3il_group_create(arr, len(envs), C.byref(g)))
        self.g = g
        if quiet_streams:
            self.set_option("quiet_streams", 1)
        self.dispatch_sets = 1
        if dispatch_sets != 1:
            self.set_option("dispatch_sets", dispatch_sets)

    def set_option(self, name: str, value: int):
        if not capi.has_group_options():
            raise capi.D3ilError("the loaded libd3il_rollout has no group options (d3il_group_set_option)")
        capi.check(self.L.d3il_group_set_option(self.g, name.encode(), int(value)))
        if name == "dispatch_sets":
            self.dispatch_sets = int(value)

    def try_option(self, name: str, value: int) -> bool:
        if not capi.has_group_options():
            return False
        try:
            self.set_option(name, value)
        except capi.D3ilError as e:
            if capi.is_unknown_group_option(e):
                return False
            raise
        return True

    def stats(self):
        merged, joined = C.c_int64(), C.c_int64()
        capi.check(self.L.d3il_group_stats(self.g, C.byref(merged), C.byref(joined)))
        return merged.value, joined.value

    def flush(self):
        if self.g:
            capi.check(self.L.d3il_group_flush(self.g))

    def close(self):
        if getattr(self, "g", None):
            self.L.d3il_group_destroy(self.g)
            self.g = None

    def __del__(self):
        try:
            self.close()
        except Exception:
            pass


class ObstacleAvoidanceVecEnv:
    task = "avoiding"
    action_dim = 7
    obs_dim = 2

    default_max_steps = 250

    def __init__(self, n_envs: int, device: int | str | torch.device = 0, render: bool = False,
                 n_substeps: int = 35, max_steps_per_episode: int | None = None):
        if max_steps_per_episode is None:
            max_steps_per_episode = self.default_max_steps
        if render:
            raise NotImplementedError("rendering is outside the batched rollout path")
        dev = torch.device(device if not isinstance(device, int) else "cuda:%d" % device)
        if dev.type != "cuda":
            raise capi.D3ilError("%s needs a HIP device (got %s); there is no CPU fallback" % (type(self).__name__, dev))
        self.device = dev
        self.n_envs = int(n_envs)
        self.L = capi.load()
        self.js = blob_mod.load_json(self.task)
        self.js["task_const"]["n_substeps"] = int(n_substeps)
        self.js["task_const"]["max_steps"] = int(max_steps_per_episode)
        self.blob = blob_mod.pack(self.js)
        self.n_substeps, self.max_steps_per_episode = int(n_substeps), int(max_steps_per_episode)
        h = C.c_void_p()
        capi.check(self.L.d3il_create(self.blob.task_id, self.n_envs, dev.index or 0, C.byref(self.blob), C.sizeof(self.blob), C.byref(h)))
        self.h = h
        b = capi.Buffers()
        capi.check(self.L.d3il_get_buffers(self.h, C.byref(b)))
        self.stride = b.stride
        n, s = self.n_envs, b.stride
        self.obs = _view(b.obs, (n, b.obs_dim), "<f4", dev, self)
        self.done = _view(b.done, (n,), "|u1", dev, self)
        self.success = _view(b.success, (n,), "|u1", dev, self)
        self.mode = _view(b.mode, (n,), "<i2", dev, self)
        self.state_rows = b.state_rows
        self.state = _view(b.state, (b.state_rows, s), "<f8", dev, self)
        self.info_f64 = _view(b.info_f64, (b.n_info_f64, s), "<f8", dev, self) if b.n_info_f64 else None
        self.flags = _view(b.flags, (s,), "<i4", dev, self)
        self.step_count = _view(b.step_count, (s,), "<i4", dev, self)
        self.policy_des = _view(b.policy_des, (3, s), "<f8", dev, self)
        self.last_reset = _view(b.last_reset, (n,), "|u1", dev, self)
        self._tally = None
        self._bound_stream = None
        self.init_qpos = None
        self._started = False

    def start(self):
        c, tc = self.js["controller"], self.js["task_const"]
        chain = UrdfChain(self.js["urdf_chain"])
        target = list(tc["init_end_eff_pos"]) + list(tc["init_end_eff_quat"])
        q, iters, err = offline_ik(chain, c["default_qpos"], target, np.array(c["joint_pos_min"]), np.array(c["joint_pos_max"]))
        self.set_init_qpos(q)
        return q, iters, err

    def set_init_qpos(self, q):
        q = np.ascontiguousarray(q, dtype=np.float64)
        capi.check(self.L.d3il_start(self.h, q.ctypes.data_as(C.c_void_p)))
        self.init_qpos = q.copy()
        self._started = True

    def _stream(self):
        if self._bound_stream is not None:
            return self._bound_stream
        return C.c_void_p(torch.cuda.current_stream(self.device).cuda_stream)

    def bind_stream(self, stream: "torch.cuda.Stream | None"):
        self._bound_stream = None if stream is None else C.c_void_p(stream.cuda_stream)

    def step_auto_reset(self, action: torch.Tensor, episode_counts: torch.Tensor):
        capi.check(self.L.d3il_step_auto_reset(self.h, C.c_void_p(action.data_ptr()), C.c_void_p(episode_counts.data_ptr()), self._stream()))

    def random_rollout_step(self, seed: int, env_offset: int, t: int, actions: torch.Tensor, episode_counts: torch.Tensor):
        capi.check(self.L.d3il_random_rollout_step(self.h, int(seed), int(env_offset), int(t), C.c_void_p(actions.data_ptr()), C.c_void_p(episode_counts.data_ptr()), self._stream()))

    def random_rollout_prepare(self, seed: int, env_offset: int, t: int, actions: torch.Tensor, episode_counts: torch.Tensor):
        capi.check(self.L.d3il_random_rollout_prepare(self.h, int(seed), int(env_offset), int(t), C.c_void_p(actions.data_ptr()), C.c_void_p(episode_counts.data_ptr()), self._stream()))

    def timing_stats(self):
        out = (C.c_double * 4)()
        capi.check(self.L.d3il_timing_stats(self.h, out))
        return float(out[0]), float(out[1]), float(out[2]), int(out[3])

    def reset(self, mask: torch.Tensor | None = None, random=True, context=None):
        mp = None
        if mask is not None:
            mask = mask.to(device=self.device, dtype=torch.uint8).contiguous()
            assert mask.numel() == self.n_envs
            mp = C.c_void_p(mask.data_ptr())
        with torch.cuda.device(self.device):
            capi.check(self.L.d3il_reset(self.h, mp, None, self._stream()))
        return self.obs

    def step(self, action: torch.Tensor):
        if action.device != self.device or action.dtype != torch.float64 or tuple(action.shape) != (self.n_envs, 7) or not action.is_contiguous():
            raise ValueError("action must be a contiguous float64 tensor of shape (%d, 7) on %s" % (self.n_envs, self.device))
        with torch.cuda.device(self.device):
            capi.check(self.L.d3il_step(self.h, C.c_void_p(action.data_ptr()), self._stream()))
        return self.obs, None, self.done, (self.mode, self.success)

    def robot_state(self):
        return self.state[capi.STATE_TCP:capi.STATE_TCP + 3, :self.n_envs].t()

    def mode_encoding(self):
        bits = torch.arange(9, device=self.device)
        return ((self.mode.to(torch.int32).unsqueeze(1) >> bits) & 1).to(torch.float32)

    def get_state(self):
        st = np.zeros((self.state_rows, self.n_envs))
        fl = np.zeros(self.n_envs, dtype=np.uint32)
        sc = np.zeros(self.n_envs, dtype=np.int32)
        capi.check(self.L.d3il_get_state(self.h, st.ctypes.data_as(C.c_void_p), st.shape[0], fl.ctypes.data_as(C.c_void_p), sc.ctypes.data_as(C.c_void_p)))
        return st, fl, sc

    def set_state(self, st, fl, sc):
        st = np.ascontiguousarray(st, np.float64); fl = np.ascontiguousarray(fl, np.uint32); sc = np.ascontiguousarray(sc, np.int32)
        assert st.ndim == 2 and st.shape[1] == self.n_envs
        capi.check(self.L.d3il_set_state(self.h, st.ctypes.data_as(C.c_void_p), st.shape[0], fl.ctypes.data_as(C.c_void_p), sc.ctypes.data_as(C.c_void_p)))

    def policy_begin(self, mask: torch.Tensor | None = None):
        mp = None
        if mask is not None:
            mask = mask.to(device=self.device, dtype=torch.uint8).contiguous()
            mp = C.c_void_p(mask.data_ptr())
        with torch.cuda.device(self.device):
            capi.check(self.L.d3il_policy_begin(self.h, mp, self._stream()))

    def policy_action(self, seed: int, env_offset: int, t: int, out: torch.Tensor):
        with torch.cuda.device(self.device):
            capi.check(self.L.d3il_policy_action(self.h, int(seed), int(env_offset), int(t), C.c_void_p(out.data_ptr()), self._stream()))
        return out

    def auto_reset(self, episode_counts: torch.Tensor | None = None):
        if episode_counts is None:
            if self.task == "avoiding":
                raise ValueError("the Avoiding auto-reset needs episode_counts (int64[2] on the env's device)")
            ptr = None
        else:
            assert episode_counts.dtype == torch.int64 and episode_counts.numel() >= 2 and episode_counts.device == self.device
            ptr = C.c_void_p(episode_counts.data_ptr())
        with torch.cuda.device(self.device):
            capi.check(self.L.d3il_auto_reset(self.h, ptr, self._stream()))

    def set_tally(self, n_ctx: int = 1, ctx_id: torch.Tensor | None = None):
        table = torch.zeros(int(n_ctx), capi.TALLY_ROW, dtype=torch.int64, device=self.device)
# ... 42 lines not shown
```

### d3il_amd/envs/sub_batch.py

```python
from __future__ import annotations

import copy
import os
import warnings

import torch

MIN_ENVS = 64
DEFAULT_HW_QUEUES = 4
MAX_CONCURRENT = 4
CUS = 256


def plan(n: int, n_sub_batches: int, min_envs: int = MIN_ENVS):
    s = max(1, min(int(n_sub_batches), n // min_envs if n >= min_envs else 1))
    base, extra = divmod(n, s)
    out, off = [], 0
    for i in range(s):
        c = base + (1 if i < extra else 0)
        out.append((off, c))
        off += c
    return out


def ensure_hw_queues(n_streams: int):
    cur = os.environ.get("GPU_MAX_HW_QUEUES")
    have = int(cur) if cur and cur.isdigit() else DEFAULT_HW_QUEUES
    if have >= n_streams:
        return have
    if not torch.cuda.is_initialized():
        os.environ["GPU_MAX_HW_QUEUES"] = str(n_streams)
        return n_streams
    warnings.warn("%d sub-batches but GPU_MAX_HW_QUEUES = %d was fixed when HIP initialised: their streams share hardware queues and will not fully "
                  "overlap (export GPU_MAX_HW_QUEUES=%d before the first GPU call)" % (n_streams, have, n_streams))
    return have


def fork_agent(agent):
    if hasattr(agent, "fork"):
        return agent.fork()
    from ..agents import _is_lane_state
    c = copy.copy(agent)
    for k, v in list(vars(agent).items()):
        if k.startswith("_parameters") or k.startswith("_modules") or k.startswith("_buffers"):
            continue
        if _is_lane_state(v):
            setattr(c, k, copy.deepcopy(v))
    return c


class SubBatch:
    __slots__ = ("index", "offset", "n", "env", "stream", "own_stream", "agent", "state")

    def __init__(self, index, offset, n, env, stream, own_stream):
        self.index, self.offset, self.n, self.env, self.stream, self.own_stream = index, offset, n, env, stream, own_stream
        self.agent, self.state = None, None


class SubBatchSet:

    def __init__(self, n: int, n_sub_batches: int, device, make_env, min_envs: int = MIN_ENVS):
        self.device = torch.device(device)
        self.parts = plan(n, n_sub_batches, min_envs)
        self.n = n
        S = len(self.parts)
        hw_queues = ensure_hw_queues(S) if S > 1 else DEFAULT_HW_QUEUES
        self.group = None
        if S > MAX_CONCURRENT:
            warnings.warn("%d sub-batches: the GPU runs %d dispatches of different streams at a time, the others wait their turn (DESIGN section 19.6)" % (S, MAX_CONCURRENT))
        self.default_stream = torch.cuda.current_stream(self.device)
        self.batches = []
        for i, (off, cnt) in enumerate(self.parts):
            own = S > 1
            stream = torch.cuda.Stream(self.device) if own else self.default_stream
            with torch.cuda.stream(stream):
                env = make_env(cnt, off)
                if own:
                    env.bind_stream(stream)
                if own and hasattr(env, "set_option") and type(env).__name__ == "ObstacleAvoidanceVecEnv":
                    env.set_option("serve_wave_max_workgroups", CUS // S)
            self.batches.append(SubBatch(i, off, cnt, env, stream, own))
        if S > 1:
            for b in self.batches:
                self.default_stream.wait_stream(b.stream)
            self.group = self._step_group(hw_queues)

    def _step_group(self, hw_queues: int):
        envs = [b.env for b in self.batches]
        want = hw_queues < len(envs) + 1
        if os.environ.get("D3IL_STEP_GROUP") in ("0", "1"):
            want = os.environ["D3IL_STEP_GROUP"] == "1"
        if not want or not all(type(e).__name__ == "ObstacleAvoidanceVecEnv" for e in envs):
            return None
        from .avoiding import StepGroup
        from .. import capi
        if len(envs) > StepGroup.MAX_MEMBERS or not capi.has_step_group():
            return None
        group = StepGroup(envs, quiet_streams=capi.has_group_options())
        sets = 2 if len(envs) >= 4 and len(envs) % 2 == 0 and hw_queues >= 3 else 1
        if os.environ.get("D3IL_STEP_GROUP_SETS") in ("1", "2"):
            sets = int(os.environ["D3IL_STEP_GROUP_SETS"])
        if sets != 1 and sets <= len(envs):
            group.try_option("dispatch_sets", sets)
        return group

    def __len__(self):
        return len(self.batches)

    def __iter__(self):
        return iter(self.batches)

    def each(self, fn):
        if len(self.batches) == 1:
            fn(self.batches[0])
            return
        try:
            for b in self.batches:
                torch.cuda.set_stream(b.stream)
                fn(b)
        finally:
            torch.cuda.set_stream(self.default_stream)

    def join(self):
        if self.group is not None:
            self.group.flush()
        if len(self.batches) > 1:
            for b in self.batches:
                self.default_stream.wait_stream(b.stream)

    def fork_agents(self, agent):
        from ..agents import as_batched
        for b in self.batches:
            a = agent if len(self.batches) == 1 else fork_agent(agent)
            if hasattr(a, "set_rollout_range"):
                a.set_rollout_range(b.offset, b.n)
            b.agent = as_batched(a, b.n)
            if b.agent is not a and hasattr(b.agent, "set_rollout_range"):
                b.agent.set_rollout_range(b.offset, b.n)
            b.agent.reset()

    @property
    def link_near_episodes(self) -> int:
        return sum(int(getattr(b.env, "link_near_episodes", 0)) for b in self.batches if b.env is not None)

    def close(self):
        if self.group is not None:
            self.group.close()
            self.group = None
        for b in self.batches:
            if b.env is not None:
                b.env.close()
                b.env = None
```

### include/d3il_rollout.h

```cpp
#ifndef D3IL_ROLLOUT_H
#define D3IL_ROLLOUT_H
#include <stddef.h>
#include <stdint.h>
#include "d3il_model_blob.h"

#ifdef __cplusplus
extern "C" {
#endif

typedef struct d3il_handle_s* d3il_handle;

enum {
  D3IL_OK = 0, D3IL_EINVAL = -1, D3IL_EBLOB = -2, D3IL_ENODEVICE = -3, D3IL_EHIP = -4, D3IL_EUNSUPPORTED = -5,
  D3IL_ESTATE = -6, D3IL_ERCCL = -7
};


enum {
  D3IL_STATE_QPOS = 0,
  D3IL_STATE_QVEL = 9,
  D3IL_STATE_BIAS = 18,
  D3IL_STATE_TCP = 25,
  D3IL_STATE_IK_Q = 28,
  D3IL_STATE_IK_QD = 35,
  D3IL_STATE_F64 = 42,
  D3IL_PUSH_STATE_BOX = 42, D3IL_PUSH_STATE_WARM = 68, D3IL_PUSH_STATE_TASK = 89, D3IL_PUSH_STATE_F64 = 91,
  D3IL_SORT_STATE_BOX = 42, D3IL_SORT_STATE_WARM = 94, D3IL_SORT_STATE_TASK = 127, D3IL_SORT_STATE_F64 = 129,
  D3IL_STACK_STATE_BOX = 28, D3IL_STACK_STATE_WARM = 67, D3IL_STACK_STATE_F64 = 94,
  D3IL_ALIGN_STATE_BOX = 42, D3IL_ALIGN_STATE_WARM = 55, D3IL_ALIGN_STATE_TARGET = 70, D3IL_ALIGN_STATE_F64 = 77,
  D3IL_INS_STATE_BOX = 42, D3IL_INS_STATE_WARM = 81, D3IL_INS_STATE_TASK = 108, D3IL_INS_STATE_F64 = 110
};
enum {
  D3IL_FLAG_MODE_MASK = 0x1FF,
  D3IL_FLAG_L1 = 1 << 9, D3IL_FLAG_L2 = 1 << 10, D3IL_FLAG_L3 = 1 << 11,
  D3IL_FLAG_TERMINATED = 1 << 12, D3IL_FLAG_SUCCESS = 1 << 13, D3IL_FLAG_ROD_CONTACT = 1 << 14,
  D3IL_FLAG_IK_VALID = 1 << 15,
  D3IL_FLAG_SOLVER_FAIL = 1 << 16,
  D3IL_FLAG_MULTI_CONTACT = 1 << 17,
  D3IL_PFLAG_FIRST_MASK = 0x7,
  D3IL_PFLAG_MODE_MASK = 0x38,
  D3IL_PFLAG_WARM_VALID = 1 << 6,
  D3IL_PFLAG_CON_OVERFLOW = 1 << 18,
  D3IL_PFLAG_OFF_TABLE = 1 << 19,
  D3IL_PFLAG_LINK_NEAR = 1 << 20,
  D3IL_SFLAG_MODE_MASK = 0xFF,
  D3IL_SFLAG_WARM_VALID = 1 << 8,
  D3IL_SFLAG_HAND_NEAR = 1 << 20
};

typedef struct d3il_buffers {
  int32_t n_envs, stride, obs_dim, action_dim;
  float* obs;
  uint8_t* done;
  uint8_t* success;
  uint16_t* mode;
  double* state;
  uint32_t* flags;
  int32_t* step_count;
  double* policy_des;
  double* info_f64;
  int32_t n_info_f64, state_rows;
  uint8_t* last_reset;
} d3il_buffers;

int d3il_create(int task_id, int n_envs, int device_id, const void* model_blob, size_t blob_len, d3il_handle* out);
int d3il_destroy(d3il_handle h);

int d3il_start(d3il_handle h, const double* init_qpos7);

int d3il_reset(d3il_handle h, const uint8_t* env_mask, const double* contexts, void* stream);

int d3il_step(d3il_handle h, const double* actions, void* stream);

int d3il_get_buffers(d3il_handle h, d3il_buffers* out);

int d3il_get_state(d3il_handle h, double* state, int32_t state_rows, uint32_t* flags, int32_t* steps);
int d3il_set_state(d3il_handle h, const double* state, int32_t state_rows, const uint32_t* flags, const int32_t* steps);

int d3il_policy_begin(d3il_handle h, const uint8_t* env_mask, void* stream);
int d3il_policy_action(d3il_handle h, uint64_t seed, uint64_t env_offset, uint32_t t, double* actions, void* stream);

int d3il_auto_reset(d3il_handle h, int64_t* episode_counts_device, void* stream);

int d3il_attention_causal_f32(const float* qkv, float* out, int B, int T, int H, int D, void* stream);

int d3il_layernorm_f32(const float* x, const float* weight, const float* bias, float* y, long rows, int C, float eps, void* stream);
int d3il_mlp_gelu_residual_f32(const float* h, const float* x, const float* w_packed, const float* b1, const float* b2, float* out, long rows, int C, int H, void* stream);
int d3il_mlp_ln_gelu_residual_f32(const float* h, const float* ln_weight, const float* ln_bias, float ln_eps, const float* x, const float* w_packed, const float* b1, const float* b2,
                                  float* out, long rows, int C, int H, void* stream);
int d3il_linear120_f32(const float* xin, const float* ln_weight, const float* ln_bias, float ln_eps, const float* w_packed, const float* bias, const float* resid, float* out,
                       long rows, int N, void* stream);

int d3il_mlp_ln_gelu_residual_f16x3(const float* h, const float* ln_weight, const float* ln_bias, float ln_eps, const float* x, const void* w_packed, const float* b1, const float* b2,
                                    float* out, long rows, int C, int H, void* stream);
int d3il_linear120_f16x3(const float* xin, const float* ln_weight, const float* ln_bias, float ln_eps, const void* w_packed, const float* bias, const float* resid, float* out,
                         long rows, int N, void* stream);
int d3il_attn_half_f16x3(const float* x, const float* ln_weight, const float* ln_bias, float ln_eps, const void* w_packed, const float* b_qkv, const float* b_proj, float* out,
                         long n_seq, int T, int n_head, int C, void* stream);
int d3il_bet_head_f32(const float* h, const float* ln_weight, const float* ln_bias, float ln_eps, const float* w_head, const float* centers, const float* lo, const float* hi,
                      const float* scale, const float* shift, uint64_t seed, uint64_t env_offset, const uint32_t* t_device, const float* u_in, float* actions, int32_t* bins,
                      float* u_out, float* probs, long rows, int C, int V, int A, void* stream);
int d3il_ddpm_gpt_step_f32(const float* hk, const float* ln_weight, const float* ln_bias, float ln_eps, const float* w_pred, const float* b_pred, const float* w_aemb,
                           const float* bias_pos, const float* temb, const float* sched, const float* lo, const float* hi, const float* scale, const float* shift,
                           const int64_t* len, uint64_t seed, uint64_t env_offset, const uint32_t* t_device, const float* noise_in, float* x, float* xbuf, float* actions,
                           int32_t* bad, float* noise_out, long n_env, int C, int A, int W, int T, int k, void* stream);
int d3il_ibc_langevin_f32(const float* state, const float* w_in, const float* b_in, const float* w_blocks, const float* b_blocks, const float* w_out, const float* b_out,
                          const float* wT_blocks, const float* wT_in_act, const float* coef, float noise_scale, const float* lo, const float* hi, const float* clip,
                          const float* scale, const float* shift, uint64_t seed, uint64_t env_offset, const uint32_t* t_device, const float* x0_in, const float* noise_in,
                          const float* u_in, float* actions, int32_t* picks, float* x_final, float* energies, float* x0_out, float* noise_out, float* u_out, long n_env,
                          int obs_dim, int A, int hidden, int n_blocks, int S, int K, void* stream);
int d3il_act_chunk_f32(const float* state, const float* w_in, const float* tab, const float* enc_w, const float* enc_v, const float* dec_w, const float* dec_v,
                       const float* head_w, const float* lo, const float* hi, const float* scale, const float* shift, uint64_t seed, uint64_t env_offset,
                       const uint32_t* t_device, const float* latent_in, int32_t* counter, float* chunk, float* actions, float* latent_out, long n_env, int obs_dim, int A,
                       int T, int width, int n_head, int latent, int n_enc, int n_dec, void* stream);
int d3il_ddpm_act_chunk_f32(const float* window, const int64_t* len, const float* w_in, const float* tab, const float* enc_w, const float* enc_v, const float* dec_w,
                            const float* dec_v, const float* head_w, const float* lo, const float* hi, const float* scale, const float* shift, uint64_t seed,
                            uint64_t env_offset, const uint32_t* t_device, const float* noise_in, const float* x_in, int32_t* counter, float* chunk, float* actions,
                            int32_t* bad, float* x_out, float* noise_out, long n_env, int obs_dim, int A, int obs_seq_len, int action_seq_len, int width, int n_head,
                            int n_enc, int n_dec, int n_timesteps, int linear_head, int k_start, int k_stop, void* stream);
int d3il_cvae_decode_f32(const float* state, const float* w_in, const float* b_in, const float* w_blocks, const float* b_blocks, const float* w_out, const float* b_out,
                         const float* lo, const float* hi, const float* scale, const float* shift, uint64_t seed, uint64_t env_offset, const uint32_t* t_device,
                         const float* z_in, float* actions, float* z_out, long n_env, int obs_dim, int latent, int A, int hidden, int n_blocks, void* stream);
enum { D3IL_HXG_CLIPPED = 0, D3IL_HXG_NONFINITE = 1, D3IL_HXG_LAUNCHES = 2, D3IL_HXG_N = 4 };
int d3il_f16x3_set_guard(long long* counts_device);

int d3il_ddpm_mlp_f32(const float* state, const float* noise, const float* temb, const float* w_in, const float* b_in, const float* w_blocks, const float* b_blocks,
                      const float* w_out, const float* b_out, const float* sched, const float* bounds, float* out, long rows, int state_dim, int n_timesteps, int hidden,
                      int n_blocks, void* stream);

int d3il_resmlp_f32(const float* x, const float* w_in, const float* b_in, const float* w_blocks, const float* b_blocks, const float* w_out, const float* b_out, float* out, long rows,
                    int in_dim, int hidden, int n_blocks, int out_dim, void* stream);

enum { D3IL_TALLY_ROW = 2 + 512, D3IL_TALLY_ALL = 256 };
int d3il_set_tally(d3il_handle h, const int32_t* ctx_id_device, int n_ctx, int64_t* table_device);

int d3il_count_metrics(d3il_handle h, int64_t* out_counts_device, void* stream);

typedef struct d3il_comm_s* d3il_comm;
typedef struct { char internal[128]; } d3il_rccl_unique_id;
int d3il_rccl_available(void);
int d3il_comm_unique_id(d3il_rccl_unique_id* out);
int d3il_comm_init(const d3il_rccl_unique_id* id, int rank, int world, int device_id, d3il_comm* out);
int d3il_comm_count(d3il_comm comm, int* ranks);
int d3il_comm_destroy(d3il_comm comm);
int d3il_reduce_metrics(d3il_handle h, d3il_comm comm, int64_t* table_device, size_t count, void* stream);

int d3il_set_timing(d3il_handle h, int enabled);
int d3il_last_step_ms(d3il_handle h, float* ms);
int d3il_timing_stats(d3il_handle h, double* out4);
int d3il_step_auto_reset(d3il_handle h, const double* actions, int64_t* episode_counts_device, void* stream);
int d3il_random_rollout_step(d3il_handle h, uint64_t seed, uint64_t env_offset, uint32_t t, double* actions, int64_t* episode_counts_device, void* stream);
typedef struct d3il_group_s* d3il_group;
int d3il_group_create(const d3il_handle* handles, int count, d3il_group* out);
int d3il_group_flush(d3il_group g);
int d3il_group_set_option(d3il_group g, const char* name, int value);
int d3il_group_stats(d3il_group g, int64_t* merged_rounds, int64_t* joined_rounds);
int d3il_group_destroy(d3il_group g);
int d3il_random_rollout_prepare(d3il_handle h, uint64_t seed, uint64_t env_offset, uint32_t t, double* actions, int64_t* episode_counts_device, void* stream);

int d3il_set_option(d3il_handle h, const char* name, int value);
int d3il_set_link_guard(d3il_handle h, const double* capsules, int n, double margin, int64_t* flagged_episodes_device);
int d3il_debug_stats(uint64_t* out32, int reset);
int d3il_debug_wave_stats(uint64_t* out_nwaves_x10, int nwaves, int reset);
int d3il_debug_wave_counts(uint64_t* out_nwaves_x8, int nwaves, int reset);
int d3il_debug_scratch(d3il_handle h, int env, double* out, int count);
enum { D3IL_BUILD_POISON = 1 , D3IL_BUILD_SK_POISON = 2 ,
       D3IL_BUILD_STATS = 4  };
int d3il_debug_build_flags(int* out8);
const char* d3il_last_error(void);
size_t d3il_blob_sizeof(void);
int d3il_version(void);

#ifdef __cplusplus
}
#endif
#endif
```

Measured before the change: 7.497 million.

## Pipeline grouped avoiding-step rounds across streams with per-workgroup epoch handoff

Adds a pipelined form of the grouped split step kernel. Successive step rounds are issued round-robin onto several member streams, and each workgroup waits on a per-workgroup epoch word in global memory that its predecessor in the prior round publishes, instead of joining all streams through events every round. This is meant to remove per-round launch gaps and cross-stream join overhead by letting consecutive rounds overlap on otherwise idle CUs. In exchange it adds spin-waits with a timeout and fault word, extra vmcnt waits, and host-side fault checks. The Python sub-batch code enables it by default when the CU budget allows a depth of 2 or more.

```diff
diff --git a/d3il_amd/capi.py b/d3il_amd/capi.py
--- a/d3il_amd/capi.py
+++ b/d3il_amd/capi.py
@@ -43,7 +43,7 @@
 EXPORTS = ["d3il_create", "d3il_destroy", "d3il_start", "d3il_reset", "d3il_step", "d3il_get_buffers", "d3il_get_state",
            "d3il_set_state", "d3il_policy_begin", "d3il_policy_action", "d3il_attention_causal_f32", "d3il_layernorm_f32", "d3il_mlp_gelu_residual_f32", "d3il_mlp_ln_gelu_residual_f32", "d3il_linear120_f32", "d3il_mlp_ln_gelu_residual_f16x3", "d3il_linear120_f16x3", "d3il_attn_half_f16x3", "d3il_f16x3_set_guard", "d3il_bet_head_f32", "d3il_ddpm_gpt_step_f32", "d3il_ibc_langevin_f32", "d3il_act_chunk_f32", "d3il_ddpm_act_chunk_f32", "d3il_cvae_decode_f32", "d3il_ddpm_mlp_f32", "d3il_resmlp_f32", "d3il_auto_reset", "d3il_set_tally", "d3il_count_metrics",
            "d3il_rccl_available", "d3il_comm_unique_id", "d3il_comm_init", "d3il_comm_count", "d3il_comm_destroy", "d3il_reduce_metrics", "d3il_set_timing",
-           "d3il_last_step_ms", "d3il_timing_stats", "d3il_step_auto_reset", "d3il_random_rollout_step", "d3il_random_rollout_prepare", "d3il_group_create", "d3il_group_flush", "d3il_group_destroy", "d3il_group_set_option", "d3il_group_stats", "d3il_set_option", "d3il_set_link_guard", "d3il_debug_stats", "d3il_debug_wave_stats", "d3il_debug_wave_counts", "d3il_debug_scratch", "d3il_debug_build_flags", "d3il_last_error", "d3il_blob_sizeof", "d3il_version"]
+           "d3il_last_step_ms", "d3il_timing_stats", "d3il_step_auto_reset", "d3il_random_rollout_step", "d3il_random_rollout_prepare", "d3il_group_create", "d3il_group_flush", "d3il_group_destroy", "d3il_group_set_option", "d3il_group_stats", "d3il_group_pipeline_stats", "d3il_set_option", "d3il_set_link_guard", "d3il_debug_stats", "d3il_debug_wave_stats", "d3il_debug_wave_counts", "d3il_debug_scratch", "d3il_debug_build_flags", "d3il_last_error", "d3il_blob_sizeof", "d3il_version"]
 
 
 class D3ilError(RuntimeError):
@@ -120,6 +120,8 @@
         if hasattr(L, "d3il_group_set_option"):
             L.d3il_group_set_option.argtypes = [C.c_void_p, C.c_char_p, C.c_int]
             L.d3il_group_stats.argtypes = [C.c_void_p, C.POINTER(C.c_int64), C.POINTER(C.c_int64)]
+        if hasattr(L, "d3il_group_pipeline_stats"):
+            L.d3il_group_pipeline_stats.argtypes = [C.c_void_p, C.POINTER(C.c_int64), C.POINTER(C.c_int64)]
         if L.d3il_blob_sizeof() != C.sizeof(ModelBlob):
             raise D3ilError("model blob layout mismatch between include/d3il_model_blob.h and d3il_amd/model/blob.py")
         _LIB = L
@@ -132,6 +134,10 @@
 
 def has_group_options() -> bool:
     return hasattr(load(), "d3il_group_set_option")
+
+
+def has_group_pipeline() -> bool:
+    return hasattr(load(), "d3il_group_pipeline_stats")
 
 
 def is_unknown_group_option(err: Exception) -> bool:
diff --git a/d3il_amd/csrc/rollout.hip b/d3il_amd/csrc/rollout.hip
--- a/d3il_amd/csrc/rollout.hip
+++ b/d3il_amd/csrc/rollout.hip
@@ -207,22 +207,68 @@
   int n, stride;
   unsigned first_wg, pad_;
 };
-struct AvoidGroupTable { AvoidGroupMember m[AVOID_GROUP_MAX]; };
+struct AvoidGroupTable {
+  AvoidGroupMember m[AVOID_GROUP_MAX];
+  unsigned* pipe_fault; unsigned long long pipe_limit;
+};
 typedef const __attribute__((address_space(4))) AvoidGroupTable CGroupTable4;
-template <bool FAST, bool SERVE, bool GROUP = false>
+
+constexpr int PIPE_WORD_STRIDE = 32, PIPE_MAX_DEPTH = 4, PIPE_MAX_WG = 256;
+constexpr unsigned PIPE_FAULT_TIMEOUT = 1u, PIPE_FAULT_CHAINED = 2u;
+typedef __attribute__((address_space(1))) unsigned GU32;
+__device__ __forceinline__ bool pipe_give_up(unsigned fault_word, unsigned long long waited_ticks, unsigned long long limit_ticks) {
+  return fault_word != 0u || waited_ticks > limit_ticks;
+}
+__device__ __forceinline__ unsigned pipe_wait(GU32* word, unsigned want, GU32* fault, unsigned long long limit_ticks) {
+  const unsigned long long t0 = wall_clock64();
+  while (__hip_atomic_load(word, __ATOMIC_RELAXED, __HIP_MEMORY_SCOPE_AGENT) != want) {
+    const unsigned f = __hip_atomic_load(fault, __ATOMIC_RELAXED, __HIP_MEMORY_SCOPE_AGENT);
+    if (pipe_give_up(f, wall_clock64() - t0, limit_ticks)) return f != 0u ? PIPE_FAULT_CHAINED : PIPE_FAULT_TIMEOUT;
+    __builtin_amdgcn_s_sleep(16);
+  }
+  return 0u;
+}
+template <bool FAST, bool SERVE, bool GROUP = false, bool PIPED = false>
 __global__ __launch_bounds__((SERVE ? 3 : 2) * WAVE) void k_avoiding_step_split(typename std::conditional<GROUP, const AvoidGroupTable*, const PandaConsts*>::type __restrict__ cp, double* __restrict__ state,
                                                                   unsigned* __restrict__ flags, int* __restrict__ steps,
                                                                   const double* __restrict__ actions, float* __restrict__ obs,
                                                                   unsigned char* __restrict__ done, unsigned char* __restrict__ success,
                                                                   unsigned short* __restrict__ mode, int n, int stride, int n_substeps, int max_steps,
-                                                                  const AvoidEpilogue* __restrict__ ep, unsigned t_next) {
+                                                                  const AvoidEpilogue* __restrict__ ep, unsigned t_next,
+                                                                  unsigned* epoch, unsigned wait_epoch, unsigned publish_epoch) {
+  static_assert(!PIPED || (GROUP && SERVE), "the pipelined form is a three-wave group form");
   __shared__ double xch[2][2 * NARM][WAVE];
   __shared__ double trg[2][2 * NARM + 1][WAVE];
   extern __shared__ double rx_smem[];
-  __shared__ unsigned long long ep_arg[3];
+  __shared__ unsigned long long ep_arg[PIPED ? 5 : 3];
   const int lane = threadIdx.x & (WAVE - 1);
   const int role = threadIdx.x / WAVE;
   RareXch rx; rx.buf = rx_smem; rx.ctl = (int*)(rx_smem + RX_ROWS * WAVE); rx.lane = lane; rx.seq = 0;
+  if constexpr (PIPED) {
+    __shared__ unsigned pipe_code;
+    if (role == 1) {
+      CGroupTable4* gt = (CGroupTable4*)(unsigned long long)cp;
+      unsigned* const word_p = epoch + (size_t)blockIdx.x * PIPE_WORD_STRIDE;
+      GU32* word = (GU32*)(unsigned long long)word_p;
+      unsigned code = 0u;
+      if (wait_epoch != 0u) {
+        if (lane == 0) {
+          GU32* fault = (GU32*)(unsigned long long)gt->pipe_fault;
+          code = pipe_wait(word, wait_epoch, fault, gt->pipe_limit);
+          if (code != 0u) {
+            __hip_atomic_fetch_or(fault, code, __ATOMIC_RELAXED, __HIP_MEMORY_SCOPE_AGENT);
+            __hip_atomic_store(word, publish_epoch, __ATOMIC_RELAXED, __HIP_MEMORY_SCOPE_AGENT);
+          }
+        }
+        __builtin_amdgcn_fence(__ATOMIC_ACQUIRE, "agent");
+        asm volatile("s_waitcnt vmcnt(0)" ::: "memory");
+      }
+      if (lane == 0) pipe_code = code;
+      ep_arg[3] = (unsigned long long)word_p; ep_arg[4] = publish_epoch;
+    }
+    __syncthreads();
+    if (__builtin_amdgcn_readfirstlane(pipe_code) != 0u) return;
+  }
   unsigned wg_index = blockIdx.x;
   if constexpr (GROUP) {
     CGroupTable4* gt = (CGroupTable4*)(unsigned long long)cp;
@@ -295,6 +341,7 @@
 #pragma unroll
       for (int i = 0; i < NARM; i++) { so[(D3IL_STATE_IK_Q + i) * (size_t)stride] = ikq[i]; so[(D3IL_STATE_IK_QD + i) * (size_t)stride] = ikqd[i]; }
     }
+    if constexpr (PIPED) asm volatile("s_waitcnt vmcnt(0)" ::: "memory");
     __syncthreads();
   } else if (SERVE && role == 2) {
     double warm[6];
@@ -380,6 +427,16 @@
       const unsigned wg = __builtin_amdgcn_readfirstlane((unsigned)ep_arg[2]);
       avoiding_tail_lane(*(CEpilogue4*)ep_bits, __builtin_amdgcn_readfirstlane((unsigned)ep_arg[1]), (int)(wg * WAVE + lane_now));
     }
+    if constexpr (PIPED) {
+      const unsigned w_lo = __builtin_amdgcn_readfirstlane((unsigned)ep_arg[3]), w_hi = __builtin_amdgcn_readfirstlane((unsigned)(ep_arg[3] >> 32));
+      const unsigned pub = __builtin_amdgcn_readfirstlane((unsigned)ep_arg[4]);
+      asm volatile("s_waitcnt vmcnt(0)" ::: "memory");
+      if (lane_now == 0u) {
+        __builtin_amdgcn_fence(__ATOMIC_RELEASE, "agent");
+        asm volatile("s_waitcnt vmcnt(0)" ::: "memory");
+        __hip_atomic_store((GU32*)((unsigned long long)w_lo | ((unsigned long long)w_hi << 32)), pub, __ATOMIC_RELAXED, __HIP_MEMORY_SCOPE_AGENT);
+      }
+    }
   }
 }
 
@@ -936,6 +993,7 @@
 }
 
 constexpr int RG_SLOTS = 2, RG_SAMPLE = 8;
+constexpr int PIPE_TIMEOUT_MS_DEFAULT = 2000;
 struct d3il_handle_s {
   int task_id, n, stride, device;
   PandaConsts hc;
@@ -994,8 +1052,24 @@
   int n_sets; d3il_dispatch_set set[AVOID_GROUP_MAX];
   int n_pending; bool busy;
   bool quiet; int64_t n_merged, n_joined;
+  int pipe_depth, pipe_timeout_ms, cu_count, cu_device, wall_khz;
+  unsigned* d_epoch; unsigned* d_fault;
+  bool pipe_made, pipe_active, pipe_unread; int pipe_d; uint32_t pipe_r;
+  hipStream_t pipe_stream[PIPE_MAX_DEPTH]; hipEvent_t ev_pipe[PIPE_MAX_DEPTH], ev_pipe_start;
+  int64_t n_pipelined, n_pipe_faults;
 };
-static inline void group_arm(d3il_group_s* g) { for (int k = 0; k < AVOID_GROUP_MAX; k++) g->set[k].armed = true; }
+static void pipe_end(d3il_group_s* g) {
+  if (!g->pipe_active) return;
+  g->pipe_active = false;
+  bool ok = hipSetDevice(g->device) == hipSuccess;
+  for (int k = 0; k < g->pipe_d && ok; k++) ok = hipEventRecord(g->ev_pipe[k], g->pipe_stream[k]) == hipSuccess;
+  for (int i = 0; i < g->count && ok; i++) {
+    hipStream_t s = g->m[i]->grp_stream;
+    for (int k = 0; k < g->pipe_d && ok; k++) if (g->pipe_stream[k] != s) ok = hipStreamWaitEvent(s, g->ev_pipe[k], 0) == hipSuccess;
+  }
+  if (!ok) { (void)hipGetLastError(); (void)hipDeviceSynchronize(); }
+}
+static inline void group_arm(d3il_group_s* g) { pipe_end(g); for (int k = 0; k < AVOID_GROUP_MAX; k++) g->set[k].armed = true; }
 #if defined(D3IL_EVENT_SYSTEM_FENCE)
 constexpr unsigned EV_ORDER_FLAGS = hipEventDisableTiming, EV_TIMING_FLAGS = hipEventDefault;
 #else
@@ -1018,6 +1092,7 @@
 extern "C" {
 
 static int group_flush(d3il_group_s* g);
+static int pipe_check_fault(d3il_group_s* g, const char* who);
 static inline int group_settle(d3il_handle_s* h) {
   if (!h || !h->group || h->group->busy) return D3IL_OK;
   group_arm(h->group);
@@ -1191,10 +1266,12 @@
 int d3il_destroy(d3il_handle h) {
   if (!h) return fail(D3IL_EINVAL, "d3il_destroy: null handle");
   (void)hipSetDevice(h->device);
+  d3il_group_s* was_in = h->group;
   group_leave(h);
   (void)hipDeviceSynchronize();
+  const int rc_f = pipe_check_fault(was_in, "d3il_destroy");
   free_handle(h);
-  return D3IL_OK;
+  return rc_f;
 }
 
 int d3il_start(d3il_handle h, const double* init_qpos7) {
@@ -1410,10 +1487,10 @@
   if (ep && !split) return fail(D3IL_ESTATE, "d3il_step: the rollout epilogue needs the split step kernel");
   if (split && nwg <= h->serve_max_wg)
     hipLaunchKernelGGL((k_avoiding_step_split<true, true>), dim3(nwg), dim3(3 * WAVE), AVOID_LDS_SERVE, s, h->dc, b.state, b.flags, b.step_count, actions, b.obs, b.done,
-                       b.success, b.mode, h->n, h->stride, h->hc.n_substeps, h->hc.max_steps, ep, t_next);
+                       b.success, b.mode, h->n, h->stride, h->hc.n_substeps, h->hc.max_steps, ep, t_next, (unsigned*)nullptr, 0u, 0u);
   else if (split)
     hipLaunchKernelGGL((k_avoiding_step_split<true, false>), dim3(nwg), dim3(2 * WAVE), 0, s, h->dc, b.state, b.flags, b.step_count, actions, b.obs, b.done,
-                       b.success, b.mode, h->n, h->stride, h->hc.n_substeps, h->hc.max_steps, ep, t_next);
+                       b.success, b.mode, h->n, h->stride, h->hc.n_substeps, h->hc.max_steps, ep, t_next, (unsigned*)nullptr, 0u, 0u);
   else if (h->fast)
     hipLaunchKernelGGL((k_avoiding_step<true, true>), dim3(nwg), dim3(WAVE), lds, s, h->dc, b.state, b.flags, b.step_count, actions, b.obs, b.done,
                        b.success, b.mode, h->n, h->stride, h->hc.n_substeps, h->hc.max_steps, h->lanes);
@@ -1443,6 +1520,7 @@
   if (int rc_ = check_state_rows(h, state, state_rows, "d3il_get_state")) return rc_;
   HIPCHK(hipSetDevice(h->device));
   HIPCHK(hipDeviceSynchronize());
+  if (int rc_ = pipe_check_fault(h->group, "d3il_get_state")) return rc_;
   if (state) HIPCHK(hipMemcpy2D(state, (size_t)h->n * 8, h->buf.state, (size_t)h->stride * 8, (size_t)h->n * 8, h->state_rows, hipMemcpyDeviceToHost));
   if (flags) HIPCHK(hipMemcpy(flags, h->buf.flags, (size_t)h->n * 4, hipMemcpyDeviceToHost));
   if (steps) HIPCHK(hipMemcpy(steps, h->buf.step_count, (size_t)h->n * 4, hipMemcpyDeviceToHost));
@@ -1886,6 +1964,7 @@
   if (!h || !out4) return fail(D3IL_EINVAL, "d3il_timing_stats: null argument");
   HIPCHK(hipSetDevice(h->device));
   while (h->ring_drained < h->ring_head) { if (int rc = timing_drain_one(h)) return rc; }
+  if (int rc_ = pipe_check_fault(h->group, "d3il_timing_stats")) return rc_;
   out4[0] = h->t_sum; out4[1] = h->t_n ? h->t_min : 0.0; out4[2] = h->t_max; out4[3] = (double)h->t_n;
   return D3IL_OK;
 }
@@ -2028,6 +2107,42 @@
   g->n_pending = 0; g->busy = false;
   return rc;
 }
+constexpr size_t PIPE_EPOCH_BYTES = (size_t)PIPE_MAX_WG * PIPE_WORD_STRIDE * sizeof(unsigned);
+static int pipe_prepare(d3il_group_s* g) {
+  if (g->pipe_made) return D3IL_OK;
+  if (!g->d_epoch) HIPCHK(hipMalloc(&g->d_epoch, PIPE_EPOCH_BYTES));
+  if (!g->d_fault) { HIPCHK(hipMalloc(&g->d_fault, 16)); HIPCHK(hipMemset(g->d_fault, 0, 16)); }
+  for (int k = 0; k < PIPE_MAX_DEPTH; k++) if (!g->ev_pipe[k]) HIPCHK(hipEventCreateWithFlags(&g->ev_pipe[k], EV_ORDER_FLAGS));
+  if (!g->ev_pipe_start) HIPCHK(hipEventCreateWithFlags(&g->ev_pipe_start, EV_ORDER_FLAGS));
+  g->pipe_made = true;
+  return D3IL_OK;
+}
+static int pipe_round_depth(const d3il_group_s* grp, const d3il_dispatch_set* g, unsigned total, bool serve, hipStream_t* ls) {
+  if (grp->pipe_depth < 2 || !grp->quiet || grp->n_sets != 1 || !serve || total > (unsigned)PIPE_MAX_WG) return 1;
+  if ((long)grp->pipe_depth * (long)total > (long)grp->cu_count || grp->wall_khz <= 0) return 1;
+  int n = 0;
+  for (int i = 0; i < g->count && n < grp->pipe_depth; i++) {
+    bool seen = false;
+    for (int k = 0; k < n; k++) seen = seen || ls[k] == g->m[i]->grp_stream;
+    if (!seen) ls[n++] = g->m[i]->grp_stream;
+  }
+  return n >= 2 ? n : 1;
+}
+static int pipe_check_fault(d3il_group_s* g, const char* who) {
+  if (!g || !g->pipe_unread || !g->d_fault) return D3IL_OK;
+  HIPCHK(hipSetDevice(g->device));
+  HIPCHK(hipDeviceSynchronize());
+  unsigned w = 0;
+  HIPCHK(hipMemcpy(&w, g->d_fault, sizeof w, hipMemcpyDeviceToHost));
+  g->pipe_unread = false;
+  if (w == 0u) return D3IL_OK;
+  g->n_pipe_faults++;
+  const unsigned zero = 0u;
+  HIPCHK(hipMemcpy(g->d_fault, &zero, sizeof zero, hipMemcpyHostToDevice));
+  return fail(D3IL_ESTATE, std::string(who) + ": a workgroup of a pipelined step round gave up waiting for its predecessor (fault word " + std::to_string(w) +
+                               ((w & PIPE_FAULT_TIMEOUT) ? ": the time limit \"pipeline_timeout_ms\" ran out" : ": behind an earlier give-up") +
+                               "); it and the rounds behind it did not step - the members do not hold the state after the steps that were called");
+}
 static int group_launch_locked(d3il_group_s* grp, d3il_dispatch_set* g) {
   HIPCHK(hipSetDevice(grp->device));
   if (!g->ev_made) {
@@ -2051,16 +2166,42 @@
     total += (unsigned)((h->n + WAVE - 1) / WAVE); serve_budget += h->serve_max_wg;
   }
   hipStream_t s0 = g->m[0]->grp_stream;
+  const bool serve = (long)total <= (long)serve_budget;
+  hipStream_t ls[PIPE_MAX_DEPTH];
+  const int depth = pipe_round_depth(grp, g, total, serve, ls);
+  if (depth >= 2) {
+    if (int rc = pipe_prepare(grp)) return rc;
+    tab.pipe_fault = grp->d_fault; tab.pipe_limit = (unsigned long long)grp->pipe_timeout_ms * (unsigned long long)grp->wall_khz;
+  } else pipe_end(grp);
   if (!g->table_valid || std::memcmp(&g->table_host, &tab, sizeof tab) != 0) {
     if (g->table_valid) HIPCHK(hipDeviceSynchronize());
     HIPCHK(hipMemcpy(g->d_table, &tab, sizeof tab, hipMemcpyHostToDevice));
     g->table_host = tab; g->table_valid = true;
-  }
-  const bool join = !grp->quiet || g->armed;
+    if (grp->pipe_active) { pipe_end(grp); g->armed = true; }
+  }
+  bool pipe_arming = false;
+  if (depth >= 2) {
+    bool same = grp->pipe_active && grp->pipe_d == depth && grp->pipe_r < 0xFFFFFFF0u;
+    for (int k = 0; k < depth && same; k++) same = grp->pipe_stream[k] == ls[k];
+    pipe_arming = g->armed || !same;
+    if (pipe_arming) pipe_end(grp);
+  }
+  const bool join = depth >= 2 ? pipe_arming : (!grp->quiet || g->armed);
   if (join) for (int i = 1; i < g->count; i++) {
     if (g->m[i]->grp_stream == s0) continue;
     HIPCHK(hipEventRecord(g->ev_join[i], g->m[i]->grp_stream));
     HIPCHK(hipStreamWaitEvent(s0, g->ev_join[i], 0));
+  }
+  hipStream_t sl = s0;
+  if (depth >= 2) {
+    if (pipe_arming) {
+      HIPCHK(hipMemsetAsync(grp->d_epoch, 0, PIPE_EPOCH_BYTES, s0));
+      HIPCHK(hipEventRecord(grp->ev_pipe_start, s0));
+      for (int k = 1; k < depth; k++) HIPCHK(hipStreamWaitEvent(ls[k], grp->ev_pipe_start, 0));
+      grp->pipe_active = true; grp->pipe_d = depth; grp->pipe_r = 0;
+      for (int k = 0; k < depth; k++) grp->pipe_stream[k] = ls[k];
+    }
+    sl = ls[grp->pipe_r % (unsigned)depth];
   }
   hipEvent_t t0 = nullptr, t1 = nullptr;
   if (g->timing) {
@@ -2070,22 +2211,26 @@
     }
     for (int i = 0; i < g->count; i++) { d3il_handle_s* h = g->m[i]; if (h->ring_head - h->ring_drained >= 128) { if (int rc = timing_drain_one(h)) return rc; } }
     t0 = g->ring0[g->ring_head % 128]; t1 = g->ring1[g->ring_head % 128];
-    HIPCHK(hipEventRecord(t0, s0));
+    HIPCHK(hipEventRecord(t0, sl));
   }
   const d3il_handle_s* h0 = g->m[0];
   const unsigned t_next = g->t + 1u;
-  if ((long)total <= (long)serve_budget)
+  if (depth >= 2)
+    hipLaunchKernelGGL((k_avoiding_step_split<true, true, true, true>), dim3(total), dim3(3 * WAVE), AVOID_LDS_SERVE, sl, (const AvoidGroupTable*)g->d_table, (double*)nullptr, (unsigned*)nullptr,
+                       (int*)nullptr, (const double*)nullptr, (float*)nullptr, (unsigned char*)nullptr, (unsigned char*)nullptr, (unsigned short*)nullptr, 0, 0, h0->hc.n_substeps,
+                       h0->hc.max_steps, (const AvoidEpilogue*)nullptr, t_next, grp->d_epoch, (unsigned)grp->pipe_r, (unsigned)grp->pipe_r + 1u);
+  else if (serve)
     hipLaunchKernelGGL((k_avoiding_step_split<true, true, true>), dim3(total), dim3(3 * WAVE), AVOID_LDS_SERVE, s0, (const AvoidGroupTable*)g->d_table, (double*)nullptr, (unsigned*)nullptr,
                        (int*)nullptr, (const double*)nullptr, (float*)nullptr, (unsigned char*)nullptr, (unsigned char*)nullptr, (unsigned short*)nullptr, 0, 0, h0->hc.n_substeps,
-                       h0->hc.max_steps, (const AvoidEpilogue*)nullptr, t_next);
+                       h0->hc.max_steps, (const AvoidEpilogue*)nullptr, t_next, (unsigned*)nullptr, 0u, 0u);
   else
     hipLaunchKernelGGL((k_avoiding_step_split<true, false, true>), dim3(total), dim3(2 * WAVE), 0, s0, (const AvoidGroupTable*)g->d_table, (double*)nullptr, (unsigned*)nullptr,
                        (int*)nullptr, (const double*)nullptr, (float*)nullptr, (unsigned char*)nullptr, (unsigned char*)nullptr, (unsigned short*)nullptr, 0, 0, h0->hc.n_substeps,
-                       h0->hc.max_steps, (const AvoidEpilogue*)nullptr, t_next);
+                       h0->hc.max_steps, (const AvoidEpilogue*)nullptr, t_next, (unsigned*)nullptr, 0u, 0u);
   HIPCHK(hipGetLastError());
   hipEvent_t done_ev = g->ev_done;
   if (g->timing) {
-    HIPCHK(hipEventRecord(t1, s0));
+    HIPCHK(hipEventRecord(t1, sl));
     done_ev = t1;
     for (int i = 0; i < g->count; i++) {
       d3il_handle_s* h = g->m[i];
@@ -2093,9 +2238,10 @@
       h->ring_alt0[slot] = t0; h->ring_alt1[slot] = t1; h->ev0 = t0; h->ev1 = t1; h->ev_valid = true; h->ring_head++;
     }
     g->ring_head++;
-  } else HIPCHK(hipEventRecord(done_ev, s0));
-  for (int i = 1; i < g->count; i++) if (g->m[i]->grp_stream != s0) HIPCHK(hipStreamWaitEvent(g->m[i]->grp_stream, done_ev, 0));
+  } else if (depth < 2) HIPCHK(hipEventRecord(done_ev, s0));
+  if (depth < 2) for (int i = 1; i < g->count; i++) if (g->m[i]->grp_stream != s0) HIPCHK(hipStreamWaitEvent(g->m[i]->grp_stream, done_ev, 0));
   for (int i = 0; i < g->count; i++) { d3il_handle_s* h = g->m[i]; fused_step_end(h, h->grp_seed, h->grp_off, h->grp_t, h->grp_actions, (void*)h->grp_stream); }
+  if (depth >= 2) { grp->pipe_r++; grp->n_pipelined++; grp->pipe_unread = true; }
   grp->n_merged++; grp->n_joined += join ? 1 : 0;
   g->armed = false;
   return D3IL_OK;
@@ -2194,6 +2340,11 @@
   if (hipFuncSetAttribute((const void*)k_avoiding_step_split<true, true, true>, hipFuncAttributeMaxDynamicSharedMemorySize, (int)AVOID_LDS_SERVE) != hipSuccess) (void)hipGetLastError();
   d3il_group_s* g = new d3il_group_s();
   g->device = handles[0]->device; g->count = count;
+  g->pipe_depth = 1; g->pipe_timeout_ms = PIPE_TIMEOUT_MS_DEFAULT;
+  if (hipDeviceGetAttribute(&g->cu_count, hipDeviceAttributeMultiprocessorCount, g->device) != hipSuccess) { g->cu_count = 0; (void)hipGetLastError(); }
+  g->cu_device = g->cu_count;
+  if (hipDeviceGetAttribute(&g->wall_khz, hipDeviceAttributeWallClockRate, g->device) != hipSuccess) { g->wall_khz = 0; (void)hipGetLastError(); }
+  if (hipFuncSetAttribute((const void*)k_avoiding_step_split<true, true, true, true>, hipFuncAttributeMaxDynamicSharedMemorySize, (int)AVOID_LDS_SERVE) != hipSuccess) (void)hipGetLastError();
   group_arm(g);
   for (int i = 0; i < count; i++) { g->m[i] = handles[i]; handles[i]->group = g; handles[i]->grp_set = 0; handles[i]->grp_pending = false; }
   group_partition(g, 1);
@@ -2209,6 +2360,7 @@
   if (!g || !name) return fail(D3IL_EINVAL, "d3il_group_set_option: null argument");
   if (std::strcmp(name, "quiet_streams") == 0) {
     if (value != 0 && value != 1) return fail(D3IL_EINVAL, "quiet_streams must be 0 or 1");
+    if (value == 0 && g->pipe_depth >= 2) return fail(D3IL_EINVAL, "quiet_streams 0: pipeline_depth >= 2 needs quiet_streams 1");
     group_arm(g);
     if (g->n_pending) { if (int rc = group_flush(g)) return rc; }
     g->quiet = value != 0;
@@ -2216,12 +2368,35 @@
   }
   if (std::strcmp(name, "dispatch_sets") == 0) {
     if (value < 1 || value > g->count) return fail(D3IL_EINVAL, "dispatch_sets must be 1 .. the number of members");
+    if (value != 1 && g->pipe_depth >= 2) return fail(D3IL_EINVAL, "dispatch_sets: pipeline_depth >= 2 needs one dispatch set");
     group_arm(g);
     if (g->n_pending) { if (int rc = group_flush(g)) return rc; }
     (void)hipSetDevice(g->device);
     group_partition(g, value);
     return D3IL_OK;
   }
+  if (std::strcmp(name, "pipeline_depth") == 0) {
+    if (value < 1 || value > PIPE_MAX_DEPTH) return fail(D3IL_EINVAL, "pipeline_depth must be 1 .. 4");
+    if (value >= 2 && (!g->quiet || g->n_sets != 1)) return fail(D3IL_EINVAL, "pipeline_depth >= 2 needs quiet_streams 1 and dispatch_sets 1");
+    group_arm(g);
+    if (g->n_pending) { if (int rc = group_flush(g)) return rc; }
+    g->pipe_depth = value;
+    return D3IL_OK;
+  }
+  if (std::strcmp(name, "pipeline_cu_budget") == 0) {
+    if (value < 1 || value > g->cu_device) return fail(D3IL_EINVAL, "pipeline_cu_budget must be 1 .. the device's CU count");
+    group_arm(g);
+    if (g->n_pending) { if (int rc = group_flush(g)) return rc; }
+    g->cu_count = value;
+    return D3IL_OK;
+  }
+  if (std::strcmp(name, "pipeline_timeout_ms") == 0) {
+    if (value < 1 || value > 600000) return fail(D3IL_EINVAL, "pipeline_timeout_ms must be 1 .. 600000");
+    group_arm(g);
+    if (g->n_pending) { if (int rc = group_flush(g)) return rc; }
+    g->pipe_timeout_ms = value;
+    return D3IL_OK;
+  }
   return fail(D3IL_EINVAL, std::string("d3il_group_set_option: unknown option ") + name);
 }
 int d3il_group_stats(d3il_group g, int64_t* merged_rounds, int64_t* joined_rounds) {
@@ -2229,12 +2404,22 @@
   *merged_rounds = g->n_merged; *joined_rounds = g->n_joined;
   return D3IL_OK;
 }
+int d3il_group_pipeline_stats(d3il_group g, int64_t* pipelined_rounds, int64_t* pipeline_faults) {
+  if (!g || !pipelined_rounds || !pipeline_faults) return fail(D3IL_EINVAL, "d3il_group_pipeline_stats: null argument");
+  *pipelined_rounds = g->n_pipelined; *pipeline_faults = g->n_pipe_faults;
+  return D3IL_OK;
+}
 int d3il_group_destroy(d3il_group g) {
   if (!g) return fail(D3IL_EINVAL, "d3il_group_destroy: null group");
   (void)hipSetDevice(g->device);
-  const int rc = group_flush(g);
+  int rc = group_flush(g);
   while (g->count > 0) group_leave(g->m[g->count - 1]);
   (void)hipDeviceSynchronize();
+  if (int rc_f = pipe_check_fault(g, "d3il_group_destroy")) { if (!rc) rc = rc_f; }
+  for (int k = 0; k < PIPE_MAX_DEPTH; k++) if (g->ev_pipe[k]) (void)hipEventDestroy(g->ev_pipe[k]);
+  if (g->ev_pipe_start) (void)hipEventDestroy(g->ev_pipe_start);
+  if (g->d_epoch) (void)hipFree(g->d_epoch);
+  if (g->d_fault) (void)hipFree(g->d_fault);
   for (int k = 0; k < AVOID_GROUP_MAX; k++) {
     d3il_dispatch_set* s = &g->set[k];
     if (s->ev_made) { for (int i = 0; i < AVOID_GROUP_MAX; i++) (void)hipEventDestroy(s->ev_join[i]); (void)hipEventDestroy(s->ev_done); (void)hipFree(s->d_table); }
diff --git a/d3il_amd/envs/avoiding.py b/d3il_amd/envs/avoiding.py
--- a/d3il_amd/envs/avoiding.py
+++ b/d3il_amd/envs/avoiding.py
@@ -64,14 +64,22 @@
         capi.check(self.L.d3il_group_stats(self.g, C.byref(merged), C.byref(joined)))
         return merged.value, joined.value
 
+    def pipeline_stats(self):
+        if not capi.has_group_pipeline():
+            return 0, 0
+        rounds, faults = C.c_int64(), C.c_int64()
+        capi.check(self.L.d3il_group_pipeline_stats(self.g, C.byref(rounds), C.byref(faults)))
+        return rounds.value, faults.value
+
     def flush(self):
         if self.g:
             capi.check(self.L.d3il_group_flush(self.g))
 
     def close(self):
         if getattr(self, "g", None):
-            self.L.d3il_group_destroy(self.g)
-            self.g = None
+            g, self.g = self.g, None
+            if self.L.d3il_group_destroy(g) == -6:
+                capi.check(-6)
 
     def __del__(self):
         try:
diff --git a/d3il_amd/envs/sub_batch.py b/d3il_amd/envs/sub_batch.py
--- a/d3il_amd/envs/sub_batch.py
+++ b/d3il_amd/envs/sub_batch.py
@@ -97,6 +97,14 @@
         if len(envs) > StepGroup.MAX_MEMBERS or not capi.has_step_group():
             return None
         group = StepGroup(envs, quiet_streams=capi.has_group_options())
+        wgs = sum((b.n + MIN_ENVS - 1) // MIN_ENVS for b in self.batches)
+        depth = min(3, len(envs), hw_queues - 1, CUS // max(1, wgs))
+        if os.environ.get("D3IL_STEP_GROUP_PIPE") in ("0", "2", "3"):
+            depth = int(os.environ["D3IL_STEP_GROUP_PIPE"])
+        elif os.environ.get("D3IL_STEP_GROUP_SETS") in ("1", "2"):
+            depth = 1
+        if depth >= 2 and capi.has_group_pipeline() and group.try_option("pipeline_depth", depth):
+            return group
         sets = 2 if len(envs) >= 4 and len(envs) % 2 == 0 and hw_queues >= 3 else 1
         if os.environ.get("D3IL_STEP_GROUP_SETS") in ("1", "2"):
             sets = int(os.environ["D3IL_STEP_GROUP_SETS"])
diff --git a/include/d3il_rollout.h b/include/d3il_rollout.h
--- a/include/d3il_rollout.h
+++ b/include/d3il_rollout.h
@@ -155,6 +155,7 @@
 int d3il_group_flush(d3il_group g);
 int d3il_group_set_option(d3il_group g, const char* name, int value);
 int d3il_group_stats(d3il_group g, int64_t* merged_rounds, int64_t* joined_rounds);
+int d3il_group_pipeline_stats(d3il_group g, int64_t* pipelined_rounds, int64_t* pipeline_faults);
 int d3il_group_destroy(d3il_group g);
 int d3il_random_rollout_prepare(d3il_handle h, uint64_t seed, uint64_t env_offset, uint32_t t, double* actions, int64_t* episode_counts_device, void* stream);
 
```

After: 8.523 million (median of 6 runs). 1.14x the previous value.
